# KrainskiL/CGE.jl

Measured on AMD Instinct MI355X. Metric: edge_alpha_evals_per_sec, higher is better.
Workload: dtype f64

## Files before the change

### cge.jl_amd/api.py

```python
from __future__ import annotations

import atexit
import ctypes as C
import os
import sys
import weakref

import numpy as np

from .args import _SplitRule

_HERE = os.path.dirname(os.path.abspath(__file__))
_LIB_PATH = os.path.join(_HERE, "csrc", "build", "libcge_hip.so")
_lib = None

CGE_OK = 0
_CODES = {-1: "AssertionError", -2: "ErrorException: Trying to split homogenous cluster",
          -3: "ErrorException: Unexpected empty cluster generated", -4: "HIP error / no GPU",
          -5: "collective hook failed", -6: "out of memory", -7: "bad argument"}


class CGEError(RuntimeError):
    def __init__(self, code, msg=""):
        super().__init__(f"{_CODES.get(code, 'error')} (code {code}){': ' + msg if msg else ''}")
# ... 103 lines not shown
            ctx.close()
        except Exception:
            pass


def library_path():
    return _LIB_PATH


def load_library():
    global _lib
    if _lib is None:
        if not os.path.exists(_LIB_PATH):
            raise CGEError(-4, f"{_LIB_PATH} not found: build it with `make -C cge.jl_amd/csrc` "
                               f"(or __graft_entry__.build()); there is no CPU fallback")
        L = C.CDLL(_LIB_PATH)
        L.cge_last_error.restype = C.c_char_p
        L.cge_last_error.argtypes = [C.c_void_p]
        L.cge_idx.restype = C.c_int64
        L.cge_idx.argtypes = [C.c_int64] * 3
        L.cge_destroy.argtypes = [C.c_void_p]
        L.cge_destroy.restype = None
        _lib = L
    return _lib


def read_table(path, column_major=True, n_threads=0):
    L = load_library()
    L.cge_text_table_close.argtypes = [C.c_void_p]
    L.cge_text_table_close.restype = None
    rows, cols, hdr, h = C.c_int64(), C.c_int64(), C.c_int(), C.c_void_p()
    err = C.create_string_buffer(512)
    rc = L.cge_text_table_open(os.fsencode(path), C.c_int(n_threads), C.byref(rows), C.byref(cols), C.byref(hdr),
                               C.byref(h), err, C.c_int64(512))
    if rc != 0:
        raise CGEError(rc, err.value.decode() or f"cannot read {path}")
    try:
        out = np.empty((rows.value, cols.value), dtype=np.float64, order="F" if column_major else "C")
        rc = L.cge_text_table_parse(h, out.ctypes.data_as(C.c_void_p), C.c_int(1 if column_major else 0), err,
                                    C.c_int64(512))
        if rc != 0:
            raise CGEError(rc, err.value.decode() or f"cannot parse {path}")
    finally:
        L.cge_text_table_close(h)
    return out, bool(hdr.value)


def _method_code(method):
    if isinstance(method, _SplitRule):
        return method.code
    if isinstance(method, str):
        return {"rss": 0, "rss2": 1, "size": 2, "diameter": 3}[method]
    return int(method)


def _p(a):
    return None if a is None else a.ctypes.data_as(C.c_void_p)


def _f64(a):
    return np.ascontiguousarray(a, dtype=np.float64)


def _i64(a):
    return np.ascontiguousarray(a, dtype=np.int64)


def _colmajor(a):
    a = np.asfortranarray(np.asarray(a, dtype=np.float64))
    return a, a.ravel(order="K")


def _view_layout(n, d, s0, s1):
    if (d == 1 or s1 == 1) and (n == 1 or s0 >= d):
        return 1, (s0 if n > 1 else d)
    if (n == 1 or s0 == 1) and (d == 1 or s1 >= n):
        return 0, (s1 if d > 1 else n)
    return None


def embedding_view(x):
    if isinstance(x, (int, np.integer)):
        raise TypeError("embedding_view: a raw pointer is not a view (Context.set_embedding_device takes device pointers)")
    torch = sys.modules.get("torch")
    v = EmbeddingView()
    if torch is not None and isinstance(x, torch.Tensor):
        codes = {torch.float64: DTYPE_F64, torch.float32: DTYPE_F32, torch.float16: DTYPE_F16, torch.bfloat16: DTYPE_BF16}
        t = x.detach()
        if t.dtype not in codes:
            raise ValueError(f"embedding_view: tensor dtype {t.dtype} (float64, float32, float16 or bfloat16)")
        if t.dim() != 2 or t.shape[0] < 1 or t.shape[1] < 1:
            raise ValueError("embedding_view: an embedding is a non-empty (n, d) matrix")
        lay = _view_layout(t.shape[0], t.shape[1], *t.stride())
        if lay is None:
            t = t.contiguous()
            lay = 1, t.shape[1]
        v.data, v.d, v.dtype, v.on_device = t.data_ptr(), t.shape[1], codes[t.dtype], int(t.is_cuda)
        v.row_major, v.ld = lay
        return v, t
    a = np.asarray(x)
    if a.dtype not in _NP_DTYPES:
        a = np.asarray(a, dtype=np.float64)
    if a.ndim != 2 or a.shape[0] < 1 or a.shape[1] < 1:
        raise ValueError("embedding_view: an embedding is a non-empty (n, d) matrix")
    sz = a.dtype.itemsize
    lay = None if a.strides[0] % sz or a.strides[1] % sz else _view_layout(a.shape[0], a.shape[1], a.strides[0] // sz, a.strides[1] // sz)
# ... 544 lines not shown
    def vect_b_test(self, GD, Ta, Tb, comm, C_, directed=False, form=0, landmarks=False, vC=None, n_modes=1, second=None,
                    vB=None):
        keep, out = [], {}

        def problem(GD, Ta, Tb, comm, C_, vC, vB, tag):
            C_ = int(C_)
            ln = C_ * C_ if directed else C_ * (C_ + 1) // 2
            q = VectBProblem()
            if GD is not None:
                GD, Ta, Tb, comm = _f64(GD), _f64(Ta), _f64(Tb), _i64(comm)
                q.N = GD.shape[0]
                assert GD.shape == (q.N, q.N) and Ta.shape == Tb.shape == comm.shape == (q.N,)
                vect = np.zeros(ln + VECT_B_GUARD)
                q.GD, q.Ta, q.Tb, q.comm = (a.ctypes.data for a in (GD, Ta, Tb, comm))
            else:
                vect = _f64(vB).copy()
                q.N = C_
                assert vect.shape == (ln,) and vC is not None
            q.C = C_
            js_dev, js_fused = np.full(3, np.nan), np.full(2, np.nan)
            if vC is not None:
                vC = _f64(vC)
                assert vC.shape == (ln,)
                q.vC = vC.ctypes.data
            q.vectB, q.js_dev, q.js_fused = vect.ctypes.data, js_dev.ctypes.data, js_fused.ctypes.data
            keep.extend((GD, Ta, Tb, comm, vC, vect, js_dev, js_fused))
            out[tag + "vectB"], out[tag + "guard"] = vect[:ln], vect[ln:]
            out[tag + "js_dev"], out[tag + "js_fused"] = js_dev, js_fused[:n_modes]
            return q

        p1 = problem(GD, Ta, Tb, comm, C_, vC, vB, "")
        p2 = None
        if second is not None:
            p2 = problem(*second[:5], second[5] if len(second) > 5 else None, None, "second_")
        ran = C.c_int(-1)
        self._check(self.L.cge_vect_b_test(self.h, C.byref(p1), C.byref(p2) if p2 is not None else None, C.c_int(int(directed)),
                                           C.c_int(form), C.c_int(int(landmarks)), C.c_int(n_modes), C.byref(ran)))
        out["form_ran"] = ran.value
        return out

    def segment_sort_test(self, z, offsets):
        z = _f64(z)
        off = np.ascontiguousarray(offsets, dtype=np.int32)
        zs, perm = np.empty_like(z), np.empty(z.size, dtype=np.int32)
        self._check(self.L.cge_segment_sort_test(self.h, _p(z), _p(off), C.c_int64(off.size - 1), _p(zs), _p(perm)))
        return zs, perm

    def wave_tree_test(self, x):
        x = np.ascontiguousarray(x, dtype=np.float64).reshape(-1, 64)
        a, b = np.empty(x.shape[0]), np.empty(x.shape[0])
        self._check(self.L.cge_wave_tree_test(self.h, _p(x), C.c_int64(x.shape[0]), _p(a), _p(b)))
        return a, b

    def js(self, vC, vB, vI=None, internal=True):
        vC, vB = _f64(vC), _f64(vB)
        vi = None if vI is None or len(vI) == 0 else np.ascontiguousarray(vI, dtype=np.uint8)
        out = C.c_double()
        self._check(self.L.cge_js(self.h, _p(vC), _p(vB), C.c_int64(len(vC)), _p(vi), C.c_int(int(bool(internal))),
                                  C.byref(out)))
        return out.value

    def exchange_buffer(self, min_doubles):
        ptr, cap = C.c_void_p(), C.c_int64()
        self._check(self.L.cge_exchange_buffer(self.h, C.c_int64(min_doubles), C.byref(ptr), C.byref(cap)))
        return ptr.value, cap.value

    def set_collectives(self, fn, rank, world):
        cb = ALLREDUCE_FN(fn)
        coll = Collectives(cb, None, rank, world)
        self._keep = [cb, coll]
        self._check(self.L.cge_set_collectives(self.h, C.byref(coll)))

    def set_collectives_ext(self, allgather=None, reduce_scatter=None):
        ag = GATHER_FN(allgather) if allgather else GATHER_FN()
        rs = GATHER_FN(reduce_scatter) if reduce_scatter else GATHER_FN()
        ext = CollectivesExt(ag, rs)
        self._keep = list(getattr(self, "_keep", [])) + [ag, rs, ext]
        self._check(self.L.cge_set_collectives_ext(self.h, C.byref(ext)))

    def clear_collectives(self):
        self._check(self.L.cge_comm_finalize(self.h))
        self._check(self.L.cge_set_collectives(self.h, None))
        self._keep = []

    def init_rccl(self, unique_id: bytes, rank: int, world: int):
        assert len(unique_id) == 128
        buf = C.create_string_buffer(bytes(unique_id), 128)
        self._check(self.L.cge_comm_init_rccl(self.h, buf, C.c_int(rank), C.c_int(world)))

    def finalize_rccl(self):
        self._check(self.L.cge_comm_finalize(self.h))

    def rccl_selftest(self, arr, op=0):
        a = np.ascontiguousarray(arr).copy()
        assert a.dtype.itemsize == 8
        self._check(self.L.cge_rccl_selftest(self.h, _p(a), C.c_int64(a.size), C.c_int(op)))
        return a

    def louvain(self):
        out = np.zeros(self.n, dtype=np.int64)
        nc, q, rounds = C.c_int64(), C.c_double(), C.c_int64()
        self._check(self.L.cge_louvain(self.h, _p(out), C.byref(nc), C.byref(q), C.byref(rounds)))
        return out, nc.value, q.value, rounds.value

    _TEST_OPTIONS = ("fit_persistent_test_delay", "fit_persistent_test_timeout", "test_bvec_plain", "test_rss2_one_kernel",
                     "exact_resident_limit")

    def set_option(self, key, value):
        if key in self._TEST_OPTIONS:
            self._check(self.L.cge_set_test_option(self.h, key.encode(), C.c_int64(int(value))))
            return
        self._check(self.L.cge_set_option(self.h, key.encode(), C.c_int64(int(value))))

    def get_stat(self, key):
        v = C.c_int64()
        self._check(self.L.cge_get_stat(self.h, key.encode(), C.byref(v)))
        return v.value

    def last_diameter(self):
        import struct

        hi = struct.unpack("d", struct.pack("q", self.get_stat("diameter_bits")))[0]
        return hi, {1: "brute", 2: "pruned"}.get(self.get_stat("diameter_path"), "none"), \
            self.get_stat("diameter_candidate_pairs"), self.get_stat("diameter_candidate_tiles")

    def profile_enable(self, on=True):
        self._check(self.L.cge_profile_enable(self.h, C.c_int(int(on))))

    def profile_select(self, names=()):
        self._check(self.L.cge_profile_select(self.h, ",".join(names).encode()))

    def profile_reset(self):
        self._check(self.L.cge_profile_reset(self.h))

    def profile(self):
        buf = C.create_string_buffer(4096)
        self._check(self.L.cge_profile_names(self.h, buf, C.c_int64(4096)))
        res = {}
        for name in filter(None, buf.value.decode().split(",")):
            n, ms = C.c_int64(), C.c_double()
            self._check(self.L.cge_profile_get(self.h, name.encode(), C.byref(n), C.byref(ms)))
            res[name] = {"launches": n.value, "total_ms": ms.value}
        return res

    def phase_ms(self):
        res = {}
        buf = C.create_string_buffer(4096)
        self._check(self.L.cge_phase_names(self.h, buf, C.c_int64(4096)))
        for ph in filter(None, buf.value.decode().split(",")):
            ms = C.c_double()
            self._check(self.L.cge_phase_ms(self.h, ph.encode(), C.byref(ms)))
            res[ph] = ms.value
        return res


_default_ctx = None


def default_context():
# ... 96 lines not shown
```

### cge.jl_amd/csrc/capi.cpp

```cpp
#include "common.hpp"
#include "../../include/cge_hip_testing.h"

void flush_timers(cge_ctx *c) {
    for (auto &kv : c->timers) {
        for (auto &pr : kv.second.pending) {
            float ms = 0.f;
            (void)hipEventSynchronize(pr.second);
            if (hipEventElapsedTime(&ms, pr.first, pr.second) == hipSuccess) kv.second.total_ms += ms;
            c->event_pool.push_back(pr.first);
            c->event_pool.push_back(pr.second);
        }
        kv.second.pending.clear();
    }
}
template <class Map>
static int key_names(const Map &m, char *buf, int64_t buf_len) {
    std::string s;
    for (auto &kv : m) s += (s.empty() ? "" : ",") + kv.first;
    snprintf(buf, (size_t)buf_len, "%s", s.c_str());
    return CGE_OK;
}

extern "C" {

// ... 217 lines not shown
    CGE_TRY_ON_DEVICE(c)
    host_js(c, vC, vB, len, vI, internal, out);
    CGE_CATCH(c)
}

int cge_edge_scatter(cge_ctx *c, const int64_t *v_to_l, int64_t N, int64_t C, int directed, int64_t e0, int64_t e1,
                     double *wedges_out, double *vect_C_out) {
    if (!c || N <= 0 || C <= 0 || e0 < 0 || e1 < e0) return CGE_E_ARG;
    CGE_TRY_ON_DEVICE(c)
    host_edge_scatter(c, v_to_l, N, C, directed, e0, e1, wedges_out, vect_C_out);
    CGE_CATCH(c)
}

int cge_louvain(cge_ctx *c, int64_t *comm_out, int64_t *n_comm, double *modularity, int64_t *rounds) {
    if (!c || !comm_out) return CGE_E_ARG;
    CGE_TRY_ON_DEVICE(c)
    if (!c->src.p || c->m <= 0 || c->n <= 0) CGE_THROW(CGE_E_ARG, "louvain: no resident graph (cge_set_graph)");
    if (c->edges_sharded) CGE_THROW(CGE_E_ARG, "louvain: the resident edge list is sharded over the ranks (option shard_ingest)");
    k_louvain_level1(c, comm_out, n_comm, modularity, rounds);
    CGE_CATCH(c)
}

int cge_set_option(cge_ctx *c, const char *key, int64_t value) {
    if (!c || !key) return CGE_E_ARG;
    const auto is = [&](const char *k) { return !strcmp(key, k); };
    const auto ranged = [&](auto &field, int64_t lo, int64_t hi) {
        if (value < lo || value > hi) return (int)CGE_E_ARG;
        field = (std::remove_reference_t<decltype(field)>)value;
        return (int)CGE_OK;
    };
    const auto flag = [&](auto &field) { field = value != 0; return (int)CGE_OK; };
    if (is("diameter")) return ranged(c->opt_diameter, 0, 2);
    if (is("diameter_f32")) return ranged(c->opt_diameter_f32, 0, 2);
    if (is("fit_persistent")) return ranged(c->opt_fit_persistent, 0, 2);
    if (is("pow_exp2")) return flag(c->opt_pow_exp2);
    if (is("shard_runsplit")) return ranged(c->opt_shard_forced, 0, 2);
    if (is("shard_samples")) return ranged(c->opt_shard_samples, 0, 2);
    if (is("exact_relabel")) return flag(c->opt_exact_relabel);
    if (is("bvec_blocks")) return flag(c->opt_bvec_blocks);
    if (is("wedges_reduce_scatter")) return flag(c->opt_wedges_rs);
    if (is("fit_fused")) return flag(c->opt_fit_fused);
    if (is("shard_ingest")) return flag(c->opt_shard_ingest);
    if (is("shard_rows")) return flag(c->opt_shard_rows);
    if (is("landmark_edges")) return flag(c->opt_landmark_edges);
    if (is("exact_packed")) return ranged(c->opt_exact_packed, 0, 1);
    if (is("fit_max_iterations")) return ranged(c->opt_fit_max_iters, 1, INT64_MAX);
    return CGE_E_ARG;
}
int cge_set_test_option(void *ctx, const char *key, int64_t value) {
    cge_ctx *c = (cge_ctx *)ctx;
    if (!c || !key) return CGE_E_ARG;
    if (!strcmp(key, "test_bvec_plain")) { c->opt_test_bvec_plain = value != 0; return CGE_OK; }
    if (!strcmp(key, "test_rss2_one_kernel")) { c->opt_test_rss2_one_kernel = value != 0; return CGE_OK; }
    if (!strcmp(key, "fit_persistent_test_delay") && value >= 0 && value <= 100000) { c->opt_fit_test_delay = (int)value; return CGE_OK; }
    if (!strcmp(key, "fit_persistent_test_timeout")) { c->opt_fit_test_timeout = value != 0; return CGE_OK; }
    if (!strcmp(key, "exact_resident_limit") && value >= 0) { c->opt_test_resident_limit = (double)value; return CGE_OK; }
    return CGE_E_ARG;
}
int cge_get_stat(cge_ctx *c, const char *key, int64_t *value) {
    if (!c || !key || !value) return CGE_E_ARG;
    if (!strcmp(key, "landmarks")) *value = c->lm_ready ? c->N : 0;
    else if (!strcmp(key, "diameter_path")) *value = c->stat_diameter_path;
    else if (!strcmp(key, "diameter_candidate_pairs")) *value = c->stat_cand_pairs;
    else if (!strcmp(key, "diameter_candidate_tiles")) *value = c->stat_cand_tiles;
    else if (!strcmp(key, "diameter_refs")) *value = c->stat_nref;
    else if (!strcmp(key, "diameter_bound_pass")) *value = c->stat_bound_pass;
    else if (!strcmp(key, "diameter_arg_i")) *value = c->stat_hi_i + 1;
    else if (!strcmp(key, "diameter_arg_j")) *value = c->stat_hi_j + 1;
    else if (!strcmp(key, "fit_persistent_alphas")) *value = c->stat_fit_persistent;
    else if (!strcmp(key, "fit_iterations")) *value = c->stat_fit_iters;
    else if (!strcmp(key, "exact_packed")) *value = c->stat_exact_packed;
    else if (!strcmp(key, "exact_matrix_bytes")) *value = c->stat_exact_matrix_bytes;
    else if (!strcmp(key, "fit_fused_alphas")) *value = c->stat_fit_fused;
    else if (!strcmp(key, "fit_persistent_fallbacks")) *value = c->stat_fit_fallbacks;
    else if (!strcmp(key, "fit_batched_launches")) *value = c->stat_fit_batched_launches;
    else if (!strcmp(key, "fit_batched_alphas")) *value = c->stat_fit_batched_alphas;
    else if (!strcmp(key, "landmark_batches")) *value = c->stat_lm_batches;
    else if (!strcmp(key, "landmark_batch_rows")) *value = c->stat_lm_rows;
    else if (!strcmp(key, "landmark_splits")) *value = c->stat_lm_splits;
    else if (!strcmp(key, "cut_tie_tasks")) {
        int v = 0;
        if (c->cut_ties.p && (hipStreamSynchronize(c->stream) != hipSuccess ||
                              hipMemcpy(&v, c->cut_ties.p, sizeof(int), hipMemcpyDeviceToHost) != hipSuccess))
            return CGE_E_HIP;
        *value = v;
    }
    else if (!strcmp(key, "edge_layout_build_us")) *value = c->stat_layout_build_us;
    else if (!strcmp(key, "edge_chunks")) *value = c->be_nchunks;
    else if (!strcmp(key, "edges_resident")) *value = c->m;
    else if (!strcmp(key, "edges_total")) *value = c->m_total;
    else if (!strcmp(key, "embedding_words_resident")) *value = (i64)c->Xr.n;
    else if (!strcmp(key, "rows_resident")) *value = c->Xr.p ? lm_rows(c) : 0;
    else if (!strcmp(key, "rows_total")) *value = c->n;
    else if (!strcmp(key, "collective_calls")) *value = c->stat_coll_calls;
    else if (!strcmp(key, "collective_bytes")) *value = c->stat_coll_bytes;
    else if (!strcmp(key, "diameter_bits")) memcpy(value, &c->stat_last_hi, sizeof(double));
    else return CGE_E_ARG;
    return CGE_OK;
}

int cge_profile_enable(cge_ctx *c, int on) {
    if (!c) return CGE_E_ARG;
    c->profiling = on != 0;
    return CGE_OK;
}
int cge_profile_select(cge_ctx *c, const char *names) {
// ... 118 lines not shown
    CGE_CATCH(c)
}

int cge_vect_b_test(void *ctx, const cge_vect_b_problem *p, const cge_vect_b_problem *p2, int directed, int form, int landmarks,
                    int n_modes, int *form_ran) {
    cge_ctx *c = (cge_ctx *)ctx;
    if (!c || !p || !form_ran || form < 0 || form > 6 || n_modes < 1 || n_modes > 2) return CGE_E_ARG;
    CGE_TRY_ON_DEVICE(c)
    host_vect_b_test(c, p, p2, directed != 0, form, landmarks, n_modes, form_ran);
    CGE_CATCH(c)
}

int cge_segment_sort_test(void *ctx, const double *z, const int32_t *task_row_off, int64_t T, double *zs_out, int32_t *perm_out) {
    cge_ctx *c = (cge_ctx *)ctx;
    if (!c || !z || !task_row_off || !zs_out || !perm_out || T <= 0) return CGE_E_ARG;
    CGE_TRY_ON_DEVICE(c)
    const i64 R = task_row_off[T];
    if (R <= 0) CGE_THROW(CGE_E_ARG, "segment_sort_test: no rows");
    std::vector<i32> rt(R), rows(R);
    i64 max_len = 0;
    for (i64 t = 0; t < T; t++) {
        if (task_row_off[t + 1] <= task_row_off[t]) CGE_THROW(CGE_E_ARG, "segment_sort_test: empty group");
        max_len = std::max<i64>(max_len, task_row_off[t + 1] - task_row_off[t]);
        for (i64 j = task_row_off[t]; j < task_row_off[t + 1]; j++) { rt[j] = (i32)t; rows[j] = (i32)j; }
    }
    DevBuf<double> dz, dzs;
    DevBuf<i32> dtro, drt, drows, dperm, dsrows, dstatus;
    dz.ensure(R); dzs.ensure(R); dtro.ensure(T + 1); drt.ensure(R); drows.ensure(R); dperm.ensure(R); dsrows.ensure(R); dstatus.ensure(T);
    HIP_CHECK(hipMemcpyAsync(dz.p, z, sizeof(double) * R, hipMemcpyHostToDevice, c->stream));
    HIP_CHECK(hipMemcpyAsync(dtro.p, task_row_off, sizeof(i32) * (T + 1), hipMemcpyHostToDevice, c->stream));
    HIP_CHECK(hipMemcpyAsync(drt.p, rt.data(), sizeof(i32) * R, hipMemcpyHostToDevice, c->stream));
    HIP_CHECK(hipMemcpyAsync(drows.p, rows.data(), sizeof(i32) * R, hipMemcpyHostToDevice, c->stream));
    k_segmented_sort_z(c, dz.p, drows.p, drt.p, dtro.p, R, T, dzs.p, dperm.p, dsrows.p, dstatus.p, max_len);
    HIP_CHECK(hipMemcpyAsync(zs_out, dzs.p, sizeof(double) * R, hipMemcpyDeviceToHost, c->stream));
    HIP_CHECK(hipMemcpyAsync(perm_out, dperm.p, sizeof(i32) * R, hipMemcpyDeviceToHost, c->stream));
    HIP_CHECK(hipStreamSynchronize(c->stream));
    CGE_CATCH(c)
}

int cge_wave_tree_test(void *ctx, const double *x, int64_t n_rows, double *out_ref, double *out_new) {
    cge_ctx *c = (cge_ctx *)ctx;
    if (!c || !x || !out_ref || !out_new || n_rows <= 0) return CGE_E_ARG;
    CGE_TRY_ON_DEVICE(c)
    DevBuf<double> dx, da, db;
    dx.ensure((size_t)n_rows * 64); da.ensure(n_rows); db.ensure(n_rows);
    HIP_CHECK(hipMemcpyAsync(dx.p, x, sizeof(double) * n_rows * 64, hipMemcpyHostToDevice, c->stream));
    k_wave_tree_test(c, dx.p, n_rows, da.p, db.p);
    HIP_CHECK(hipMemcpyAsync(out_ref, da.p, sizeof(double) * n_rows, hipMemcpyDeviceToHost, c->stream));
    HIP_CHECK(hipMemcpyAsync(out_new, db.p, sizeof(double) * n_rows, hipMemcpyDeviceToHost, c->stream));
    HIP_CHECK(hipStreamSynchronize(c->stream));
    CGE_CATCH(c)
}

int cge_resident_embedding_test(void *ctx, double *out, int64_t capacity_doubles, int64_t *rows, int64_t *d, int32_t *ids_out) {
    cge_ctx *c = (cge_ctx *)ctx;
    if (!c || !rows || !d) return CGE_E_ARG;
    CGE_TRY_ON_DEVICE(c)
    if (!c->Xr.p || c->d <= 0) CGE_THROW(CGE_E_ARG, "embedding not resident");
    const i64 nl = lm_rows(c);
    *rows = nl;
    *d = c->d;
    if (!out || capacity_doubles < nl * c->d) CGE_THROW(CGE_E_ARG, "resident embedding: %lld x %lld doubles do not fit the buffer", (long long)nl, (long long)c->d);
    HIP_CHECK(hipMemcpyAsync(out, c->Xr.p, sizeof(double) * (size_t)nl * c->d, hipMemcpyDeviceToHost, c->stream));
    HIP_CHECK(hipStreamSynchronize(c->stream));
    if (ids_out)
        for (i64 i = 0; i < nl; i++) ids_out[i] = c->rows_sharded ? c->h_loc2glob[i] : (i32)i;
    CGE_CATCH(c)
}

int cge_resident_graph_test(void *ctx, cge_resident_graph *o) {
    cge_ctx *c = (cge_ctx *)ctx;
    if (!c || !o) return CGE_E_ARG;
    CGE_TRY_ON_DEVICE(c)
    const bool graph = c->src.p && c->dst.p && c->m > 0;
    o->n = c->n;
    o->m = graph ? c->m : 0;
    o->unit = graph && c->unit_weights ? 1 : 0;
    o->n_comm_max = c->comm.p ? c->n_comm_max : 0;
    o->n_comm16 = c->comm16.p ? (i64)c->comm16.n : 0;
    o->have = (c->comm.p ? 1 : 0) | (c->vw.p ? 2 : 0);
    const size_t m = (size_t)o->m, n = (size_t)c->n;
    if (((o->src || o->dst || o->w) && o->cap_edges < o->m) || ((o->comm || o->vweight) && o->cap_vertices < o->n) ||
        (o->comm16 && o->cap_comm16 < o->n_comm16))
        CGE_THROW(CGE_E_ARG, "resident graph: n = %lld, m = %lld, %lld comm16 entries do not fit the buffers", (long long)o->n,
                  (long long)o->m, (long long)o->n_comm16);
    if (o->src && m) HIP_CHECK(hipMemcpyAsync(o->src, c->src.p, sizeof(i32) * m, hipMemcpyDeviceToHost, c->stream));
    if (o->dst && m) HIP_CHECK(hipMemcpyAsync(o->dst, c->dst.p, sizeof(i32) * m, hipMemcpyDeviceToHost, c->stream));
    if (o->w && m && !o->unit) {
        if (!c->w.p || c->h_w.size() != m) CGE_THROW(CGE_E_ARG, "resident graph: a weighted list without its weights or their host mirror");
        HIP_CHECK(hipMemcpyAsync(o->w, c->w.p, sizeof(double) * m, hipMemcpyDeviceToHost, c->stream));
    }
    if (o->comm && c->comm.p) HIP_CHECK(hipMemcpyAsync(o->comm, c->comm.p, sizeof(i32) * n, hipMemcpyDeviceToHost, c->stream));
    if (o->comm16 && c->comm16.p)
        HIP_CHECK(hipMemcpyAsync(o->comm16, c->comm16.p, sizeof(unsigned short) * c->comm16.n, hipMemcpyDeviceToHost, c->stream));
    if (o->vweight && c->vw.p) HIP_CHECK(hipMemcpyAsync(o->vweight, c->vw.p, sizeof(double) * n, hipMemcpyDeviceToHost, c->stream));
    HIP_CHECK(hipStreamSynchronize(c->stream));
    CGE_CATCH(c)
}

}
```

### cge.jl_amd/csrc/common.hpp

```cpp
#pragma once
#include <hip/hip_runtime.h>

#include <algorithm>
#include <atomic>
#include <chrono>
#include <condition_variable>
#include <functional>
#include <mutex>
#include <thread>
#include <cstdint>
#include <cstdio>
#include <cstdlib>
#include <cstring>
#include <map>
#include <memory>
#include <string>
#include <vector>

#include "../../include/cge_hip.h"

typedef int64_t i64;
typedef int32_t i32;

struct MaxRec {
// ... 172 lines not shown
                cv_.wait(lk, [&]() { return gen_ != seen; });
                seen = gen_;
                if (stop_) return;
                job = cur_;
            }
            if (job) work(*job);
        }
    }
    std::vector<std::thread> workers_;
    std::mutex m_;
    std::condition_variable cv_;
    std::shared_ptr<Job> cur_;
    unsigned long long gen_ = 0;
    bool stop_ = false;
};

struct KernelTimer {
    std::vector<std::pair<hipEvent_t, hipEvent_t>> pending;
    i64 launches = 0;
    double total_ms = 0.0;
};

struct Phase {
    std::map<std::string, double> ms;
};

struct ScoreGraph {
    i64 N = 0, d = 0, C = 0;
    const double *emb = nullptr;
    const double *dist = nullptr;
    const double *vw = nullptr;
    const i32 *comm = nullptr;
    const double *vectC = nullptr;
    const double *deg_in = nullptr, *deg_out = nullptr;
};

struct SampleSet {
    i64 S = 0, n_sets = 0;
    std::vector<i64> pos_idx, neg_i, neg_j, pos_idx2;
    bool on_device = false;
    DevBuf<i32> d_pos, d_ni, d_nj, d_pos2;
    void reset() {
        S = n_sets = 0;
        on_device = false;
        pos_idx.clear(); neg_i.clear(); neg_j.clear(); pos_idx2.clear();
    }
};
struct DevSamples {
    DevBuf<i32> pi, pj, ni, nj;
    DevBuf<double> wts, dpos, dneg;
    DevBuf<i32> aidx;
    DevBuf<double> afac;
};

struct cge_ctx {
    int device = 0;
    hipStream_t stream = nullptr;
    bool own_stream = false;
    std::vector<hipEvent_t> event_pool;
    PinBuf<unsigned char> stage[2];
    hipEvent_t stage_ev[2] = {nullptr, nullptr};
    hipStream_t copy_stream = nullptr;
    hipEvent_t copy_ev = nullptr, copy_done = nullptr;
    std::string err;
    int n_threads = 8;
    ThreadPool *pool = nullptr;
    cge_collectives coll{};
    cge_collectives_ext coll_ext{};
    bool has_coll = false;
    int opt_wedges_rs = 0;
    void *rccl_comm = nullptr;
    i64 stat_coll_calls = 0, stat_coll_bytes = 0;
    DevBuf<double> xown;
    double *xptr = nullptr;
    size_t xcap = 0;

    i64 n = 0, m = 0, d = 0;
    i64 m_total = 0, e_first = 0;
    bool edges_sharded = false;
    int opt_shard_ingest = 0;
    DevBuf<double> samp_xchg;
    int opt_shard_rows = 0;
    bool rows_sharded = false;
    i64 n_loc = 0;
    std::vector<i32> h_loc2glob, h_glob2loc;
    std::vector<int> comm_owner;
    DevBuf<i32> loc2glob, glob2loc, comm_loc;
    DevBuf<double> vw_loc;
    std::vector<double> h_vw_loc;
    std::vector<i32> h_gl_off;
    std::vector<int> lm_owner;
    DevBuf<i32> v2l_loc;
    bool wedges_block_only = false;
    bool unit_weights = false;
    bool blocked_ready = false;
    DevBuf<i32> src, dst;
    DevBuf<double> w;
    DevBuf<double> Xr;
    DevBuf<double> Xc;
    DevBuf<double> rnorm;
    i64 ldn = 0, dpad = 0;
    bool centred_ready = false;
    DevBuf<i32> comm;
    DevBuf<unsigned short> comm16;
    DevBuf<double> vw;
    DevBuf<unsigned> be_edge;
// ... 82 lines not shown
    bool fit_persistent_broken = false;
    i64 stat_fit_fallbacks = 0;
    int fit_fallback_streak = 0;
    i64 fit_skip_sweeps = 0;
    DevBuf<i32> sw_cm_off, sw_cm_mem, sw_cm_pos;
    DevBuf<double> sw_zeros, sw_zsum;
    DevBuf<MaxRec> mp_recs;
    DevBuf<i64> mp_count;
    DevBuf<int2> nt_pairs, nt_tiles;
    DevBuf<i32> nt_idx;
    DevBuf<double> nt_out, nt_rows;
    DevBuf<double> mp_rd2, mp_refmu;
    DevBuf<double> mp_commax;
    DevBuf<int2> mp_plist;
    DevBuf<i32> mp_lref, mp_refoff, mp_refmem;
    DevBuf<double> gmean;
    bool emb_nonfinite = false;
    DevBuf<double> Xs, rns, Ms, mnorm, Pm;
    DevBuf<double> pc_groups;
    DevBuf<float> Xs32, Ms32;
    DevBuf<unsigned short> Xb16, Mb16;
    DevBuf<int> dm_flag;
    DevBuf<double> xe, xe_rns, dm_seed;
    DevBuf<i32> xe_pos, xe_glob, xe_sub, dm_soffE;
    int opt_diameter_f32 = 2;
    DevBuf<i32> pos2node, sub_land, dm_soff, dm_memoff, dm_mem;
    DevBuf<BoundRec> bound_list;
    DevBuf<int2> tile_list;
    std::vector<i32> h_mem_off, h_mem;
    DevBuf<uint64_t> uniq_hash;
    DevBuf<unsigned long long> uniq_table;
    int opt_diameter = 0;
    i64 stat_cand_pairs = 0, stat_cand_tiles = 0;
    int stat_diameter_path = 0;
    double stat_last_hi = 0.0;
    i64 stat_hi_i = -1, stat_hi_j = -1;
    int stat_bound_pass = 0;
    i64 stat_nref = 0;
    DevBuf<i32> ls_rows, ls_row_task, ls_ct, ls_cb, ls_ce, ls_co, ls_tco;
    DevBuf<double> ls_part, ls_mean, ls_sw, ls_cov, ls_vec, ls_z, ls_sums;
    DevBuf<unsigned char> ls_side, ls_state;
    DevBuf<double> ls_params;
    PinBuf<double> pin_sums, pin_params;
    PinBuf<i32> pin_clusters;
    PinBuf<i32> pin_hb_rows, pin_hb_row_task;
    DevBuf<i32> sp_srows, sp_meta, sp_rounds, sp_tro, sp_perm, sp_status, sort_idx, sort_idx2, sort_keys32, sort_k32b, sort_cnt;
    DevBuf<unsigned char> sort_keys8;
    DevBuf<i32> lm_arena;
    i64 lm_arena_used = 0;
    DevBuf<double> lm_means;
    i64 lm_means_used = 0;
    DevBuf<i64> ls_moff;
    PinBuf<i32> pin_tab[2], pin_res;
    DevBuf<i32> dev_tab, dev_res;
    hipEvent_t tab_ev[2] = {nullptr, nullptr};
    int tab_slot = 0;
    bool lm_index_on_device = false;
    DevBuf<i32> ls_toff, ls_nlow, lm_goff, lm_glen, lm_mem, lm_memoff;
    DevBuf<unsigned char> ls_keys;
    PinBuf<i32> pin_small;
    DevBuf<unsigned char> sort_tmp;
    DevBuf<unsigned long long> sort_k64;

    DevBuf<double> sp_zs, sp_ctot, sp_coff, sp_prefix, sp_vals;
    DevBuf<double> r2_F, r2_ck;
    i64 r2_rows = 0;

    int opt_landmark_edges = 0;
    DevBuf<i32> epd_i, s_star;
    DevBuf<i64> wed_cnt;
    DevBuf<double> cc_dense;
    DevBuf<unsigned> samp_attempt;
    DevBuf<i32> samp_todo_a, samp_todo_b, samp_hit, samp_flag;
    DevBuf<unsigned long long> samp_table, samp_count;
    struct DrawPending {
        bool on = false;
        i64 seed = 0, stream_id = 0, S = 0, cnt = 0;
        int directed = 0, round = 0;
        i32 *d_pos = nullptr, *d_ni = nullptr, *d_nj = nullptr;
        const i32 *todo = nullptr;
        i32 *next = nullptr;
    } samp_pending;
    PinBuf<unsigned long long> samp_pin_cnt;
    hipEvent_t samp_ev = nullptr;
    SampleSet smp;
    std::vector<std::unique_ptr<DevSamples>> dsets;

    bool profiling = false;
    std::vector<std::string> profile_only;
    std::map<std::string, KernelTimer> timers;
    Phase phases;
};

struct ScopedKernelTimer {
    cge_ctx *c;
    KernelTimer *t = nullptr;
    hipEvent_t a = nullptr, b = nullptr;
    ScopedKernelTimer(cge_ctx *ctx, const char *name) : c(ctx) {
        if (!c->profiling) return;
        if (!c->profile_only.empty()) {
            bool hit = false;
            for (const std::string &n : c->profile_only) hit = hit || n == name;
            if (!hit) return;
        }
        t = &c->timers[name];
        a = take_event();
        b = take_event();
// ... 148 lines not shown
              RES_LEN = RES_FIT + 2, RES_STRIDE = RES_FIT + 16;
#define CGE_PREFIX_STRIDE 8
void k_gather_means(cge_ctx *c, const double *arena, const i64 *off, i64 T, i64 d, double *mean);
void k_gather_rows(cge_ctx *c, const i32 *arena, const i32 *task_off, const i32 *task_row_off, const i32 *chunk_task,
                   const i32 *chunk_beg, const i32 *chunk_end, i64 n_chunks, i32 *rows, i32 *row_task);
void k_rss_child_keys(cge_ctx *c, const i32 *perm, const i32 *row_task, const i32 *task_row_off, const i32 *meta,
                      const i32 *rounds, i64 R, i64 T, unsigned char *keys, i32 *nlow);
void k_side_counts(cge_ctx *c, const unsigned char *side, const i32 *task_row_off, i64 T, i32 *nlow);
void k_sort_children(cge_ctx *c, const unsigned char *keys, const i32 *rows, const i32 *task_row_off, const i32 *chunk_beg,
                     const i32 *chunk_end, const i32 *task_chunk_off, i64 n_chunks, i64 R, i64 T, int key_bits, i32 *out);
i64 k_groups_to_index(cge_ctx *c, const i32 *arena, const i32 *goff, const i32 *glen, i64 N, i64 n, i32 *v2l, i32 *mem);
void k_segmented_sort_z(cge_ctx *c, const double *z, const i32 *rows, const i32 *row_task, const i32 *task_row_off,
                        i64 R, i64 T, double *zs, i32 *perm, i32 *srows, i32 *status, i64 max_len = 0 );
void k_rss_side(cge_ctx *c, const double *z, const i32 *row_task, i64 n_rows, const double *params,
                unsigned char *state, unsigned char *side);
bool k_group_eig(cge_ctx *c, const double *cov, i64 n_tasks, i64 d, double *vec);
void k_group_project(cge_ctx *c, const double *Xr, const double *vw, const i32 *rows, const i32 *row_task, i64 n_rows,
                     i64 d, const double *mean, const double *vec, double *z);
void k_landmark_aggregate(cge_ctx *c, const double *Xr, const double *vw, const i32 *comm, const i32 *mem_off,
                          const i32 *mem, i64 N, i64 d, double *lemb, double *lweight, double *dii, i32 *lcomm);
bool k_edge_scatter_blocked_applies(const cge_ctx *c, i64 C);
bool k_blocked_edges_possible(const cge_ctx *c);
void k_pack_upper(cge_ctx *c, const double *dense, i64 C, double *packed);
bool k_build_blocked_edges(cge_ctx *c);
void k_edge_scatter_blocked(cge_ctx *c, i64 c0, i64 c1, i64 C, int directed, double *vectC);
bool k_wedge_scatter_blocked(cge_ctx *c, const i32 *v2l, i64 N, i64 c0, i64 c1, int directed, double *wedges, i64 *positive,
                             const char *timer = "edge_scatter_wedges");
#define CGE_COMM16_PAD 32768
void k_edge_scatter(cge_ctx *c, const i32 *src, const i32 *dst, const double *w, i64 e0, i64 e1, const i32 *v2l,
                    const i32 *comm, i64 N, i64 C, int directed, double *wedges, double *vectC);
void k_edge_degrees(cge_ctx *c, const i32 *src, const i32 *dst, const double *w, i64 m, double *deg_out,
                    double *deg_in, i32 *star);
void k_wedge_degrees(cge_ctx *c, const double *wedges, i64 N, double *deg_out, double *deg_in, i32 *star);
void k_compact_count(cge_ctx *c, const double *wedges, i64 N, int directed, i64 *count, i64 row0 = 0, i64 row1 = -1);
void k_wedge_degrees_block(cge_ctx *c, const double *wedges, i64 N, i64 row0, i64 row1, double *out3N);
void k_degrees_unpack(cge_ctx *c, const double *in3N, i64 N, double *deg_out, double *deg_in, i32 *star);
void k_louvain_level1(cge_ctx *c, i64 *comm_out_host, i64 *n_comm, double *quality, i64 *rounds);
void k_dist_matrix(cge_ctx *c, const double *emb, const double *diag, i64 N, i64 d, double *D);
void k_minmax_upper(cge_ctx *c, const double *D, i64 N, double *lo_hi);
void k_normalise(cge_ctx *c, double *D, i64 N, const double *lo_hi);
void k_packed_extrema(cge_ctx *c, const double *emb, const double *diag, i64 N, i64 d, double *lo_hi);
void k_packed_gd(cge_ctx *c, const double *emb, const double *diag, i64 N, i64 d, const double *lo_hi, double alpha,
                 int pow_method, double *PK);
void k_max_pair(cge_ctx *c, const double *Xc, const double *rnorm, i64 n, i64 ldn, i64 dpad, int part, int nparts,
                double *best_val, i64 *best_i, i64 *best_j, std::vector<double> *wg_best = nullptr);
void k_pair_dist(cge_ctx *c, const double *Xr, i64 d, const i32 *pi, const i32 *pj, i64 S, double inv_scale_den,
                 double *out);
void k_diameter_layout(cge_ctx *c, const i32 *mem_off, const i32 *mem, const i32 *soff, i64 N, i32 *pos2node, i32 *sub_land,
                       i64 n_sub);
void k_pcent(cge_ctx *c, const double *Xs, const double *rns, i64 lds_rows, const double *Ms, const double *mnorm,
             i64 ldm, i64 n_land, i64 N, i64 dpad, const i32 *soff, double *P, int part = 0, int nparts = 1);
void k_max_pair_tile_list(i64 ldn, int part, int nparts, const std::vector<double> &wg, double thr, std::vector<int2> &out);
i64 k_pair_collect(cge_ctx *c, const double *Xs, const double *rns, i64 ld, i64 nrows, i64 dpad, const int2 *tiles, i64 t0, i64 t1,
                   int tri, double thr, const i32 *ids, int2 *out, i64 cap);
void k_pair_list(cge_ctx *c, const double *Xs, const double *rns, i64 lds_rows, i64 npos, i64 dpad, const int2 *tiles,
                 i64 ntiles, double *best_val, i64 *best_i, i64 *best_j, std::vector<double> *wg_best = nullptr);
i64 k_bound_select(cge_ctx *c, const double *Q, const i32 *lref, i64 N, i64 nref, double L, BoundRec *list, i64 cap,
                   const i32 *ref_off = nullptr, const i32 *ref_mem = nullptr);
void k_ref_dist2_fm(cge_ctx *c, const double *Ms_fm, i64 nref, i64 dpad, i64 ldm);
i64 k_argmax_mapped(cge_ctx *c, const double *v, i64 n, const i32 *map, double *val = nullptr);
void k_pair_local_idx(cge_ctx *c, const i32 *pi, const i32 *pj, i64 S, const i32 *glob2loc, i32 *idx);
void k_pair_dist_rows(cge_ctx *c, const double *B, i64 d, const i32 *pi, const i32 *pj, i64 S, double den, double *out);
void k_position_ids(cge_ctx *c, const i32 *pos2node, const i32 *loc2glob, i64 npos, i32 *ids);
void k_ref_centroids(cge_ctx *c, const double *mu, const double *lw, const i32 *ref_off, const i32 *ref_mem, i64 nref,
                     i64 d, double *out);
void k_farthest_enqueue(cge_ctx *c, const double *Xr, i64 n, i64 d, i64 src, const double *srow = nullptr);
void k_farthest_collect(cge_ctx *c, double *best_val, i64 *best_i);
void k_col_mean(cge_ctx *c, const double *Xrow, i64 n, i64 d, double *mean, double sums_only = 0.0);
void k_scale_vector(cge_ctx *c, double *v, i64 n, double f);
void k_pack_landmarks(cge_ctx *c, double *lemb, double *lweight, double *dii, i32 *lcomm, i64 N, i64 d, double *X, int unpack);
void k_scatter_u64(cge_ctx *c, const uint64_t *src, const i32 *idx, i64 cnt, uint64_t *dst);
void k_scatter_i32(cge_ctx *c, const i32 *src, const i32 *idx, i64 cnt, i32 add, i32 *dst);
void k_add_i32(cge_ctx *c, const i32 *src, i64 n, i32 add, i32 *dst);
void k_gather_centre_fm(cge_ctx *c, const double *src_rowmajor, const i32 *idx, const double *mean, double *dst,
                        double *rnorm, i64 npos, i64 d, i64 ld, i64 dpad, float *dst32 = nullptr,
                        unsigned short *planes = nullptr, i64 KP = 0, int *flag = nullptr);
void k_pcent_f32(cge_ctx *c, const float *Xs32, const double *rns, i64 lds_rows, const float *Ms32, const double *mnorm,
                 i64 ldm, i64 n_land, i64 N, i64 dpad, const i32 *sub_land, double *P, int part = 0, int nparts = 1);
bool k_pcent_bf16_applies(i64 dpad);
void k_pcent_bf16(cge_ctx *c, const unsigned short *Xb, const double *rns, i64 lds_rows, const unsigned short *Mb,
                  const double *mnorm, i64 ldm, i64 n_land, i64 N, i64 KP, const i32 *sub_land, double *P, int part = 0, int nparts = 1);
void k_wave_tree_test(cge_ctx *c, const double *x, i64 n_rows, double *out_ref, double *out_new);
void k_copy_segments(cge_ctx *c, const i32 *src, const i64 *seg, i64 nseg, i32 *dst);
void k_permute_rows(cge_ctx *c, const double *src, const i32 *order, i64 n, i64 width, double *dst);
void k_permute_i32(cge_ctx *c, const i32 *src, const i32 *order, i64 n, i32 *dst);
void k_remap_i32(cge_ctx *c, i32 *idx, const i32 *map, i64 n);
#define CGE_WORD_SEGS 8
void k_copy_words(cge_ctx *c, int nseg, void *const *dst, const void *const *src, const i64 *words);
struct WordPacker {
    cge_ctx *c;
    std::vector<void *> dst;
    std::vector<const void *> src;
    std::vector<i64> words;
    explicit WordPacker(cge_ctx *c_) : c(c_) {}
    template <class T>
    void add(T *device, const T *host, i64 count) {
        static_assert(sizeof(T) % 4 == 0, "4-byte words");
        if (count <= 0) return;
        dst.push_back(device);
        src.push_back(host);
        words.push_back(count * (i64)(sizeof(T) / 4));
    }
    void flush() {
        if (dst.empty()) return;
        i64 tot = 0;
        for (i64 w : words) tot += w + (w & 1);
        const int slot = c->tab_slot;
        c->tab_slot ^= 1;
        HIP_CHECK(hipEventSynchronize(c->tab_ev[slot]));
        c->pin_tab[slot].ensure((size_t)tot);
        c->dev_tab.ensure((size_t)tot);
        i32 *h = c->pin_tab[slot].p;
        std::vector<const void *> dsrc(dst.size());
        i64 pos = 0;
        for (size_t q = 0; q < dst.size(); q++) {
            std::memcpy(h + pos, src[q], (size_t)words[q] * 4);
            dsrc[q] = c->dev_tab.p + pos;
            pos += words[q] + (words[q] & 1);
        }
        HIP_CHECK(hipMemcpyAsync(c->dev_tab.p, h, sizeof(i32) * (size_t)tot, hipMemcpyHostToDevice, c->stream));
        HIP_CHECK(hipEventRecord(c->tab_ev[slot], c->stream));
        for (size_t q0 = 0; q0 < dst.size(); q0 += CGE_WORD_SEGS) {
            const int n = (int)std::min<size_t>(CGE_WORD_SEGS, dst.size() - q0);
            k_copy_words(c, n, &dst[q0], &dsrc[q0], &words[q0]);
        }
        dst.clear(); src.clear(); words.clear();
    }
};
void k_gather_means_slots(cge_ctx *c, const double *arena, const i64 *off, const i64 *slot, i64 T, i64 d, i64 stride, i64 lead,
                          double *dst);
void k_pow_prepare(cge_ctx *c, const double *D, i64 N, bool upper_only, bool blocked = false);
void k_pow_matrix(cge_ctx *c, const double *D, i64 N, double alpha, double *GD, bool upper_only = false);
void k_pow_test(cge_ctx *c, const double *x, i64 n, double alpha, int method, double *out);
#define CGE_FLOW_NP 32
struct cge_fit_fused {
    const double *Lh; const float *Ll; double alpha;
    const i32 *comm, *fc, *ns, *base; double *partial;
    i64 S; const double *dpos, *dneg, *wts; const i32 *aidx; const double *afac, *aden; double *apw; double *auc_part;
};
bool k_fit_flow_enqueue(cge_ctx *c, const double *GD, i64 N, const double *T0, double *Tout, i64 Tld, const double *w,
                        double eps, double delta, int *dev_flags, const cge_fit_fused *ff = nullptr,
                        const cge_fit_fused *ff_dev = nullptr);
bool k_fit_flow_fused_applies(cge_ctx *c, i64 N);
void k_bins_prepare(cge_ctx *c, const i32 *cm_off, i64 N, i64 C, i64 n_partials);
struct cge_chain_tail {
    double *host_out; const double *scal; int res_js, res_len;
    uint4 *arm; i64 arm_n16; unsigned arm_word;
};
void k_bins_js(cge_ctx *c, const i32 *cm_off, i64 N, i64 C, const double *vC, double *vectB, int n_modes, double *fpart,
               const cge_chain_tail *tail = nullptr);
bool k_fit_flow_arm_region(cge_ctx *c, i64 N, i64 Tld, uint4 **ptr, i64 *n16, unsigned *word);
struct cge_flow_problem {
    const double *Lh; const float *Ll; double alpha; const cge_fit_fused *epi; int want, pad0;
    const double *T0; double *Tout; const double *w;
    double *ring, *P, *fq; unsigned *sync; int *flags;
    i64 N, Tld; int Nt, G, wg0, pad1;
};
bool k_fit_flow_geometry(i64 N, int *G, int *NW);
i64 k_fit_flow_slot_doubles(i64 N, i64 Tld);
#define CGE_BATCH_MAX 16
struct cge_flow_multi { cge_flow_problem p[CGE_BATCH_MAX]; int n, pad; };
void k_fit_flow_multi(cge_ctx *c, cge_flow_multi &tab, int NW, double eps, double delta, DevBuf<double> &flow);
bool k_fit_flow_multi_fits(int NW);
struct cge_bins_problem { const double *partial; const i32 *cm_off, *fc, *ns, *base; i64 C; int Nt, pad; double *vectB; };
struct cge_js_problem { const double *vC, *vB; i64 len, C; int mode, pad; double *part, *fpart; };
struct cge_bins_multi { cge_bins_problem p[CGE_BATCH_MAX]; };
struct cge_js_multi { cge_js_problem p[2 * CGE_BATCH_MAX]; };
void k_bins_js_multi(cge_ctx *c, const cge_bins_multi &bins, int n_bins, i64 max_C, const cge_js_multi &js, int n_js);
void k_bvec_tiles(cge_ctx *c, const double *GD, const double *Ta, const double *Tb, const i32 *cm_off, i64 N, int directed,
                  bool packed = false);
void k_auc_prepare(cge_ctx *c, const i32 *v2l, const i32 *old2new, const double *vw_orig, const double *lweight, const i32 *pi,
                   const i32 *pj, const i32 *ni, const i32 *nj, const double *wts, i64 S, i32 *aidx, double *afac, double *aden);
void k_bvec_bins(cge_ctx *c, const i32 *cm_off, i64 N, i64 C, int directed, double *vectB);
bool k_fit_persistent_dir(cge_ctx *c, const double *GD, i64 N, double *Tin, double *Tout, const double *deg_in,
                          const double *deg_out, double eps0, double f0, double delta, i64 *iters, int *dev_flags = nullptr,
                          bool *enqueued_only = nullptr);
void k_fit_verdict(cge_ctx *c, const int *flags, int async, double *out);
void k_fit_sym_step(cge_ctx *c, const double *GD, const double *Tin, double *Tout, const double *w, i64 N, double eps,
                double delta, int k, unsigned long long *fring, int *done, int *iters, bool packed = false);
void k_fit_symv_dir(cge_ctx *c, const double *GD, const double *Tin, const double *Tout, i64 N, double *Sin,
                    double *Sout, const int *done);
// ... 153 lines not shown
```

### cge.jl_amd/csrc/diameter_host.cpp

```cpp
#include <algorithm>
#include <cmath>
#include <functional>
#include <limits>

#include "common.hpp"

namespace {
struct ExactBest {
    double hi = -1.0;
    i64 i = 0, j = 0;
    void offer(double v, i64 a, i64 b) {
        if (a > b) std::swap(a, b);
        if (v > hi || (v == hi && (a < i || (a == i && b < j)))) { hi = v; i = a; j = b; }
    }
};
struct SideStream {
    cge_ctx *c;
    explicit SideStream(cge_ctx *c_) : c(c_) { std::swap(c->stream, c->copy_stream); }
    ~SideStream() { std::swap(c->stream, c->copy_stream); }
};
}

static double gram_delta(i64 dpad, double rmax) { return (double)(8 * dpad + 32) * 2.220446049250313e-16 * rmax; }

static void dm_eval_pairs(cge_ctx *c, const int2 *pairs, i64 cnt, ExactBest &eb) {
    const i64 d = c->d;
    hipStream_t st = c->stream;
    const i64 CH = 1 << 16;
    if (!c->rows_sharded) {
        std::vector<i32> ij;
        std::vector<double> val;
        for (i64 k0 = 0; k0 < cnt; k0 += CH) {
            const i64 kc = std::min(CH, cnt - k0);
            ij.resize(2 * kc);
            val.resize(kc);
            for (i64 k = 0; k < kc; k++) { ij[k] = pairs[k0 + k].x; ij[kc + k] = pairs[k0 + k].y; }
            c->nt_idx.ensure(2 * kc);
            c->nt_out.ensure(kc);
            HIP_CHECK(hipMemcpyAsync(c->nt_idx.p, ij.data(), sizeof(i32) * 2 * kc, hipMemcpyHostToDevice, st));
            k_pair_dist(c, c->Xr.p, d, c->nt_idx.p, c->nt_idx.p + kc, kc, 1.0, c->nt_out.p);
            HIP_CHECK(hipMemcpyAsync(val.data(), c->nt_out.p, sizeof(double) * kc, hipMemcpyDeviceToHost, st));
            HIP_CHECK(hipStreamSynchronize(st));
            for (i64 k = 0; k < kc; k++) eb.offer(val[k], ij[k], ij[kc + k]);
        }
        return;
    }
    const int W = c->coll.world, me = c->coll.rank;
    const i64 RCH = 4096;
    const i64 steps = (i64)cge_allreduce_scalar_max(c, (double)((cnt + RCH - 1) / RCH));
    std::vector<int2> all((size_t)W * RCH);
    std::vector<i32> loc, two;
    std::vector<double> val;
    for (i64 s = 0; s < steps; s++) {
        const i64 k0 = s * RCH, kc = std::max<i64>(0, std::min(RCH, cnt - k0));
        c->nt_pairs.ensure((size_t)W * RCH);
        HIP_CHECK(hipMemsetAsync(c->nt_pairs.p, 0, sizeof(int2) * W * RCH, st));
        std::vector<int2> mine(kc);
        for (i64 k = 0; k < kc; k++) mine[k] = make_int2(pairs[k0 + k].x + 1, pairs[k0 + k].y + 1);
        if (kc > 0) HIP_CHECK(hipMemcpyAsync(c->nt_pairs.p + (size_t)me * RCH, mine.data(), sizeof(int2) * kc, hipMemcpyHostToDevice, st));
        HIP_CHECK(hipStreamSynchronize(st));
        cge_allreduce_dev(c, reinterpret_cast<double *>(c->nt_pairs.p), W * RCH, 2);
        HIP_CHECK(hipMemcpyAsync(all.data(), c->nt_pairs.p, sizeof(int2) * W * RCH, hipMemcpyDeviceToHost, st));
        HIP_CHECK(hipStreamSynchronize(st));
        loc.clear();
        std::vector<int2> got;
        for (const int2 &q : all)
            if (q.x > 0 && q.y > 0) {
                got.push_back(make_int2(q.x - 1, q.y - 1));
                loc.push_back(c->h_glob2loc[q.x - 1]);
                loc.push_back(c->h_glob2loc[q.y - 1]);
            }
        const i64 T = (i64)got.size();
        if (T == 0) continue;
        two.resize(2 * T);
        for (i64 k = 0; k < T; k++) { two[k] = (i32)(2 * k); two[T + k] = (i32)(2 * k + 1); }
        val.resize(T);
        c->nt_idx.ensure(4 * T);
        c->nt_rows.ensure((size_t)2 * T * d);
        c->nt_out.ensure(T);
        HIP_CHECK(hipMemcpyAsync(c->nt_idx.p, loc.data(), sizeof(i32) * 2 * T, hipMemcpyHostToDevice, st));
        HIP_CHECK(hipMemcpyAsync(c->nt_idx.p + 2 * T, two.data(), sizeof(i32) * 2 * T, hipMemcpyHostToDevice, st));
        k_gather_rows_f64(c, c->Xr.p, c->n_loc, d, 1, c->nt_idx.p, 2 * T, c->nt_rows.p);
        cge_allreduce_dev(c, c->nt_rows.p, 2 * T * d, 2);
        k_pair_dist(c, c->nt_rows.p, d, c->nt_idx.p + 2 * T, c->nt_idx.p + 3 * T, T, 1.0, c->nt_out.p);
        HIP_CHECK(hipMemcpyAsync(val.data(), c->nt_out.p, sizeof(double) * T, hipMemcpyDeviceToHost, st));
        HIP_CHECK(hipStreamSynchronize(st));
        for (i64 k = 0; k < T; k++) eb.offer(got[k].x == got[k].y ? 0.0 : val[k], got[k].x, got[k].y);
    }
}

static const i64 NT_CAP = (i64)1 << 20;
template <class Flush>
static void dm_collect(cge_ctx *c, const double *Xs, const double *rns, i64 ld, i64 nrows, i64 dpad, const std::vector<int2> &tl,
                       int tri, double thr, const i32 *ids, Flush flush) {
    const i64 ntiles = (i64)tl.size();
    if (ntiles == 0) return;
    c->nt_pairs.ensure((size_t)NT_CAP);
    c->nt_tiles.ensure((size_t)ntiles);
    HIP_CHECK(hipMemcpyAsync(c->nt_tiles.p, tl.data(), sizeof(int2) * ntiles, hipMemcpyHostToDevice, c->stream));
    std::vector<int2> h;
    i64 t0 = 0, step = std::min<i64>(ntiles, (i64)1 << 17);
    while (t0 < ntiles) {
        const i64 t1 = std::min(ntiles, t0 + step);
        const i64 cnt = k_pair_collect(c, Xs, rns, ld, nrows, dpad, c->nt_tiles.p, t0, t1, tri, thr, ids, c->nt_pairs.p, NT_CAP);
        if (cnt > NT_CAP) {
            if (t1 - t0 <= 1) CGE_THROW(CGE_E_ARG, "diameter: a tile with more pairs than it has entries");
            step = (t1 - t0 + 1) / 2;
            continue;
        }
        if (cnt > 0) {
            h.resize(cnt);
            HIP_CHECK(hipMemcpyAsync(h.data(), c->nt_pairs.p, sizeof(int2) * cnt, hipMemcpyDeviceToHost, c->stream));
            HIP_CHECK(hipStreamSynchronize(c->stream));
            flush(h.data(), cnt);
        }
        t0 = t1;
    }
}

static void ensure_centred(cge_ctx *c) {
    if (c->centred_ready) return;
    if (c->rows_sharded) CGE_THROW(CGE_E_ARG, "the brute-force diameter over the whole embedding needs every row on one rank; the resident rows are sharded (option shard_rows)");
    if (!c->Xr.p || c->d <= 0) CGE_THROW(CGE_E_ARG, "diameter: embedding not resident");
    c->Xc.alloc_exact((size_t)c->ldn * c->dpad);
    c->rnorm.alloc_exact((size_t)c->ldn);
    k_gather_centre_fm(c, c->Xr.p, nullptr, c->gmean.p, c->Xc.p, c->rnorm.p, c->n, c->d, c->ldn, c->dpad);
    c->centred_ready = true;
}

double host_diameter_brute(cge_ctx *c, int part, int nparts, i64 *ai, i64 *aj) {
    ExactBest eb;
    if (c->emb_nonfinite)
        eb.hi = std::numeric_limits<double>::quiet_NaN();
    else {
        ensure_centred(c);
        double bv;
        i64 bi, bj;
        std::vector<double> wg;
        k_max_pair(c, c->Xc.p, c->rnorm.p, c->n, c->ldn, c->dpad, part, nparts, &bv, &bi, &bj, &wg);
        if (bv > -1.0) {
            double rmax = 0.0;
            k_argmax_mapped(c, c->rnorm.p, c->n, nullptr, &rmax);
            const double thr = bv - gram_delta(c->dpad, rmax);
            std::vector<int2> tl;
            k_max_pair_tile_list(c->ldn, part, nparts, wg, thr, tl);
            dm_collect(c, c->Xc.p, c->rnorm.p, c->ldn, c->n, c->dpad, tl, 1, thr, nullptr,
                       [&](const int2 *p, i64 cnt) { dm_eval_pairs(c, p, cnt, eb); });
        }
        if (eb.hi < 0.0) eb.hi = 0.0;
    }
    c->stat_diameter_path = 1;
    c->stat_hi_i = eb.i; c->stat_hi_j = eb.j;
    if (ai) *ai = eb.i + 1;
    if (aj) *aj = eb.j + 1;
    return eb.hi;
}

struct DmPrep {
    std::vector<i64> soff;
    i64 npos = 0, lds_rows = 0;
    const i32 *d_off = nullptr, *d_mem = nullptr;
    bool by_comm = false;
    i64 nref = 0, ldm = 0, KP = 0;
    const double *mu_ref = nullptr;
    bool b16 = false, f32 = false;
    double seed_norm = -1.0;
// ... 47 lines not shown
            if (lcomm[a] < 0 || lcomm[a] >= C) CGE_THROW(CGE_E_ARG, "diameter: landmark community out of range");
            lref[a] = lcomm[a];
            roff[lcomm[a] + 1]++;
        }
        for (i64 q = 0; q < C; q++) roff[q + 1] += roff[q];
        std::vector<i32> cur(roff.begin(), roff.end() - 1);
        for (i64 a = 0; a < N; a++) rmem[cur[lcomm[a]]++] = (i32)a;
        c->mp_refoff.ensure(C + 1);
        c->mp_refmem.ensure(N);
        c->mp_refmu.ensure((size_t)C * d);
        c->mp_lref.ensure(N);
        WordPacker pk(c);
        pk.add(c->mp_refoff.p, roff.data(), C + 1);
        pk.add(c->mp_refmem.p, rmem.data(), N);
        pk.add(c->mp_lref.p, lref.data(), N);
        pk.flush();
        k_ref_centroids(c, mu, lw, c->mp_refoff.p, c->mp_refmem.p, C, d, c->mp_refmu.p);
        mu_ref = c->mp_refmu.p;
    } else {
        for (i64 a = 0; a < N; a++) lref[a] = (i32)a;
        c->mp_lref.ensure(N);
        WordPacker pk(c);
        pk.add(c->mp_lref.p, lref.data(), N);
        pk.flush();
    }
    const i64 ldm = S.ldm = (nref + 127) / 128 * 128;
    c->rns.ensure(lds_rows);
    c->Ms.ensure((size_t)ldm * dpad);
    c->mnorm.ensure(ldm);
    c->Pm.ensure((size_t)N * nref);
    bool &b16 = S.b16, &f32 = S.f32;
    b16 = c->opt_diameter_f32 >= 2 && k_pcent_bf16_applies(dpad);
    f32 = c->opt_diameter_f32 != 0 && !b16;
    const i64 KP = S.KP = (dpad + 31) / 32 * 32;
    if (f32) {
        c->Xs32.ensure((size_t)lds_rows * dpad);
        c->Ms32.ensure((size_t)ldm * dpad);
    }
    if (b16) {
        c->Xb16.ensure((size_t)2 * lds_rows * KP);
        c->Mb16.ensure((size_t)2 * ldm * KP);
    }
    const bool lowp = b16 || f32;
    if (lowp) {
        c->dm_flag.ensure(1);
        HIP_CHECK(hipMemsetAsync(c->dm_flag.p, 0, sizeof(int), st));
    } else
        c->Xs.ensure((size_t)lds_rows * dpad);
    k_gather_centre_fm(c, c->Xr.p, c->pos2node.p, c->gmean.p, lowp ? nullptr : c->Xs.p, c->rns.p, npos, d, lds_rows, dpad,
                       f32 ? c->Xs32.p : nullptr, b16 ? c->Xb16.p : nullptr, KP, lowp ? c->dm_flag.p : nullptr);
    k_gather_centre_fm(c, mu_ref, nullptr, c->gmean.p, c->Ms.p, c->mnorm.p, nref, d, ldm, dpad, f32 ? c->Ms32.p : nullptr,
                       b16 ? c->Mb16.p : nullptr, KP, lowp ? c->dm_flag.p : nullptr);
    int unfit = 0;
    if (lowp) HIP_CHECK(hipMemcpyAsync(&unfit, c->dm_flag.p, sizeof(int), hipMemcpyDeviceToHost, st));
    S.seed_norm = -1.0;
    S.seed_vertex = k_argmax_mapped(c, c->rns.p, npos, c->pos2node.p, &S.seed_norm);
    if (RS && lowp) {
        const double bad = cge_allreduce_scalar_max(c, (unfit & 1) ? 1.0 : 0.0), big = cge_allreduce_scalar_max(c, (unfit & 2) ? 1.0 : 0.0);
        unfit = (bad != 0.0 ? 1 : 0) | (big != 0.0 ? 2 : 0);
    }
    if (lowp && ((unfit & 1) || !(unfit & 2))) {
        b16 = f32 = false;
        c->Xs.ensure((size_t)lds_rows * dpad);
        k_gather_centre_fm(c, c->Xr.p, c->pos2node.p, c->gmean.p, c->Xs.p, c->rns.p, npos, d, lds_rows, dpad, nullptr, nullptr, KP, nullptr);
    }
    c->stat_bound_pass = b16 ? 2 : (f32 ? 1 : 0);
    return true;
}

static void dm_bound_pass(cge_ctx *c, const DmPrep &S, i64 N, int part, int nparts) {
    const i64 dpad = c->dpad;
    if (S.npos > 0) {
        if (S.b16)
            k_pcent_bf16(c, c->Xb16.p, c->rns.p, S.lds_rows, c->Mb16.p, c->mnorm.p, S.ldm, N, S.nref, S.KP, c->sub_land.p, c->Pm.p, part, nparts);
        else if (S.f32)
            k_pcent_f32(c, c->Xs32.p, c->rns.p, S.lds_rows, c->Ms32.p, c->mnorm.p, S.ldm, N, S.nref, dpad, c->dm_soff.p, c->Pm.p, part, nparts);
        else
            k_pcent(c, c->Xs.p, c->rns.p, S.lds_rows, c->Ms.p, c->mnorm.p, S.ldm, N, S.nref, dpad, c->sub_land.p, c->Pm.p, part, nparts);
    } else
        HIP_CHECK(hipMemsetAsync(c->Pm.p, 0, sizeof(double) * (size_t)(N * S.nref), c->stream));
}

struct DmSearch {
    cge_ctx *c;
    const bool RS;
    const int W, me;
    const int part, nparts;
    const i64 N;
    const std::vector<i32> &gl_off;
    DmPrep prep;
    double rmax = -1.0;
    double L = 0.0;
    i64 far_i = -1, far_j = -1;
    double delta = 0.0;
    ExactBest eb;
    double best = 0.0;
    std::vector<BoundRec> cand;
    size_t left = 0;
    double tphase = now_ms();
    void lap(const char *name) { const double t = now_ms(); c->phases.ms[name] += t - tphase; tphase = t; }
    i64 len16(i64 a) const { return (i64)((gl_off[a + 1] - gl_off[a] + 15) / 16 * 16); }
    i64 pair_tiles(const BoundRec &r, const std::function<void(i64, i64)> &visit = nullptr) const {
        const i64 ta = (len16(r.a) + 127) / 128, tb = (len16(r.b) + 127) / 128;
        if (visit)
            for (i64 x = 0; x < ta; x++)
                for (i64 y = (r.a == r.b ? x : 0); y < tb; y++) visit(x, y);
        return r.a == r.b ? ta * (ta + 1) / 2 : ta * tb;
    }
};
// ... 20 lines not shown
        k_ref_dist2_fm(c, c->Ms.p, P.nref, c->dpad, P.ldm);
        return;
    }
    hipStream_t st = c->stream;
    const int winner = dm_elect(c, P.seed_norm, P.seed_vertex >= 0, &S.rmax);
    c->dm_seed.ensure(d + 1);
    HIP_CHECK(hipMemsetAsync(c->dm_seed.p, 0, sizeof(double) * (d + 1), st));
    if (winner == S.me) {
        HIP_CHECK(hipMemcpyAsync(c->dm_seed.p, c->Xr.p + P.seed_vertex * d, sizeof(double) * d, hipMemcpyDeviceToDevice, st));
        const double gid = (double)(c->h_loc2glob[P.seed_vertex] + 1);
        HIP_CHECK(hipMemcpyAsync(c->dm_seed.p + d, &gid, sizeof(double), hipMemcpyHostToDevice, st));
        HIP_CHECK(hipStreamSynchronize(st));
    }
    cge_allreduce_dev(c, c->dm_seed.p, d + 1, 2);
    double gid = 0.0;
    HIP_CHECK(hipMemcpyAsync(&gid, c->dm_seed.p + d, sizeof(double), hipMemcpyDeviceToHost, st));
    HIP_CHECK(hipStreamSynchronize(st));
    S.far_i = S.far_j = (i64)gid - 1;
    k_farthest_enqueue(c, c->Xr.p, lm_rows(c), d, 0, c->dm_seed.p);
    k_ref_dist2_fm(c, c->Ms.p, P.nref, c->dpad, P.ldm);
}

static void dm_bounds(DmSearch &S) {
    cge_ctx *c = S.c;
    const DmPrep &P = S.prep;
    double v = -1.0, Lmax;
    i64 q = 0;
    if (S.RS) {
        k_farthest_collect(c, &v, &q);
        const int winner = dm_elect(c, v, true, &Lmax);
        const double qid = cge_allreduce_scalar_max(c, winner == S.me ? (double)(c->h_loc2glob[q] + 1) : 0.0);
        if (Lmax > S.L) { S.L = Lmax; S.far_j = (i64)qid - 1; }
    }
    const bool shard_q = !S.RS && S.nparts > 1 && c->has_coll && (c->rccl_comm || (c->xptr && (size_t)(S.N * P.nref) <= c->xcap));
    dm_bound_pass(c, P, S.N, shard_q ? S.part : 0, shard_q ? S.nparts : 1);
    if (shard_q || S.RS) cge_allreduce_dev(c, c->Pm.p, S.N * P.nref, 1);
    S.lap("dm_refs_pcent");
    if (!S.RS) {
        SideStream side(c);
        k_farthest_collect(c, &v, &q);
        if (v > S.L) { S.L = v; S.far_j = q; }
    }
    S.lap("dm_farthest");
}

static bool dm_select(DmSearch &S) {
    cge_ctx *c = S.c;
    const DmPrep &P = S.prep;
    S.delta = gram_delta(c->dpad, std::max(S.rmax, 0.0));
    const int2 far = make_int2((int)S.far_i, (int)S.far_j);
    dm_eval_pairs(c, &far, 1, S.eb);
    const i64 cap = std::min<i64>(S.N * (S.N + 1) / 2, (i64)4 << 20);
    c->bound_list.ensure((size_t)cap);
    const i64 cnt = k_bound_select(c, c->Pm.p, c->mp_lref.p, S.N, P.nref, S.L * (1.0 - 1e-9), c->bound_list.p, cap,
                                   P.by_comm ? c->mp_refoff.p : nullptr, P.by_comm ? c->mp_refmem.p : nullptr);
    c->stat_cand_pairs = cnt;
    if (cnt > cap) {
        if (S.RS) CGE_THROW(CGE_E_ARG, "diameter (shard_rows): the bounds prune too little (more than %lld candidate landmark pairs) and the brute-force "
                                       "fallback needs every row on one rank", (long long)cap);
        return false;
    }
    S.cand.resize(cnt);
    if (cnt > 0) {
        HIP_CHECK(hipMemcpyAsync(S.cand.data(), c->bound_list.p, sizeof(BoundRec) * cnt, hipMemcpyDeviceToHost, c->stream));
        HIP_CHECK(hipStreamSynchronize(c->stream));
    }
    S.lap("dm_select");
    std::make_heap(S.cand.begin(), S.cand.end(), cand_later);
    S.left = S.cand.size();
    double tiles_total = 0.0;
    for (const BoundRec &r : S.cand) tiles_total += (double)S.pair_tiles(r);
    const double nT = (double)((c->n + 127) / 128);
    if (!S.RS && c->opt_diameter != 2 && tiles_total > 0.5 * nT * (nT + 1) / 2) return false;
    S.best = S.L - S.delta;
    return true;
}

struct DmRound {
    std::vector<BoundRec> pairs;
    std::vector<i32> lms;
    std::vector<char> in_round;
    std::vector<i32> eoff;
    i64 E = 0, ldE = 0;
    i64 tile_cap = 4096;
    i64 global_tile = 0;
    explicit DmRound(i64 N) : in_round(N, 0), eoff(N + 1) {}
};

static bool dm_round_fill(DmSearch &S, DmRound &R) {
    const i64 pos_cap = std::max<i64>(8192, ((i64)512 << 20) / (S.c->dpad * 8));
    std::vector<BoundRec> &cand = S.cand;
    R.pairs.clear();
    R.lms.clear();
    R.E = 0;
    i64 ntile = 0;
    while (S.left > 0 && ntile < R.tile_cap) {
        std::pop_heap(cand.begin(), cand.begin() + S.left, cand_later);
        const BoundRec r = cand[S.left - 1];
        if (r.B * (1.0 + 1e-9) + 1e-9 < S.best) { S.left = 0; break; }
        const i64 extra = (R.in_round[r.a] ? 0 : S.len16(r.a)) + ((r.b != r.a && !R.in_round[r.b]) ? S.len16(r.b) : 0);
        if (!R.pairs.empty() && R.E + extra > pos_cap) {
            std::push_heap(cand.begin(), cand.begin() + S.left, cand_later);
            break;
        }
        S.left--;
        R.pairs.push_back(r);
        for (i32 a : {r.a, r.b})
            if (!R.in_round[a]) { R.in_round[a] = 1; R.lms.push_back(a); R.E += S.len16(a); }
        ntile += S.pair_tiles(r);
    }
    R.tile_cap = 131072;
    return !R.pairs.empty();
}

static void dm_round_gather(DmSearch &S, DmRound &R) {
    cge_ctx *c = S.c;
    const i64 N = S.N, d = c->d, dpad = c->dpad, E = R.E;
    i64 at = 0;
    for (i64 a = 0; a < N; a++) {
// ... 147 lines not shown
```

### cge.jl_amd/csrc/kernels_dist.hip

```cpp
#include "common.hpp"
#include <type_traits>
#include "mfma_tile.hpp"

#define WAVE 64

#define DT 64
#define DK 16
__device__ __forceinline__ void tile_dist2(const double *__restrict__ emb, i64 N, i64 d, i64 i0, i64 j0, int ty, int tx,
                                           double (*As)[DK + 1], double (*Bs)[DK + 1], double acc[4][4]) {
#pragma unroll
    for (int a = 0; a < 4; a++)
#pragma unroll
        for (int b = 0; b < 4; b++) acc[a][b] = 0.0;
    for (i64 k0 = 0; k0 < d; k0 += DK) {
        __syncthreads();
        for (int e = threadIdx.x; e < DT * DK; e += 256) {
            const int r = e / DK, kk = e % DK;
            const i64 k = k0 + kk;
            As[r][kk] = (i0 + r < N && k < d) ? emb[(i0 + r) * d + k] : 0.0;
            Bs[r][kk] = (j0 + r < N && k < d) ? emb[(j0 + r) * d + k] : 0.0;
        }
        __syncthreads();
        const int kmax = (int)min((i64)DK, d - k0);
        for (int kk = 0; kk < kmax; kk++) {
// ... 700 lines not shown
        d4 acc[4][4];
        gram_tile_128(Xs + (i64)wave * lds_rows + i0 + c2, Xs + (i64)wave * lds_rows + j0 + c2, lds_rows, lds_rows,
                      nchunk, lds, acc, wave, c2, wr, wc, lr, lk);
#pragma unroll
        for (int b = 0; b < 4; b++) {
            const i64 j = j0 + wc * 64 + b * 16 + lr;
            const double rj = rns[j];
#pragma unroll
            for (int a = 0; a < 4; a++)
#pragma unroll
                for (int r = 0; r < 4; r++) {
                    const i64 i = i0 + wr * 64 + a * 16 + lk + 4 * r;
                    if (i < npos && j < npos) {
                        const double v = gram_value(rns[i], rj, acc[a][b][r]);
                        if (v > best) { best = v; best_i = i; best_j = j; }
                    }
                }
        }
    }
    reduce_best(best, best_i, best_j, lds, recs);
}

__global__ __launch_bounds__(256, 2) void pair_collect_kernel(const double *__restrict__ Xs, const double *__restrict__ rns, i64 ld,
                                                              i64 nrows, i64 dpad, const int2 *__restrict__ tiles, i64 t0, i64 t1,
                                                              int tri, double thr, const i32 *__restrict__ ids,
                                                              int2 *__restrict__ out, unsigned *__restrict__ count, unsigned cap) {
    extern __shared__ __attribute__((aligned(16))) double lds[];
    const int tid = threadIdx.x, wave = tid >> 6, lane = tid & 63;
    const int wr = wave >> 1, wc = wave & 1, lr = lane & 15, lk = lane >> 4, c2 = lane * 2;
    const i64 nchunk = dpad / MP_BK;
    for (i64 t = t0 + blockIdx.x; t < t1; t += gridDim.x) {
        const i64 i0 = tiles[t].x, j0 = tiles[t].y;
        d4 acc[4][4];
        gram_tile_128(Xs + (i64)wave * ld + i0 + c2, Xs + (i64)wave * ld + j0 + c2, ld, ld, nchunk, lds, acc, wave, c2, wr, wc, lr, lk);
#pragma unroll
        for (int b = 0; b < 4; b++) {
            const i64 j = j0 + wc * 64 + b * 16 + lr;
            const double rj = rns[j];
#pragma unroll
            for (int a = 0; a < 4; a++)
#pragma unroll
                for (int r = 0; r < 4; r++) {
                    const i64 i = i0 + wr * 64 + a * 16 + lk + 4 * r;
                    const bool in = tri ? (j < nrows && i < j) : (i < nrows && j < nrows);
                    if (in && gram_value(rns[i], rj, acc[a][b][r]) >= thr) {
                        const unsigned at = atomicAdd(count, 1u);
                        if (at < cap) out[at] = ids ? make_int2(ids[i] - 1, ids[j] - 1) : make_int2((int)i, (int)j);
                    }
                }
        }
    }
}

static void best_of_recs(cge_ctx *c, const MaxRec *d_recs, int nwg, double *bv, i64 *bi, i64 *bj, std::vector<double> *wg = nullptr) {
    std::vector<MaxRec> h(nwg);
    HIP_CHECK(hipMemcpyAsync(h.data(), d_recs, sizeof(MaxRec) * nwg, hipMemcpyDeviceToHost, c->stream));
    HIP_CHECK(hipStreamSynchronize(c->stream));
    *bv = -1.0; *bi = 0; *bj = 0;
    for (int k = 0; k < nwg; k++)
        if (h[k].val > *bv || (h[k].val == *bv && (h[k].i < *bi || (h[k].i == *bi && h[k].j < *bj)))) {
            *bv = h[k].val; *bi = h[k].i; *bj = h[k].j;
        }
    if (wg) {
        wg->resize(nwg);
        for (int k = 0; k < nwg; k++) (*wg)[k] = h[k].val;
    }
}
#define MP_NWG 512
#define MP_LDS_BYTES ((size_t)2 * 2 * MP_BK * MP_LD * sizeof(double))

void k_max_pair(cge_ctx *c, const double *Xc, const double *rnorm, i64 n, i64 ldn, i64 dpad, int part, int nparts,
                double *best_val, i64 *best_i, i64 *best_j, std::vector<double> *wg_best) {
    c->mp_recs.ensure(MP_NWG);
    MaxRec *recs = c->mp_recs.p;
    {
        ScopedKernelTimer t(c, "max_pair_dist");
        hipLaunchKernelGGL(max_pair_kernel, dim3(MP_NWG), dim3(256), MP_LDS_BYTES, c->stream, Xc, rnorm, n, ldn, dpad,
                           part, nparts, recs);
    }
    best_of_recs(c, recs, MP_NWG, best_val, best_i, best_j, wg_best);
}

void k_pcent(cge_ctx *c, const double *Xs, const double *rns, i64 lds_rows, const double *Ms, const double *mnorm,
             i64 ldm, i64 n_land, i64 N, i64 dpad, const i32 *sub_land, double *P, int part, int nparts) {
    HIP_CHECK(hipMemsetAsync(P, 0, sizeof(double) * n_land * N, c->stream));
    ScopedKernelTimer t(c, "pcent");
    const i64 nTI = lds_rows / MP_BM, I0 = nTI * part / nparts, I1 = nTI * (part + 1) / nparts;
    const i64 ntiles = (I1 - I0) * (ldm / MP_BN);
    if (ntiles <= 0) return;
    hipLaunchKernelGGL(pcent_kernel, dim3((unsigned)std::min<i64>(ntiles, 2048)), dim3(256), MP_LDS_BYTES, c->stream, Xs,
                       rns, lds_rows, Ms, mnorm, ldm, N, dpad, sub_land, reinterpret_cast<unsigned long long *>(P), I0, I1,
                       1.0 + (double)(dpad + 8) * 2.220446049250313e-16);
}

void k_pcent_f32(cge_ctx *c, const float *Xs32, const double *rns, i64 lds_rows, const float *Ms32, const double *mnorm,
                 i64 ldm, i64 n_land, i64 N, i64 dpad, const i32 *soff, double *P, int part, int nparts) {
    const i64 ngroups = lds_rows / 16;
    c->pc_groups.ensure((size_t)ngroups * ldm);
    if (nparts > 1) HIP_CHECK(hipMemsetAsync(c->pc_groups.p, 0, sizeof(double) * (size_t)ngroups * ldm, c->stream));
    ScopedKernelTimer t(c, "pcent");
    const i64 nTI = lds_rows / 128, I0 = nTI * part / nparts, I1 = nTI * (part + 1) / nparts;
    const i64 ntiles = (I1 - I0) * (ldm / 128);
    const double e1 = 1.0 + 1.01 * (double)(dpad + 3) * 5.9604644775390625e-08;
    if (ntiles > 0 && dpad <= 128) {
        cge_allow_lds((const void *)pcent_f32_rowres_kernel, 160 * 1024);
        const size_t lds = ((size_t)dpad * 128 + 2 * PF_BK * 128) * sizeof(float);
        hipLaunchKernelGGL(pcent_f32_rowres_kernel, dim3((unsigned)std::min<i64>(I1 - I0, 512)), dim3(256), lds, c->stream, Xs32, rns,
                           lds_rows, Ms32, mnorm, ldm, N, dpad, c->pc_groups.p, I0, I1, e1);
    } else if (ntiles > 0)
        hipLaunchKernelGGL(pcent_f32_kernel, dim3((unsigned)std::min<i64>(ntiles, 2048)), dim3(256), PF_LDS_BYTES, c->stream,
// ... 3 lines not shown

bool k_pcent_bf16_applies(i64 dpad) { return (dpad + 31) / 32 * 32 <= 128; }
void k_pcent_bf16(cge_ctx *c, const unsigned short *Xb, const double *rns, i64 lds_rows, const unsigned short *Mb,
                  const double *mnorm, i64 ldm, i64 n_land, i64 N, i64 KP, const i32 *sub_land, double *P, int part, int nparts) {
    HIP_CHECK(hipMemsetAsync(P, 0, sizeof(double) * n_land * N, c->stream));
    ScopedKernelTimer t(c, "pcent");
    const i64 nTI = lds_rows / 128, I0 = nTI * part / nparts, I1 = nTI * (part + 1) / nparts;
    const double e1 = 1.0 + 1.05 * (3.0 * (double)(KP + 2) * 1.1920928955078125e-07 + 3.2 * 1.52587890625e-05);
    if (I1 > I0) {
        const size_t lds = (size_t)4 * 128 * (KP + PB_APAD) * sizeof(unsigned short) + (size_t)8 * 128 * sizeof(double);
        const int pb_diag = 0;
#define PB_GO(NKS)                                                                                                         \
    do {                                                                                                                   \
        auto kern = pcent_bf16_kernel<NKS>;                                                                                 \
        cge_allow_lds((const void *)kern, 160 * 1024); \
        hipLaunchKernelGGL(kern, dim3((unsigned)std::min<i64>(I1 - I0, 256)), dim3(PB_T), lds, c->stream, Xb, rns, lds_rows, Mb, \
                           mnorm, ldm, sub_land, N, reinterpret_cast<unsigned long long *>(P), I0, I1, e1, pb_diag);        \
    } while (0)
        if (KP == 32) PB_GO(2);
        else if (KP == 64) PB_GO(4);
        else if (KP == 96) PB_GO(6);
        else PB_GO(8);
#undef PB_GO
    }
}

void k_pair_list(cge_ctx *c, const double *Xs, const double *rns, i64 lds_rows, i64 npos, i64 dpad, const int2 *tiles,
                 i64 ntiles, double *best_val, i64 *best_i, i64 *best_j, std::vector<double> *wg_best) {
    c->mp_recs.ensure(MP_NWG);
    MaxRec *recs = c->mp_recs.p;
    const int nwg = (int)std::max<i64>(1, std::min<i64>(ntiles, MP_NWG));
    {
        ScopedKernelTimer t(c, "pair_list");
        hipLaunchKernelGGL(pair_list_kernel, dim3(nwg), dim3(256), MP_LDS_BYTES, c->stream, Xs, rns, lds_rows, npos,
                           dpad, tiles, ntiles, recs);
    }
    best_of_recs(c, recs, nwg, best_val, best_i, best_j, wg_best);
}

void k_max_pair_tile_list(i64 ldn, int part, int nparts, const std::vector<double> &wg, double thr, std::vector<int2> &out) {
    const i64 nT = ldn / MP_BM, nS = (nT + MP_SB - 1) / MP_SB, total = nS * (nS + 1) / 2 * MP_SB * MP_SB;
    out.clear();
    for (i64 b = 0; b < (i64)wg.size(); b++) {
        if (!(wg[b] >= thr)) continue;
        for (i64 t = b; t < total; t += (i64)wg.size()) {
            i64 SI, I, J;
            tile_from_linear(t, nS, SI, I, J);
            if (I >= nT || J >= nT || J < I || (SI % nparts) != part) continue;
            out.push_back(make_int2((int)(I * MP_BM), (int)(J * MP_BN)));
        }
    }
}
i64 k_pair_collect(cge_ctx *c, const double *Xs, const double *rns, i64 ld, i64 nrows, i64 dpad, const int2 *tiles, i64 t0, i64 t1,
                   int tri, double thr, const i32 *ids, int2 *out, i64 cap) {
    if (t1 <= t0) return 0;
    c->mp_count.ensure(2);
    unsigned *cnt = reinterpret_cast<unsigned *>(c->mp_count.p);
    HIP_CHECK(hipMemsetAsync(cnt, 0, sizeof(unsigned), c->stream));
    {
        ScopedKernelTimer t(c, "pair_collect");
        hipLaunchKernelGGL(pair_collect_kernel, dim3((unsigned)std::min<i64>(t1 - t0, MP_NWG)), dim3(256), MP_LDS_BYTES, c->stream, Xs, rns,
                           ld, nrows, dpad, tiles, t0, t1, tri, thr, ids, out, cnt, (unsigned)cap);
    }
    unsigned h = 0;
    HIP_CHECK(hipMemcpyAsync(&h, cnt, sizeof(unsigned), hipMemcpyDeviceToHost, c->stream));
    HIP_CHECK(hipStreamSynchronize(c->stream));
    return (i64)h;
}

__global__ __launch_bounds__(256) void bound_select_kernel(const double *__restrict__ Q, const i32 *__restrict__ lref,
                                                           const double *__restrict__ rd2, i64 N, i64 nref, double L,
                                                           BoundRec *__restrict__ list, i64 cap,
                                                           unsigned long long *__restrict__ count) {
    const i64 total = N * N, stride = (i64)gridDim.x * blockDim.x;
    for (i64 e = (i64)blockIdx.x * blockDim.x + threadIdx.x; e < total; e += stride) {
        const i64 a = e / N, b = e - a * N;
        if (b < a) continue;
        const i64 ra = lref[a], rb = lref[b];
        const double qaa = Q[a * nref + ra], qbb = Q[b * nref + rb];
        const double pre = Q[a * nref + rb] + Q[b * nref + ra] + 2.0 * sqrt(qaa * qbb);
        if (pre * (1.0 + 1e-9) + 1e-9 < L) continue;
        const double Bv = pre - rd2[ra * nref + rb] * (1.0 - 1e-9);
        if (Bv * (1.0 + 1e-9) + 1e-9 >= L) {
            const unsigned long long idx = atomicAdd(count, 1ULL);
            if ((i64)idx < cap) list[idx] = BoundRec{Bv, (i32)a, (i32)b};
        }
    }
}
__global__ __launch_bounds__(256) void ref_dist2_fm_kernel(const double *__restrict__ Ms, i64 nref, i64 dpad, i64 ldm,
                                                           double *__restrict__ rd2) {
    const i64 a = blockIdx.x;
    for (i64 b = threadIdx.x; b < nref; b += blockDim.x) {
        double s = 0.0;
#pragma unroll 8
        for (i64 k = 0; k < dpad; k++) {
            const double df = Ms[k * ldm + a] - Ms[k * ldm + b];
            s += df * df;
        }
        rd2[a * nref + b] = s;
    }
}
__global__ __launch_bounds__(256) void comm_max_kernel(const double *__restrict__ Q, const i32 *__restrict__ ref_off,
                                                       const i32 *__restrict__ ref_mem, i64 nref, double *__restrict__ Mx) {
    const i64 ca = blockIdx.x;
    const i32 b = ref_off[ca], e = ref_off[ca + 1];
    for (i64 r = threadIdx.x; r < nref; r += blockDim.x) {
        double v = 0.0;
        for (i32 t = b; t < e; t++) v = fmax(v, Q[(i64)ref_mem[t] * nref + r]);
        Mx[ca * nref + r] = v;
    }
}
__global__ __launch_bounds__(256) void comm_pairs_kernel(const double *__restrict__ Mx, const double *__restrict__ rd2, i64 C,
                                                         double L, int2 *__restrict__ plist, unsigned *__restrict__ pcount) {
    const i64 total = C * C, stride = (i64)gridDim.x * blockDim.x;
    for (i64 e = (i64)blockIdx.x * blockDim.x + threadIdx.x; e < total; e += stride) {
        const i64 ca = e / C, cb = e - ca * C;
        if (cb < ca) continue;
        const double pre = Mx[ca * C + cb] + Mx[cb * C + ca] + 2.0 * sqrt(Mx[ca * C + ca] * Mx[cb * C + cb]);
        if (pre * (1.0 + 1e-9) + 1e-9 < L) continue;
        const double Bv = pre - rd2[ca * C + cb] * (1.0 - 1e-9);
        if (Bv * (1.0 + 1e-9) + 1e-9 >= L) plist[atomicAdd(pcount, 1u)] = make_int2((int)ca, (int)cb);
    }
}
__global__ __launch_bounds__(256) void bound_expand_kernel(const double *__restrict__ Q, const double *__restrict__ rd2,
                                                           const i32 *__restrict__ ref_off, const i32 *__restrict__ ref_mem,
                                                           i64 nref, double L, const int2 *__restrict__ plist,
                                                           const unsigned *__restrict__ pcount, BoundRec *__restrict__ list,
                                                           i64 cap, unsigned long long *__restrict__ count) {
    const unsigned np = *pcount;
    for (unsigned q = blockIdx.x; q < np; q += gridDim.x) {
        const i64 ca = plist[q].x, cb = plist[q].y;
        const i32 a0 = ref_off[ca], na = ref_off[ca + 1] - a0, b0 = ref_off[cb], nb = ref_off[cb + 1] - b0;
        const double r2 = rd2[ca * nref + cb] * (1.0 - 1e-9);
        for (i64 e = threadIdx.x; e < (i64)na * nb; e += blockDim.x) {
            const i64 ia = e / nb, ib = e - ia * nb;
            i64 a = ref_mem[a0 + ia], b = ref_mem[b0 + ib];
            if (ca == cb && b < a) continue;
            i64 ra = ca, rb = cb;
            if (b < a) { const i64 t = a; a = b; b = t; ra = cb; rb = ca; }
            const double qaa = Q[a * nref + ra], qbb = Q[b * nref + rb];
            const double pre = Q[a * nref + rb] + Q[b * nref + ra] + 2.0 * sqrt(qaa * qbb);
            if (pre * (1.0 + 1e-9) + 1e-9 < L) continue;
            const double Bv = pre - r2;
            if (Bv * (1.0 + 1e-9) + 1e-9 >= L) {
                const unsigned long long idx = atomicAdd(count, 1ULL);
                if ((i64)idx < cap) list[idx] = BoundRec{Bv, (i32)a, (i32)b};
            }
        }
    }
}
void k_ref_dist2_fm(cge_ctx *c, const double *Ms_fm, i64 nref, i64 dpad, i64 ldm) {
    c->mp_rd2.ensure((size_t)nref * nref);
    hipLaunchKernelGGL(ref_dist2_fm_kernel, dim3((unsigned)nref), dim3(256), 0, c->stream, Ms_fm, nref, dpad, ldm, c->mp_rd2.p);
}
i64 k_bound_select(cge_ctx *c, const double *Q, const i32 *lref, i64 N, i64 nref, double L, BoundRec *list, i64 cap,
                   const i32 *ref_off, const i32 *ref_mem) {
    c->mp_count.ensure(2);
    HIP_CHECK(hipMemsetAsync(c->mp_count.p, 0, 2 * sizeof(i64), c->stream));
    ScopedKernelTimer tm(c, "bound_select");
    if (ref_off && ref_mem) {
        c->mp_commax.ensure((size_t)nref * nref);
        c->mp_plist.ensure((size_t)nref * (nref + 1) / 2);
        hipLaunchKernelGGL(comm_max_kernel, dim3((unsigned)nref), dim3(256), 0, c->stream, Q, ref_off, ref_mem, nref, c->mp_commax.p);
        hipLaunchKernelGGL(comm_pairs_kernel, dim3(grid_for(nref * nref, 256)), dim3(256), 0, c->stream, c->mp_commax.p, c->mp_rd2.p,
                           nref, L, c->mp_plist.p, reinterpret_cast<unsigned *>(c->mp_count.p + 1));
        hipLaunchKernelGGL(bound_expand_kernel, dim3(2048), dim3(256), 0, c->stream, Q, c->mp_rd2.p, ref_off, ref_mem, nref, L,
                           c->mp_plist.p, reinterpret_cast<const unsigned *>(c->mp_count.p + 1), list, cap,
                           reinterpret_cast<unsigned long long *>(c->mp_count.p));
    } else
        hipLaunchKernelGGL(bound_select_kernel, dim3(grid_for(N * N, 256)), dim3(256), 0, c->stream, Q, lref, c->mp_rd2.p, N,
                           nref, L, list, cap, reinterpret_cast<unsigned long long *>(c->mp_count.p));
    i64 cnt = 0;
    HIP_CHECK(hipMemcpyAsync(&cnt, c->mp_count.p, sizeof(i64), hipMemcpyDeviceToHost, c->stream));
    HIP_CHECK(hipStreamSynchronize(c->stream));
    return cnt;
}

__device__ __forceinline__ double row16_sum(double v) {
    const auto mv = [](double x, auto ctrl) {
        const long long b = __double_as_longlong(x);
        const int lo = __builtin_amdgcn_update_dpp(0, (int)(unsigned)b, decltype(ctrl)::value, 0xf, 0xf, false);
        const int hi = __builtin_amdgcn_update_dpp(0, (int)(unsigned)(b >> 32), decltype(ctrl)::value, 0xf, 0xf, false);
        return __longlong_as_double(((long long)hi << 32) | (unsigned)lo);
    };
    v += mv(v, std::integral_constant<int, 0xB1>());
    v += mv(v, std::integral_constant<int, 0x4E>());
    v += mv(v, std::integral_constant<int, 0x141>());
    v += mv(v, std::integral_constant<int, 0x140>());
    return v;
}
__global__ __launch_bounds__(256) void farthest_kernel(const double *__restrict__ Xr, i64 n, i64 d, i64 src,
                                                       const double *__restrict__ srow, MaxRec *__restrict__ recs) {
    extern __shared__ __attribute__((aligned(16))) double lds[];
    const int lane = threadIdx.x & 63, sub = lane & 15, quarter = lane >> 4;
    const i64 wave_global = ((i64)blockIdx.x * blockDim.x + threadIdx.x) >> 6;
    const i64 nwaves = ((i64)gridDim.x * blockDim.x) >> 6;
    const double *s = srow ? srow : Xr + src * d;
    double best = -1.0;
    i64 bi = 0;
    for (i64 base = wave_global * 8; base < n; base += nwaves * 8) {
        const i64 i0 = base + quarter, i1 = base + 4 + quarter;
        const bool in0 = i0 < n, in1 = i1 < n;
        const double *x0 = Xr + (in0 ? i0 : 0) * d, *x1 = Xr + (in1 ? i1 : 0) * d;
        double a0 = 0.0, a1 = 0.0;
        if ((d & 1) == 0) {
            const d2 *p0 = reinterpret_cast<const d2 *>(x0), *p1 = reinterpret_cast<const d2 *>(x1),
                     *s2 = reinterpret_cast<const d2 *>(s);
            for (i64 k = sub; k < (d >> 1); k += 16) {
                const d2 sv = s2[k], v0 = p0[k], v1 = p1[k];
                const double t0 = v0.x - sv.x, t1 = v0.y - sv.y, u0 = v1.x - sv.x, u1 = v1.y - sv.y;
                a0 += t0 * t0 + t1 * t1;
                a1 += u0 * u0 + u1 * u1;
            }
        } else
            for (i64 k = sub; k < d; k += 16) {
                const double t = x0[k] - s[k], u = x1[k] - s[k];
                a0 += t * t;
                a1 += u * u;
            }
        a0 = row16_sum(a0);
        a1 = row16_sum(a1);
        if (in0 && a0 > best) { best = a0; bi = i0; }
        if (in1 && a1 > best) { best = a1; bi = i1; }
    }
    reduce_best(best, bi, src, lds, recs);
}
__global__ __launch_bounds__(256) void argmax_kernel(const double *__restrict__ v, i64 n, const i32 *__restrict__ map,
                                                     MaxRec *__restrict__ recs) {
    extern __shared__ __attribute__((aligned(16))) double lds[];
    double best = -1.0;
    i64 bi = 0;
    for (i64 i = (i64)blockIdx.x * blockDim.x + threadIdx.x; i < n; i += (i64)gridDim.x * blockDim.x)
        if (v[i] > best) { best = v[i]; bi = i; }
    reduce_best(best, bi, map ? (i64)map[bi] : bi, lds, recs);
}
i64 k_argmax_mapped(cge_ctx *c, const double *v, i64 n, const i32 *map, double *val) {
    if (n <= 0) { if (val) *val = -1.0; return -1; }
    c->mp_recs.ensure(MP_NWG);
    MaxRec *recs = c->mp_recs.p;
    const int nwg = (int)std::max<i64>(1, std::min<i64>((n + 255) / 256, 256));
    hipLaunchKernelGGL(argmax_kernel, dim3(nwg), dim3(256), 768 * sizeof(double), c->stream, v, n, map, recs);
    double bv;
    i64 bi, bj;
    best_of_recs(c, recs, nwg, &bv, &bi, &bj);
    if (val) *val = bv;
    return bj;
}
static const int FAR_NWG = 1024 > MP_NWG ? MP_NWG : 1024;
void k_farthest_enqueue(cge_ctx *c, const double *Xr, i64 n, i64 d, i64 src, const double *srow) {
    c->mp_recs.ensure(MP_NWG);
    MaxRec *recs = c->mp_recs.p;
    hipLaunchKernelGGL(farthest_kernel, dim3(FAR_NWG), dim3(256), 768 * sizeof(double), c->stream, Xr, n, d, src, srow, recs);
}
void k_farthest_collect(cge_ctx *c, double *best_val, i64 *best_i) {
    i64 bj;
    best_of_recs(c, c->mp_recs.p, FAR_NWG, best_val, best_i, &bj);
}

__global__ void pair_dist_kernel(const double *__restrict__ Xr, i64 d, const i32 *__restrict__ pi,
                                 const i32 *__restrict__ pj, i64 S, double den, double *__restrict__ out) {
    const i64 stride = (i64)gridDim.x * blockDim.x;
    for (i64 k = (i64)blockIdx.x * blockDim.x + threadIdx.x; k < S; k += stride) {
        const double *a = Xr + (i64)pi[k] * d, *b = Xr + (i64)pj[k] * d;
        double s = 0.0;
        if (pi[k] != pj[k]) {
            for (i64 q = 0; q < d; q++) {
                const double df = __dsub_rn(a[q], b[q]);
                s = __dadd_rn(s, __dmul_rn(df, df));
            }
            s = sqrt(s);
        }
        out[k] = s / den;
    }
}
__global__ void pair_local_idx_kernel(const i32 *__restrict__ pi, const i32 *__restrict__ pj, i64 S, const i32 *__restrict__ glob2loc,
                                      i32 *__restrict__ idx) {
    const i64 k = (i64)blockIdx.x * blockDim.x + threadIdx.x;
    if (k >= S) return;
    idx[2 * k] = glob2loc[pi[k]];
    idx[2 * k + 1] = glob2loc[pj[k]];
}
__global__ void pair_dist_rows_kernel(const double *__restrict__ B, i64 d, const i32 *__restrict__ pi, const i32 *__restrict__ pj,
                                      i64 S, double den, double *__restrict__ out) {
    const i64 stride = (i64)gridDim.x * blockDim.x;
    for (i64 k = (i64)blockIdx.x * blockDim.x + threadIdx.x; k < S; k += stride) {
        const double *a = B + (2 * k) * d, *b = a + d;
        double s = 0.0;
        if (pi[k] != pj[k]) {
            for (i64 q = 0; q < d; q++) {
                const double df = __dsub_rn(a[q], b[q]);
                s = __dadd_rn(s, __dmul_rn(df, df));
            }
            s = sqrt(s);
        }
        out[k] = s / den;
    }
}
// ... 87 lines not shown
```

### cge.jl_amd/csrc/kernels_lm.hip

```cpp
#include "common.hpp"
#include <type_traits>
#include "mfma_tile.hpp"

#define WAVE 64

template <int CTRL>
__device__ __forceinline__ double dpp_move(double v) {
    const long long b = __double_as_longlong(v);
    const int lo = __builtin_amdgcn_update_dpp(0, (int)(unsigned)b, CTRL, 0xf, 0xf, false);
    const int hi = __builtin_amdgcn_update_dpp(0, (int)(unsigned)(b >> 32), CTRL, 0xf, 0xf, false);
    return __longlong_as_double(((long long)hi << 32) | (unsigned)lo);
}
__device__ __forceinline__ double lane_value(double v, int lane) {
    const long long b = __double_as_longlong(v);
    const int lo = __builtin_amdgcn_readlane((int)(unsigned)b, lane);
    const int hi = __builtin_amdgcn_readlane((int)(unsigned)(b >> 32), lane);
    return __longlong_as_double(((long long)hi << 32) | (unsigned)lo);
}
__device__ __forceinline__ double wave_allsum(double v) {
    v += dpp_move<0xB1>(v);
    v += dpp_move<0x4E>(v);
    v += dpp_move<0x141>(v);
    v += dpp_move<0x140>(v);
    return ((lane_value(v, 0) + lane_value(v, 16)) + lane_value(v, 32)) + lane_value(v, 48);
// ... 160 lines not shown
                const double *row = src + (node[r] < 0 ? 0 : node[r]) * d;
                const bool in = node[r] >= 0;
                if ((d & 1) == 0 && k + 1 < d) {
                    const double2 t = *reinterpret_cast<const double2 *>(row + k);
                    v0[r] = in ? t.x : m0;
                    v1[r] = in ? t.y : m1;
                } else {
                    v0[r] = (in && k < d) ? row[k] : m0;
                    v1[r] = (in && k + 1 < d) ? row[k + 1] : m1;
                }
            }
#pragma unroll
            for (int r = 0; r < R; r++) {
                const i64 p = p0 + r;
                if (p >= npos) continue;
                const double a = v0[r] - m0, b = v1[r] - m1;
                unsigned short h[2], l[2];
                const double vv[2] = {a, b};
#pragma unroll
                for (int q = 0; q < 2; q++) {
                    const float f = (float)vv[q], af = fabsf(f);
                    if (flag) {
                        if (!(af < 1.2676506e30f) || (af != 0.0f && af < 7.8886091e-31f)) bad = true;
                        if (af >= 9.094947e-13f) big = true;
                    }
                    unsigned u = __float_as_uint(f);
                    u += 0x7FFFu + ((u >> 16) & 1u);
                    h[q] = (unsigned short)(u >> 16);
                    unsigned w = __float_as_uint(f - __uint_as_float((unsigned)h[q] << 16));
                    w += 0x7FFFu + ((w >> 16) & 1u);
                    l[q] = (unsigned short)(w >> 16);
                }
                *reinterpret_cast<unsigned *>(planes + p * KP + k) = (unsigned)h[0] | ((unsigned)h[1] << 16);
                *reinterpret_cast<unsigned *>(planes + ld * KP + p * KP + k) = (unsigned)l[0] | ((unsigned)l[1] << 16);
                sq[r] += a * a + b * b;
            }
        }
#pragma unroll
        for (int r = 0; r < R; r++) {
            const double s = wave_allsum(sq[r]);
            if (lane == 0 && p0 + r < npos) rnorm[p0 + r] = s;
        }
    }
    if (flag) {
        const unsigned long long mb = __ballot(bad), mg = __ballot(big);
        const int need = (mb ? 1 : 0) | (mg ? 2 : 0);
        if (lane == 0 && need && (__hip_atomic_load(flag, __ATOMIC_RELAXED, __HIP_MEMORY_SCOPE_AGENT) & need) != need) atomicOr(flag, need);
    }
}
void k_gather_centre_fm(cge_ctx *c, const double *src_rowmajor, const i32 *idx, const double *mean, double *dst,
                        double *rnorm, i64 npos, i64 d, i64 ld, i64 dpad, float *dst32, unsigned short *planes, i64 KP,
                        int *flag) {
    const bool planes_only = planes && !dst && !dst32 && npos > 0;
    if (dst) HIP_CHECK(hipMemsetAsync(dst, 0, sizeof(double) * (size_t)(ld * dpad), c->stream));
    if (planes_only) {
        for (int q = 0; q < 2; q++)
            HIP_CHECK(hipMemsetAsync(planes + (size_t)q * ld * KP + (size_t)npos * KP, 0, sizeof(unsigned short) * (size_t)((ld - npos) * KP), c->stream));
    } else if (planes)
        HIP_CHECK(hipMemsetAsync(planes, 0, sizeof(unsigned short) * (size_t)(2 * ld * KP), c->stream));
    if (dst32) HIP_CHECK(hipMemsetAsync(dst32, 0, sizeof(float) * (size_t)(ld * dpad), c->stream));
    HIP_CHECK(hipMemsetAsync(rnorm, 0, sizeof(double) * (size_t)ld, c->stream));
    if (planes_only) {
        const unsigned nb = (unsigned)std::min<i64>((npos + 15) / 16, 16384);
        hipLaunchKernelGGL(gather_planes_kernel, dim3(nb), dim3(256), 0, c->stream, src_rowmajor, idx, mean, npos, d, ld, planes, KP,
                           flag, rnorm);
        return;
    }
    dim3 grid((unsigned)((npos + 31) / 32));
    hipLaunchKernelGGL(gather_centre_fm_kernel, grid, dim3(32, 8), 0, c->stream, src_rowmajor, idx, mean, dst, npos, d,
                       ld, dst32, planes, KP, flag, rnorm);
}

__device__ __forceinline__ uint64_t mix64(uint64_t x) {
    x ^= x >> 30; x *= 0xbf58476d1ce4e5b9ULL;
    x ^= x >> 27; x *= 0x94d049bb133111ebULL;
    x ^= x >> 31;
    return x;
}
__global__ void row_hash_kernel(const double *__restrict__ Xrow, uint64_t *__restrict__ hash, i64 n, i64 d) {
    i64 row = ((i64)blockIdx.x * blockDim.x + threadIdx.x) / WAVE;
    int lane = threadIdx.x & (WAVE - 1);
    if (row >= n) return;
    const uint64_t *p = reinterpret_cast<const uint64_t *>(Xrow + row * d);
    uint64_t h = 0;
    for (i64 k = lane; k < d; k += WAVE) h += mix64(p[k] ^ (0x9e3779b97f4a7c15ULL * (uint64_t)(k + 1)));
    for (int off = 32; off > 0; off >>= 1) h += __shfl_down(h, off);
    if (lane == 0) hash[row] = mix64(h);
}
void k_row_hash(cge_ctx *c, const double *Xrow, uint64_t *hash, i64 n, i64 d) {
    i64 threads = n * WAVE;
    hipLaunchKernelGGL(row_hash_kernel, dim3((unsigned)((threads + 255) / 256)), dim3(256), 0, c->stream, Xrow, hash,
                       n, d);
}
__global__ void count_distinct_kernel(const uint64_t *__restrict__ hash, i64 n, unsigned long long *__restrict__ table, i64 mask,
                                      unsigned long long *__restrict__ count) {
    const i64 stride = (i64)gridDim.x * blockDim.x;
    unsigned long long mine = 0;
    for (i64 i = (i64)blockIdx.x * blockDim.x + threadIdx.x; i < n; i += stride) {
        unsigned long long key = hash[i];
        if (key == ~0ULL) key = 0x5bd1e995ULL;
        i64 slot = (i64)(mix64(key) & (uint64_t)mask);
        for (;;) {
            const unsigned long long old = atomicCAS(&table[slot], ~0ULL, key);
            if (old == ~0ULL) { mine++; break; }
            if (old == key) break;
            slot = (slot + 1) & mask;
        }
    }
    if (mine) atomicAdd(count, mine);
}
i64 k_count_distinct(cge_ctx *c, const uint64_t *hash, i64 n) {
    i64 tsize = 1024;
    while (tsize < 2 * n) tsize <<= 1;
    c->uniq_table.ensure((size_t)tsize + 1);
    HIP_CHECK(hipMemsetAsync(c->uniq_table.p, 0xFF, sizeof(unsigned long long) * tsize, c->stream));
    HIP_CHECK(hipMemsetAsync(c->uniq_table.p + tsize, 0, sizeof(unsigned long long), c->stream));
    hipLaunchKernelGGL(count_distinct_kernel, dim3(grid_for(n, 256, 1024)), dim3(256), 0, c->stream, hash, n, c->uniq_table.p, tsize - 1,
                       c->uniq_table.p + tsize);
    unsigned long long cnt = 0;
    HIP_CHECK(hipMemcpyAsync(&cnt, c->uniq_table.p + tsize, sizeof(cnt), hipMemcpyDeviceToHost, c->stream));
    HIP_CHECK(hipStreamSynchronize(c->stream));
    return (i64)cnt;
}

#define MAXSLOT 16

template <int NS>
__global__ __launch_bounds__(256) void group_mean_partial_kernel(const double *__restrict__ Xr,
                                                                 const double *__restrict__ vw,
                                                                 const i32 *__restrict__ rows,
                                                                 const i32 *__restrict__ chunk_beg,
                                                                 const i32 *__restrict__ chunk_end, i64 d,
                                                                 double *__restrict__ part ) {
    __shared__ double red[4][WAVE * 4 + 1];
    const int wave = threadIdx.x >> 6, lane = threadIdx.x & 63;
    const i64 ch = blockIdx.x;
    const i32 beg = chunk_beg[ch], end = chunk_end[ch];
    double acc[MAXSLOT];
#pragma unroll
    for (int s = 0; s < MAXSLOT; s++) acc[s] = 0.0;
    double wsum = 0.0;
    constexpr int RF = NS <= 4 ? 4 : 1;
    i32 j = beg + wave;
    for (; j + 4 * (RF - 1) < end; j += 4 * RF) {
        double xv[RF][NS], w[RF];
#pragma unroll
        for (int q = 0; q < RF; q++) {
            const i64 v = rows[j + 4 * q];
            w[q] = vw[v];
            const double *x = Xr + v * d;
#pragma unroll
            for (int s = 0; s < NS; s++) {
                const i64 col = lane + 64 * s;
                xv[q][s] = (col < d) ? x[col] : 0.0;
            }
        }
#pragma unroll
        for (int q = 0; q < RF; q++) {
            wsum += w[q];
#pragma unroll
            for (int s = 0; s < NS; s++) acc[s] += xv[q][s] * w[q];
        }
    }
    for (; j < end; j += 4) {
        const i64 v = rows[j];
        const double w = vw[v];
        wsum += w;
        const double *x = Xr + v * d;
#pragma unroll
        for (int s = 0; s < NS; s++) {
            const i64 col = lane + 64 * s;
            if (col < d) acc[s] += x[col] * w;
        }
    }
// ... 1305 lines not shown
            const unsigned long long below = (i == 0) ? 0ULL : (~0ULL >> (64 - i));
            const i64 cl = nlow + __popcll(ml & below) + el, ch = nhigh + __popcll(mh & below) + eh;
            if (cl < ch) { al |= 1ULL << i; el++; } else eh++;
        }
        if (valid) side[o + j] = (isl || (ise && ((al >> lane) & 1ULL))) ? 1 : 2;
        nlow += __popcll(ml) + el;
        nhigh += __popcll(mh) + eh;
        }
    }
    if (lane == 0 && nlow_out) nlow_out[t] = (i32)nlow;
}
void k_cut_sides(cge_ctx *c, const double *z, const double *zs, const i32 *task_row_off, i64 n_tasks, int use_median,
                 unsigned char *side, i32 *nlow_out, int *tie_tasks) {
    ScopedKernelTimer t(c, "cut_sides");
    hipLaunchKernelGGL(cut_sides_kernel, dim3((unsigned)n_tasks), dim3(256), 0, c->stream, z, zs, task_row_off, use_median, side, nlow_out,
                       tie_tasks);
}

__global__ void rss_side_kernel(const double *__restrict__ z, const i32 *__restrict__ row_task, i64 n_rows,
                                const double *__restrict__ params, unsigned char *__restrict__ state,
                                unsigned char *__restrict__ side) {
    const i64 j = (i64)blockIdx.x * blockDim.x + threadIdx.x;
    if (j >= n_rows) return;
    const double *p = params + 4 * (i64)row_task[j];
    unsigned char st = state[j], sd = 0;
    if (st == 0) {
        const int absorb = (int)p[1], mode = (int)p[3];
        const double zj = z[j];
        if (absorb != 0 && ((zj < p[0]) ? 1 : 2) == absorb) {
            st = (unsigned char)absorb;
            state[j] = st;
        }
        if (st == 0 && mode != 0) sd = (mode == 2) ? 1 : ((zj < p[2]) ? 1 : 2);
    }
    side[j] = sd;
}
void k_rss_side(cge_ctx *c, const double *z, const i32 *row_task, i64 n_rows, const double *params,
                unsigned char *state, unsigned char *side) {
    hipLaunchKernelGGL(rss_side_kernel, dim3((unsigned)((n_rows + 255) / 256)), dim3(256), 0, c->stream, z, row_task,
                       n_rows, params, state, side);
}

struct WordSegs {
    unsigned *dst[CGE_WORD_SEGS];
    const unsigned *src[CGE_WORD_SEGS];
    long long end[CGE_WORD_SEGS];
};
__global__ void copy_words_kernel(WordSegs s, int n) {
    const long long total = s.end[n - 1];
    for (long long i = (long long)blockIdx.x * blockDim.x + threadIdx.x; i < total; i += (long long)gridDim.x * blockDim.x) {
        long long beg = 0;
#pragma unroll
        for (int q = 0; q < CGE_WORD_SEGS; q++) {
            if (q < n && i >= beg && i < s.end[q]) s.dst[q][i - beg] = s.src[q][i - beg];
            if (q < n) beg = s.end[q];
        }
    }
}
void k_copy_words(cge_ctx *c, int nseg, void *const *dst, const void *const *src, const i64 *words) {
    if (nseg <= 0) return;
    if (nseg > CGE_WORD_SEGS) CGE_THROW(CGE_E_ARG, "k_copy_words: %d segments", nseg);
    WordSegs s;
    long long tot = 0;
    for (int q = 0; q < CGE_WORD_SEGS; q++) {
        s.dst[q] = q < nseg ? (unsigned *)dst[q] : nullptr;
        s.src[q] = q < nseg ? (const unsigned *)src[q] : nullptr;
        if (q < nseg) tot += words[q];
        s.end[q] = tot;
    }
    if (tot == 0) return;
    const unsigned nb = (unsigned)std::min<long long>((tot + 255) / 256, 1024);
    hipLaunchKernelGGL(copy_words_kernel, dim3(nb), dim3(256), 0, c->stream, s, nseg);
}

__device__ __forceinline__ double fast_rcp(double q) {
    double r = __builtin_amdgcn_rcp(q);
    r = fma(fma(-q, r, 1.0), r, r);
    return r;
}
constexpr int STURM_B = 8;
__device__ __forceinline__ double sturm_top_eigenvalue(const double *diag, const double *off2, int d, double glo, double ghi,
                                                       double tiny, int lane) {
    const double rtiny = fast_rcp(tiny);
    double lo = glo, hi = ghi + tiny;
    for (int it = 0; it < 64; it++) {
        const double x = lo + (hi - lo) * ((double)(lane + 1) / 65.0);
        int cnt = 0;
        double q = diag[0] - x;
        if (q < 0) cnt++;
        auto step = [&](double dg, double o2) {
            const double r = fast_rcp(q);
            q = dg - x - o2 * (q == 0.0 ? rtiny : r);
            if (q < 0) cnt++;
        };
        int i = 1;
        for (; i + STURM_B <= d; i += STURM_B) {
            double dg[STURM_B], o2[STURM_B];
#pragma unroll
            for (int u = 0; u < STURM_B; u++) { dg[u] = diag[i + u]; o2[u] = off2[i + u]; }
#pragma unroll
            for (int u = 0; u < STURM_B; u++) step(dg[u], o2[u]);
        }
        for (; i < d; i++) step(diag[i], off2[i]);
        const unsigned long long mask = __ballot(cnt >= d);
        double nlo, nhi;
        if (mask == 0ULL) {
            nlo = __shfl(x, 63);
            nhi = hi;
        } else {
            const int f = __ffsll((long long)mask) - 1;
            nhi = __shfl(x, f);
            nlo = (f > 0) ? __shfl(x, f - 1) : lo;
        }
        if (!(nhi > nlo) || (nlo == lo && nhi == hi)) break;
        lo = fmax(lo, nlo);
        hi = fmin(hi, nhi);
    }
    return 0.5 * (lo + hi);
}
template <int N>
__device__ __forceinline__ void fmac_bcast(double &acc, double bc, double a) {
    asm volatile("v_fmac_f64_dpp %0, %1, %2 row_newbcast:%3 row_mask:0xf bank_mask:0xf" : "+v"(acc) : "v"(bc), "v"(a), "n"(N));
}
template <int N>
__device__ __forceinline__ void fnmac_bcast(double &acc, double bc, double a) {
// ... 1344 lines not shown
```

### cge.jl_amd/csrc/kernels_sort.hip

```cpp
#include <cstring>

#include "common.hpp"

#include <rocprim/rocprim.hpp>

using RadixOnly = rocprim::radix_sort_config<rocprim::default_config, rocprim::default_config, rocprim::default_config, 4096>;
static int sort_radix_mask() { return 1; }
template <class K, class V>
static hipError_t radix_pairs(void *tmp, size_t &bytes, const K *ki, K *ko, const V *vi, V *vo, size_t n, int b0, int b1,
                              hipStream_t st) {
    if (sort_radix_mask() & (sizeof(K) > 4 ? 2 : 1))
        return rocprim::radix_sort_pairs<RadixOnly>(tmp, bytes, ki, ko, vi, vo, n, b0, b1, st);
    return rocprim::radix_sort_pairs(tmp, bytes, ki, ko, vi, vo, n, b0, b1, st);
}
__global__ void iota_local_kernel(const i32 *__restrict__ row_task, const i32 *__restrict__ task_row_off, i64 R,
                                  i32 *__restrict__ idx) {
    const i64 j = (i64)blockIdx.x * blockDim.x + threadIdx.x;
    if (j < R) idx[j] = (i32)(j - task_row_off[row_task[j]]);
}
__global__ void sorted_gather_kernel(const i32 *__restrict__ rows, const i32 *__restrict__ row_task,
                                     const i32 *__restrict__ task_row_off, const i32 *__restrict__ perm, i64 R,
                                     i32 *__restrict__ srows) {
    const i64 j = (i64)blockIdx.x * blockDim.x + threadIdx.x;
    if (j < R) srows[j] = rows[task_row_off[row_task[j]] + perm[j]];
// ... 328 lines not shown
        __syncthreads();
        for (int k = tid; k < B; k += 256) run[k] += (wcnt[0][k] + wcnt[1][k]) + (wcnt[2][k] + wcnt[3][k]);
        __syncthreads();
    }
}
void k_sort_children(cge_ctx *c, const unsigned char *keys, const i32 *rows, const i32 *task_row_off, const i32 *chunk_beg,
                     const i32 *chunk_end, const i32 *task_chunk_off, i64 n_chunks, i64 R, i64 T, int key_bits, i32 *out) {
    ScopedKernelTimer tm(c, "children_sort");
    if (R <= 0 || T <= 0 || n_chunks <= 0) return;
    const int B = 1 << key_bits;
    if (B > CP_MAXB) CGE_THROW(CGE_E_ASSERT, "children lists: %d buckets", B);
    c->sort_cnt.ensure((size_t)n_chunks * B);
    hipLaunchKernelGGL(child_hist_kernel, dim3((unsigned)n_chunks), dim3(256), 0, c->stream, keys, chunk_beg, chunk_end, B, c->sort_cnt.p);
    hipLaunchKernelGGL(child_offsets_kernel, dim3((unsigned)T), dim3(CP_MAXB), 0, c->stream, task_chunk_off, task_row_off, B,
                       c->sort_cnt.p);
    hipLaunchKernelGGL(child_scatter_kernel, dim3((unsigned)n_chunks), dim3(256), 0, c->stream, keys, rows, chunk_beg, chunk_end, B,
                       c->sort_cnt.p, out);
}

__global__ __launch_bounds__(256) void assign_groups_kernel(const i32 *__restrict__ arena, const i32 *__restrict__ goff,
                                                            const i32 *__restrict__ glen, i32 *__restrict__ v2l) {
    const i64 g = blockIdx.x;
    const i64 o = goff[g], k = glen[g];
    for (i64 q = threadIdx.x; q < k; q += 256) v2l[arena[o + q]] = (i32)g;
}
__global__ void count_unassigned_kernel(const i32 *__restrict__ v2l, i64 n, i32 *__restrict__ cnt) {
    const i64 i = (i64)blockIdx.x * blockDim.x + threadIdx.x;
    if (i < n && v2l[i] < 0) atomicAdd(cnt, 1);
}
__global__ void iota_kernel(i32 *__restrict__ x, i64 n) {
    const i64 i = (i64)blockIdx.x * blockDim.x + threadIdx.x;
    if (i < n) x[i] = (i32)i;
}
i64 k_groups_to_index(cge_ctx *c, const i32 *arena, const i32 *goff, const i32 *glen, i64 N, i64 n, i32 *v2l, i32 *mem) {
    hipStream_t st = c->stream;
    HIP_CHECK(hipMemsetAsync(v2l, 0xFF, sizeof(i32) * n, st));
    hipLaunchKernelGGL(assign_groups_kernel, dim3((unsigned)N), dim3(256), 0, st, arena, goff, glen, v2l);
    c->sort_cnt.ensure(1);
    HIP_CHECK(hipMemsetAsync(c->sort_cnt.p, 0, sizeof(i32), st));
    const unsigned nb = (unsigned)((n + 255) / 256);
    hipLaunchKernelGGL(count_unassigned_kernel, dim3(nb), dim3(256), 0, st, v2l, n, c->sort_cnt.p);
    c->sort_idx.ensure(n);
    c->sort_keys32.ensure(n);
    hipLaunchKernelGGL(iota_kernel, dim3(nb), dim3(256), 0, st, c->sort_idx.p, n);
    int bits = 1;
    while (((i64)1 << bits) < N) bits++;
    size_t bytes = 0;
    HIP_CHECK(radix_pairs(nullptr, bytes, (const unsigned *)v2l, (unsigned *)c->sort_keys32.p, c->sort_idx.p, mem,
                                        (size_t)n, 0, bits, st));
    c->sort_tmp.ensure(bytes);
    HIP_CHECK(radix_pairs(c->sort_tmp.p, bytes, (const unsigned *)v2l, (unsigned *)c->sort_keys32.p,
                                        c->sort_idx.p, mem, (size_t)n, 0, bits, st));
    i32 bad = 0;
    HIP_CHECK(hipMemcpyAsync(&bad, c->sort_cnt.p, sizeof(i32), hipMemcpyDeviceToHost, st));
    HIP_CHECK(hipStreamSynchronize(st));
    return bad;
}

__global__ void scatter_i32_kernel(const i32 *__restrict__ src, const i32 *__restrict__ idx, i64 cnt, i32 add, i32 *__restrict__ dst) {
    const i64 i = (i64)blockIdx.x * blockDim.x + threadIdx.x;
    if (i < cnt) dst[idx[i]] = src[i] + add;
}
__global__ void add_i32_kernel(const i32 *__restrict__ src, i64 n, i32 add, i32 *__restrict__ dst) {
    const i64 i = (i64)blockIdx.x * blockDim.x + threadIdx.x;
    if (i < n) dst[i] = src[i] + add;
}
void k_scatter_i32(cge_ctx *c, const i32 *src, const i32 *idx, i64 cnt, i32 add, i32 *dst) {
    if (cnt > 0) hipLaunchKernelGGL(scatter_i32_kernel, dim3((unsigned)((cnt + 255) / 256)), dim3(256), 0, c->stream, src, idx, cnt, add, dst);
}
void k_add_i32(cge_ctx *c, const i32 *src, i64 n, i32 add, i32 *dst) {
    if (n > 0) hipLaunchKernelGGL(add_i32_kernel, dim3((unsigned)((n + 255) / 256)), dim3(256), 0, c->stream, src, n, add, dst);
}

__global__ void gather_means_kernel(const double *__restrict__ arena, const i64 *__restrict__ off, i64 d,
                                    double *__restrict__ mean) {
    const i64 t = blockIdx.x;
    const double *src = arena + off[t];
    for (i64 q = threadIdx.x; q < d; q += blockDim.x) mean[t * d + q] = src[q];
}
__global__ void copy_segments_kernel(const i32 *__restrict__ src, const i64 *__restrict__ seg, i32 *__restrict__ dst) {
    const i64 so = seg[3 * blockIdx.x], dof = seg[3 * blockIdx.x + 1], len = seg[3 * blockIdx.x + 2];
    for (i64 j = threadIdx.x; j < len; j += blockDim.x) dst[dof + j] = src[so + j];
}
void k_copy_segments(cge_ctx *c, const i32 *src, const i64 *seg, i64 nseg, i32 *dst) {
    if (nseg > 0) hipLaunchKernelGGL(copy_segments_kernel, dim3((unsigned)nseg), dim3(256), 0, c->stream, src, seg, dst);
}
__global__ void gather_means_slots_kernel(const double *__restrict__ arena, const i64 *__restrict__ off,
                                          const i64 *__restrict__ slot, i64 d, i64 stride, i64 lead, double *__restrict__ dst) {
    const i64 t = blockIdx.x;
    const double *src = arena + off[t];
    double *out = dst + slot[t] * stride + lead;
    for (i64 q = threadIdx.x; q < d; q += blockDim.x) out[q] = src[q];
}
void k_gather_means_slots(cge_ctx *c, const double *arena, const i64 *off, const i64 *slot, i64 T, i64 d, i64 stride, i64 lead,
                          double *dst) {
    if (T > 0)
        hipLaunchKernelGGL(gather_means_slots_kernel, dim3((unsigned)T), dim3(128), 0, c->stream, arena, off, slot, d, stride, lead, dst);
}
void k_gather_means(cge_ctx *c, const double *arena, const i64 *off, i64 T, i64 d, double *mean) {
    hipLaunchKernelGGL(gather_means_kernel, dim3((unsigned)T), dim3(128), 0, c->stream, arena, off, d, mean);
}
```

### cge.jl_amd/csrc/landmarks_host.cpp

```cpp
#include <algorithm>
#include <atomic>
#include <cfloat>
#include <cmath>
#include <memory>

#include "common.hpp"

namespace {

struct PhaseAcc {
    cge_ctx *c;
    const char *name;
    double t0;
    PhaseAcc(cge_ctx *ctx, const char *n) : c(ctx), name(n), t0(now_ms()) {}
    ~PhaseAcc() { c->phases.ms[name] += now_ms() - t0; }
};

struct Group {
    i64 off = -1, len = 0;
    std::vector<i64> what;
    double value = 0.0;
    bool has_split = false;
    int rc = CGE_OK;
    i64 coff = -1, nlow = 0;
// ... 265 lines not shown
    nrm = std::sqrt(nrm);
    if (!(nrm > 0.0) || !std::isfinite(nrm)) {
        for (i64 i = 0; i < d; i++) y[i] = (i == 0) ? 1.0 : 0.0;
        nrm = 1.0;
    }
    i64 big = 0;
    for (i64 i = 0; i < d; i++) {
        vout[i] = y[i] / nrm;
        if (std::fabs(vout[i]) > std::fabs(vout[big])) big = i;
    }
    if (vout[big] < 0.0)
        for (i64 i = 0; i < d; i++) vout[i] = -vout[i];
}

namespace {

struct Batch {
    i64 T = 0, R = 0, NC = 0, max_len = 0;
    i32 *rows = nullptr, *row_task = nullptr;
    std::vector<i32> chunk_task, chunk_beg, chunk_end, chunk_order, task_chunk_off, task_row_off, task_off;
};
void batch_tables(Batch &B, const std::vector<i64> &lens) {
    const i64 CH = CGE_CHUNK_ROWS, T = (i64)lens.size();
    B.T = T;
    B.chunk_task.clear(); B.chunk_beg.clear(); B.chunk_end.clear();
    B.task_chunk_off.assign(T + 1, 0);
    B.task_row_off.assign(T + 1, 0);
    i64 pos = 0;
    B.max_len = 0;
    for (i64 t = 0; t < T; t++) {
        B.task_row_off[t] = (i32)pos;
        B.task_chunk_off[t] = (i32)B.chunk_task.size();
        const i64 k = lens[t];
        B.max_len = std::max(B.max_len, k);
        for (i64 s = 0; s < k; s += CH) {
            B.chunk_task.push_back((i32)t);
            B.chunk_beg.push_back((i32)(pos + s));
            B.chunk_end.push_back((i32)(pos + std::min(k, s + CH)));
        }
        pos += k;
    }
    B.R = pos;
    B.task_row_off[T] = (i32)pos;
    B.task_chunk_off[T] = (i32)B.chunk_task.size();
    B.NC = (i64)B.chunk_task.size();
    const i64 NB = CH / 16 + 1;
    std::vector<i32> first(NB + 1, 0);
    auto bucket = [&](i64 ch) { return NB - 1 - (B.chunk_end[ch] - B.chunk_beg[ch] + 15) / 16; };
    for (i64 ch = 0; ch < B.NC; ch++) first[bucket(ch) + 1]++;
    for (i64 b = 0; b < NB; b++) first[b + 1] += first[b];
    B.chunk_order.resize(B.NC);
    for (i64 ch = 0; ch < B.NC; ch++) B.chunk_order[first[bucket(ch)]++] = (i32)ch;
}
struct WordGatherer {
    cge_ctx *c;
    std::vector<void *> ddst;
    std::vector<const void *> dsrc;
    std::vector<i64> words, offs;
    i64 tot = 0;
    explicit WordGatherer(cge_ctx *c_) : c(c_) {}
    template <class T>
    size_t add(const T *device, i64 count) {
        static_assert(sizeof(T) % 4 == 0, "4-byte words");
        dsrc.push_back(device);
        const i64 w = count * (i64)(sizeof(T) / 4);
        words.push_back(w);
        offs.push_back(tot);
        tot += w + (w & 1);
        return words.size() - 1;
    }
    void fetch() {
        fetch_async();
        wait();
    }
    void wait() { HIP_CHECK(hipEventSynchronize(c->copy_done)); }
    void fetch_async() {
        c->pin_res.ensure((size_t)std::max<i64>(tot, 1));
        c->dev_res.ensure((size_t)std::max<i64>(tot, 1));
        ddst.resize(dsrc.size());
        for (size_t q = 0; q < dsrc.size(); q++) ddst[q] = c->dev_res.p + offs[q];
        for (size_t q0 = 0; q0 < dsrc.size(); q0 += CGE_WORD_SEGS) {
            const int n = (int)std::min<size_t>(CGE_WORD_SEGS, dsrc.size() - q0);
            k_copy_words(c, n, &ddst[q0], &dsrc[q0], &words[q0]);
        }
        if (tot > 0)
            HIP_CHECK(hipMemcpyAsync(c->pin_res.p, c->dev_res.p, sizeof(i32) * (size_t)tot, hipMemcpyDeviceToHost, c->stream));
        HIP_CHECK(hipEventRecord(c->copy_done, c->stream));
    }
    template <class T>
    const T *get(size_t item) const { return reinterpret_cast<const T *>(c->pin_res.p + offs[item]); }
};
void upload_tables(cge_ctx *c, const Batch &B, WordPacker &pk) {
    const i64 d = c->d;
    c->ls_rows.ensure(B.R); c->ls_row_task.ensure(B.R); c->ls_ct.ensure(B.NC); c->ls_cb.ensure(B.NC);
    c->ls_ce.ensure(B.NC); c->ls_co.ensure(B.NC); c->ls_tco.ensure(B.T + 1); c->sp_tro.ensure(B.T + 1);
    c->ls_part.ensure((size_t)B.NC * std::max(d * d, 2 * (2 * d + 1)));
    c->ls_side.ensure(B.R);
    c->ls_sums.ensure((size_t)B.T * 2 * (2 * d + 1));
    pk.add(c->ls_ct.p, B.chunk_task.data(), B.NC);
    pk.add(c->ls_cb.p, B.chunk_beg.data(), B.NC);
    pk.add(c->ls_ce.p, B.chunk_end.data(), B.NC);
    pk.add(c->ls_co.p, B.chunk_order.data(), B.NC);
    pk.add(c->ls_tco.p, B.task_chunk_off.data(), B.T + 1);
    pk.add(c->sp_tro.p, B.task_row_off.data(), B.T + 1);
}
void build_batch(cge_ctx *c, Group *const *groups, i64 T, Batch &B) {
    std::vector<i64> lens(T);
    B.task_off.resize(T);
    for (i64 t = 0; t < T; t++) {
        lens[t] = groups[t]->len;
        B.task_off[t] = (i32)groups[t]->off;
    }
    batch_tables(B, lens);
}
void upload_batch(cge_ctx *c, const Batch &B, const i64 *moff = nullptr) {
    WordPacker pk(c);
    upload_tables(c, B, pk);
    c->ls_toff.ensure(B.T);
    pk.add(c->ls_toff.p, B.task_off.data(), B.T);
    if (moff) {
        c->ls_moff.ensure(B.T);
        pk.add(c->ls_moff.p, moff, B.T);
    }
    pk.flush();
    k_gather_rows(c, c->lm_arena.p, c->ls_toff.p, c->sp_tro.p, c->ls_ct.p, c->ls_cb.p, c->ls_ce.p, B.NC, c->ls_rows.p,
                  c->ls_row_task.p);
}
void build_batch_host(cge_ctx *c, Group *const *groups, i64 T, Batch &B) {
    std::vector<i64> lens(T);
    for (i64 t = 0; t < T; t++) lens[t] = (i64)groups[t]->what.size();
    batch_tables(B, lens);
    c->pin_hb_rows.ensure(B.R);
    c->pin_hb_row_task.ensure(B.R);
    B.rows = c->pin_hb_rows.p;
    B.row_task = c->pin_hb_row_task.p;
    parallel_for(c, T, [&](i64 t) {
        const Group *g = groups[t];
        const i64 o = B.task_row_off[t], k = (i64)g->what.size();
        for (i64 j = 0; j < k; j++) {
            B.rows[o + j] = (i32)(g->what[j] - 1);
            B.row_task[o + j] = (i32)t;
        }
    });
}
// ... 199 lines not shown
}
void rule_rss_sorted_collect(cge_ctx *c, SplitBatch &S) {
    const i64 T = S.B.T, d = c->d;
    S.wg->wait();
    const i32 *status = S.wg->get<i32>(S.i_status), *meta = S.wg->get<i32>(S.i_meta);
    const double *vals = S.wg->get<double>(S.i_vals);
    std::memcpy(S.nlow.data(), S.wg->get<i32>(S.i_nlow), sizeof(i32) * T);
    for (i64 t = 0; t < T; t++) {
        Group *g = S.groups[t];
        if (status[t] == 2) { g->rc = CGE_E_HOMOGENEOUS; S.done[t] = 1; continue; }
        if (status[t] == 1 || meta[2 * t + 1] != 0) { S.done[t] = 0; continue; }
        S.vlow[t] = vals[2 * t];
        S.vhigh[t] = vals[2 * t + 1];
        g->cmean_off = S.mbase + 2 * t * d;
        g->rc = CGE_OK;
        S.done[t] = 1;
    }
}

void rule_rss2_enqueue(cge_ctx *c, SplitBatch &S) {
    const Batch &B = S.B;
    const i64 T = B.T, R = B.R, d = c->d;
    hipStream_t st = c->stream;
    c->sp_srows.ensure(R); c->sp_zs.ensure(R); c->sp_perm.ensure(R); c->sp_status.ensure(T);
    c->sp_meta.ensure(2 * T); c->sp_vals.ensure(2 * T);
    k_segmented_sort_z(c, c->ls_z.p, c->ls_rows.p, c->ls_row_task.p, c->sp_tro.p, R, T, c->sp_zs.p, c->sp_perm.p,
                       c->sp_srows.p, c->sp_status.p, B.max_len);
    HIP_CHECK(hipMemcpyAsync(c->lm_arena.p + S.base, c->sp_srows.p, sizeof(i32) * R, hipMemcpyDeviceToDevice, st));
    c->r2_rows = R;
    k_rss2_walk(c, c->Xr.p, lm_vw(c), c->sp_srows.p, c->sp_tro.p, T, d, c->sp_meta.p, c->sp_vals.p, c->lm_means.p + S.mbase);
    S.wg.reset(new WordGatherer(c));
    S.i_meta = S.wg->add(c->sp_meta.p, 2 * T); S.i_vals = S.wg->add(c->sp_vals.p, 2 * T);
    S.wg->fetch_async();
}
void rule_rss2_collect(cge_ctx *c, SplitBatch &S) {
    const i64 T = S.B.T, d = c->d;
    S.wg->wait();
    const i32 *meta = S.wg->get<i32>(S.i_meta);
    const double *vals = S.wg->get<double>(S.i_vals);
    for (i64 t = 0; t < T; t++) {
        Group *g = S.groups[t];
        S.nlow[t] = meta[2 * t] + 1;
        S.vlow[t] = vals[2 * t];
        S.vhigh[t] = vals[2 * t + 1];
        g->cmean_off = S.mbase + 2 * t * d;
        g->rc = CGE_OK;
        S.done[t] = 1;
    }
}

void rule_cut_enqueue(cge_ctx *c, SplitBatch &S, bool use_median) {
    const Batch &B = S.B;
    const i64 T = B.T, R = B.R, d = c->d;
    hipStream_t st = c->stream;
    if (use_median) {
        c->sp_srows.ensure(R); c->sp_zs.ensure(R); c->sp_perm.ensure(R); c->sp_status.ensure(T);
        k_segmented_sort_z(c, c->ls_z.p, c->ls_rows.p, c->ls_row_task.p, c->sp_tro.p, R, T, c->sp_zs.p, c->sp_perm.p,
                           c->sp_srows.p, c->sp_status.p, B.max_len);
    }
    c->ls_nlow.ensure(T);
    k_cut_sides(c, c->ls_z.p, use_median ? c->sp_zs.p : nullptr, c->sp_tro.p, T, use_median ? 1 : 0, c->ls_side.p, c->ls_nlow.p,
                c->cut_ties.p);
    c->pin_res.ensure((size_t)T);
    HIP_CHECK(hipMemcpyAsync(c->pin_res.p, c->ls_nlow.p, sizeof(i32) * T, hipMemcpyDeviceToHost, st));
    k_group_side_sums(c, c->Xr.p, lm_vw(c), c->ls_rows.p, c->ls_side.p, c->ls_cb.p, c->ls_ce.p, B.NC, c->ls_tco.p, B.T, d,
                      c->ls_part.p, c->ls_sums.p);
    c->sp_vals.ensure(2 * T);
    k_side_values_means(c, c->ls_sums.p, T, d, c->sp_vals.p, c->lm_means.p + S.mbase);
    c->pin_sums.ensure((size_t)2 * T);
    HIP_CHECK(hipMemcpyAsync(c->pin_sums.p, c->sp_vals.p, sizeof(double) * 2 * T, hipMemcpyDeviceToHost, st));
    HIP_CHECK(hipEventRecord(c->copy_done, st));
    k_sort_children(c, c->ls_side.p, c->ls_rows.p, c->sp_tro.p, c->ls_cb.p, c->ls_ce.p, c->ls_tco.p, B.NC, R, T, 2, c->lm_arena.p + S.base);
}
void rule_cut_collect(cge_ctx *c, SplitBatch &S) {
    const i64 T = S.B.T, d = c->d;
    HIP_CHECK(hipEventSynchronize(c->copy_done));
    const double *vals = c->pin_sums.p;
    std::memcpy(S.nlow.data(), c->pin_res.p, sizeof(i32) * T);
    for (i64 t = 0; t < T; t++) {
        Group *g = S.groups[t];
        S.vlow[t] = vals[2 * t];
        S.vhigh[t] = vals[2 * t + 1];
        g->cmean_off = S.mbase + 2 * t * d;
        g->rc = CGE_OK;
        S.done[t] = 1;
    }
}

void rss_generic_tasks(cge_ctx *c, SplitBatch &out, const std::vector<i64> &todo) {
    const Batch &B = out.B;
    Group *const *groups = out.groups;
    const i64 d = c->d, width = 2 * (2 * d + 1), base = out.base;
    hipStream_t st = c->stream;
    std::vector<Group *> fg;
    std::vector<std::vector<i32>> rows(todo.size());
    std::vector<double> fz;
    std::vector<i64> zoff(todo.size() + 1, 0);
    for (size_t q = 0; q < todo.size(); q++) zoff[q + 1] = zoff[q] + groups[todo[q]]->len;
    fz.resize(zoff.back());
    for (size_t q = 0; q < todo.size(); q++) {
        const i64 t = todo[q], o = B.task_row_off[t], k = groups[t]->len;
        rows[q].resize(k);
        HIP_CHECK(hipMemcpyAsync(rows[q].data(), c->ls_rows.p + o, sizeof(i32) * k, hipMemcpyDeviceToHost, st));
        HIP_CHECK(hipMemcpyAsync(fz.data() + zoff[q], c->ls_z.p + o, sizeof(double) * k, hipMemcpyDeviceToHost, st));
    }
    HIP_CHECK(hipStreamSynchronize(st));
    for (size_t q = 0; q < todo.size(); q++) {
        Group *g = groups[todo[q]];
        g->what.resize(rows[q].size());
        for (size_t j = 0; j < rows[q].size(); j++) g->what[j] = (i64)rows[q][j] + 1;
        fg.push_back(g);
    }
    Batch FB;
    build_batch_host(c, fg.data(), (i64)fg.size(), FB);
    upload_batch_host(c, FB);
    c->ls_z.ensure(FB.R);
    HIP_CHECK(hipMemcpyAsync(c->ls_z.p, fz.data(), sizeof(double) * FB.R, hipMemcpyHostToDevice, st));
    std::vector<RssState> rs;
    rule_rss_batched(c, FB, fg.data(), fz.data(), rs);
    std::vector<unsigned char> side(FB.R, 0);
    for (size_t q = 0; q < fg.size(); q++) {
        if (rs[q].rc != CGE_OK) continue;
        unsigned char *sd = &side[FB.task_row_off[q]];
        for (i64 j : rs[q].low) sd[j] = 1;
        for (i64 j : rs[q].high) sd[j] = 2;
    }
    const double *sums = side_sums(c, FB, side);
    for (size_t q = 0; q < fg.size(); q++) {
        const i64 t = todo[q];
        Group *g = fg[q];
        g->rc = rs[q].rc;
// ... 652 lines not shown
    const i64 nbig = (i64)locals.size(), W = c->has_coll ? c->coll.world : 1;
    if (c->rows_sharded) return forced_rowsharded(c, locals, forced, method, pool);
    if (W > 1 && c->opt_shard_forced && forced >= 2) {
        GroupGather G;
        G.shape(total, nbig, nbig * forced, 3, c->d);
        if (cge_exchange_fits(c, (size_t)(G.words() + W))) return forced_over_ranks(c, locals, cl_off, forced, method, pool, G);
    }
    forced_local(c, locals, forced, method, pool);
}

void merge_into_global(cge_ctx *c, const i64 *cl_off, const std::vector<i64> &order, i64 forced, const StagedClusters &sc,
                       const std::vector<Local> &locals, GroupPool &pool, Heap &H) {
    PhaseAcc pa(c, "lm_merge");
    size_t li = 0;
    for (i64 cidx : order) {
        if (cl_off[cidx + 1] - cl_off[cidx] > forced) {
            for (Group *g : locals[li++].out) H.put(g);
            continue;
        }
        for (i64 t = cl_off[cidx]; t < cl_off[cidx + 1]; t++) {
            pool.emplace_back();
            Group *g = &pool.back();
            g->off = sc.a_off[cidx] >= 0 ? sc.a_off[cidx] + (t - cl_off[cidx]) : -1;
            g->len = 1;
            g->value = DBL_EPSILON;
            g->owner = sc.owner[cidx];
            H.put(g);
        }
    }
}

void final_index(cge_ctx *c, const Heap &H, std::vector<i64> &group_ids, bool want_index) {
    PhaseAcc pfin(c, "lm_final");
    const i64 n = c->n, NG = (i64)H.len(), nrows = lm_rows(c);
    const bool RS = c->rows_sharded;
    const int me = RS ? c->coll.rank : 0;
    hipStream_t st = c->stream;
    c->pin_small.ensure((size_t)2 * NG + 2);
    i32 *goff = c->pin_small.p, *glen = goff + NG;
    c->h_mem_off.assign(NG + 1, 0);
    c->h_gl_off.assign(NG + 1, 0);
    c->lm_owner.assign(NG, 0);
    for (i64 g = 0; g < NG; g++) {
        const Group *G = H.at(g + 1);
        const bool mine = !RS || G->owner == me;
        goff[g] = mine ? (i32)G->off : 0;
        glen[g] = mine ? (i32)G->len : 0;
        c->h_mem_off[g + 1] = c->h_mem_off[g] + glen[g];
        c->h_gl_off[g + 1] = c->h_gl_off[g] + (i32)G->len;
        c->lm_owner[g] = G->owner;
    }
    DevBuf<i32> &v2l_rows = RS ? c->v2l_loc : c->v2l;
    c->lm_goff.ensure(NG); c->lm_glen.ensure(NG); c->v2l.ensure(n); v2l_rows.ensure(nrows); c->lm_mem.ensure(nrows); c->lm_memoff.ensure(NG + 1);
    HIP_CHECK(hipMemcpyAsync(c->lm_goff.p, goff, sizeof(i32) * NG, hipMemcpyHostToDevice, st));
    HIP_CHECK(hipMemcpyAsync(c->lm_glen.p, glen, sizeof(i32) * NG, hipMemcpyHostToDevice, st));
    HIP_CHECK(hipMemcpyAsync(c->lm_memoff.p, c->h_mem_off.data(), sizeof(i32) * (NG + 1), hipMemcpyHostToDevice, st));
    const i64 unassigned = k_groups_to_index(c, c->lm_arena.p, c->lm_goff.p, c->lm_glen.p, NG, nrows, v2l_rows.p, c->lm_mem.p);
    bool cover_bad = unassigned != 0 || c->h_mem_off[NG] != nrows || c->h_gl_off[NG] != n;
    if (RS) {
        const i64 words = (n + 1) / 2;
        DevBuf<i32> &tmp = c->sort_idx2;
        tmp.ensure(2 * words);
        HIP_CHECK(hipMemsetAsync(tmp.p, 0, sizeof(i32) * 2 * words, st));
        k_scatter_i32(c, v2l_rows.p, c->loc2glob.p, nrows, 1, tmp.p);
        cge_allreduce_dev(c, reinterpret_cast<double *>(tmp.p), words, 2);
        k_add_i32(c, tmp.p, n, -1, c->v2l.p);
        std::vector<double> verdict(1, cover_bad ? 1.0 : 0.0);
        exchange_group_words(c, verdict);
        cover_bad = verdict[0] != 0.0;
    }
    if (cover_bad)
        CGE_THROW(CGE_E_ASSERT, "AssertionError: all(>=(0), group_ids) [%lld rows without a group, %lld of %lld rows in the groups here, %lld of %lld over all ranks]",
                  (long long)unassigned, (long long)c->h_mem_off[NG], (long long)nrows, (long long)c->h_gl_off[NG], (long long)n);
    c->lm_index_on_device = want_index;
    c->h_mem.clear();
    if (want_index) {
        HIP_CHECK(hipStreamSynchronize(st));
        group_ids.clear();
        return;
    }
    c->h_v2l0.resize(n);
    HIP_CHECK(hipMemcpyAsync(c->h_v2l0.data(), c->v2l.p, sizeof(i32) * n, hipMemcpyDeviceToHost, st));
    HIP_CHECK(hipStreamSynchronize(st));
    group_ids.resize(n);
    parallel_for(c, 64, [&](i64 part) {
        for (i64 i = n * part / 64; i < n * (part + 1) / 64; i++) group_ids[i] = c->h_v2l0[i];
    });
}

}

void host_group_stats_test(cge_ctx *c, const i32 *ids, const i32 *task_row_off, i64 T, const unsigned char *side, const double *mean_in,
                           double *mean, double *sw, double *cov, double *vec, double *z, double *sums) {
    const i64 d = c->d, nrows = lm_rows(c);
    if (!c->Xr.p || d <= 0 || c->Xr.n < (size_t)(nrows * d) || !c->vw.p || (i64)c->h_vw.size() != c->n)
        CGE_THROW(CGE_E_ARG, "group_stats_test: embedding / vertex weights are not resident");
    if (c->rows_sharded) CGE_THROW(CGE_E_ARG, "group_stats_test: not with option shard_rows");
    if (side && d > 512) CGE_THROW(CGE_E_ARG, "group_stats_test: side sums need d <= 512");
    if (task_row_off[0] != 0) CGE_THROW(CGE_E_ARG, "group_stats_test: task_row_off[0] != 0");
    for (i64 t = 0; t < T; t++)
        if (task_row_off[t + 1] <= task_row_off[t]) CGE_THROW(CGE_E_ARG, "group_stats_test: empty group %lld", (long long)t);
    const i64 R = task_row_off[T];
    std::vector<char> seen((size_t)nrows, 0);
    for (i64 j = 0; j < R; j++) {
        if (ids[j] < 0 || ids[j] >= nrows) CGE_THROW(CGE_E_ARG, "group_stats_test: id %d outside the %lld resident rows", ids[j], (long long)nrows);
        if (seen[ids[j]]) CGE_THROW(CGE_E_ARG, "group_stats_test: id %d in two groups", ids[j]);
        seen[ids[j]] = 1;
        if (side && side[j] > 2) CGE_THROW(CGE_E_ARG, "group_stats_test: side %d of row %lld", (int)side[j], (long long)j);
    }
// ... 138 lines not shown
```

### cge.jl_amd/csrc/score_host.cpp

```cpp
#include "common.hpp"

struct EdgeShare {
    i64 rank, world;
    i64 lo(i64 cnt) const { return cnt * rank / world; }
    i64 hi(i64 cnt) const { return cnt * (rank + 1) / world; }
};
static EdgeShare edge_share(const cge_ctx *c) {
    const bool split = c->has_coll && !c->edges_sharded;
    return {split ? c->coll.rank : 0, split ? c->coll.world : 1};
}
struct RowBlock { i64 per, r0, r1; };
static RowBlock wedge_row_block(const cge_ctx *c, i64 N) {
    if (!c->has_coll) return {N, 0, N};
    const i64 per = (N + c->coll.world - 1) / c->coll.world, r0 = std::min<i64>(N, per * c->coll.rank);
    return {per, r0, std::min<i64>(N, r0 + per)};
}


static i64 count_distinct_rows(const double *X, i64 d, std::vector<i64> &rows) {
    const size_t bytes = sizeof(double) * d;
    std::sort(rows.begin(), rows.end(), [&](i64 a, i64 b) { return memcmp(X + a * d, X + b * d, bytes) < 0; });
    i64 uniq = rows.empty() ? 0 : 1;
    for (size_t t = 1; t < rows.size(); t++)
        if (memcmp(X + rows[t - 1] * d, X + rows[t] * d, bytes) != 0) uniq++;
// ... 55 lines not shown
    return std::min(land, uniq);
}

static void scatter_vectC_resident(cge_ctx *c, i64 C, int directed, double *vectC) {
    const i64 vlen = directed ? C * C : packed_len(C);
    const EdgeShare mine = edge_share(c);
    bool done = false;
    if (k_edge_scatter_blocked_applies(c, C) && (c->blocked_ready || k_build_blocked_edges(c))) {
        k_edge_scatter_blocked(c, mine.lo(c->be_nchunks), mine.hi(c->be_nchunks), C, directed, vectC);
        done = true;
    } else if (C > 1 && C <= 16384 && (c->blocked_ready || (k_blocked_edges_possible(c) && k_build_blocked_edges(c)))) {
        DevBuf<i64> &cnt = c->wed_cnt;
        cnt.ensure(1);
        double *dense = vectC;
        if (!directed) { c->cc_dense.ensure((size_t)C * C); dense = c->cc_dense.p; }
        if (k_wedge_scatter_blocked(c, c->comm.p, C, mine.lo(c->be_nchunks), mine.hi(c->be_nchunks), directed, dense, cnt.p, "edge_scatter")) {
            if (!directed) k_pack_upper(c, dense, C, vectC);
            done = true;
        }
    }
    if (!done) {
        HIP_CHECK(hipMemsetAsync(vectC, 0, sizeof(double) * vlen, c->stream));
        k_edge_scatter(c, c->src.p, c->dst.p, c->unit_weights ? nullptr : c->w.p, mine.lo(c->m), mine.hi(c->m), nullptr, c->comm.p, 1, C,
                       directed, nullptr, vectC);
    }
    if (c->has_coll) cge_allreduce_dev(c, vectC, vlen, 0);
}

static void scatter_wedges(cge_ctx *c, int directed) {
    const i64 N = c->N;
    hipStream_t st = c->stream;
    const RowBlock blk = wedge_row_block(c, N);
    const i64 Npad = c->has_coll ? blk.per * c->coll.world : N;
    c->wedges.ensure((size_t)Npad * N);
    c->wedges_block_only = false;
    DevBuf<i64> &cnt = c->wed_cnt;
    cnt.ensure(1);
    const EdgeShare mine = edge_share(c);
    bool tiled = (c->blocked_ready || (k_blocked_edges_possible(c) && k_build_blocked_edges(c))) &&
                 k_wedge_scatter_blocked(c, c->v2l.p, N, mine.lo(c->be_nchunks), mine.hi(c->be_nchunks), directed, c->wedges.p, cnt.p);
    if (!tiled) {
        HIP_CHECK(hipMemsetAsync(c->wedges.p, 0, sizeof(double) * N * N, st));
        k_edge_scatter(c, c->src.p, c->dst.p, c->unit_weights ? nullptr : c->w.p, mine.lo(c->m), mine.hi(c->m), c->v2l.p, c->comm.p, N,
                       c->n_comm_max, directed, c->wedges.p, nullptr);
    }
    if (c->has_coll) {
        if (Npad > N) HIP_CHECK(hipMemsetAsync(c->wedges.p + (size_t)N * N, 0, sizeof(double) * (size_t)(Npad - N) * N, st));
        c->wedges_block_only = c->opt_wedges_rs && cge_reduce_scatter_dev(c, c->wedges.p, blk.per * N);
        if (!c->wedges_block_only) cge_allreduce_dev(c, c->wedges.p, N * N, 0);
        k_compact_count(c, c->wedges.p, N, directed, cnt.p, blk.r0, blk.r1);
        cge_allreduce_dev(c, reinterpret_cast<double *>(cnt.p), 1, 2);
    } else if (!tiled)
        k_compact_count(c, c->wedges.p, N, directed, cnt.p);
    HIP_CHECK(hipMemcpyAsync(&c->n_ledges, cnt.p, sizeof(i64), hipMemcpyDeviceToHost, st));
    HIP_CHECK(hipStreamSynchronize(st));
    c->wedges_ready = true;
}

static void lm_clamp(cge_ctx *c, LandmarkRun &R) {
    check_resident(c, "landmarks");
    if (R.method < 0 || R.method > 3) CGE_THROW(CGE_E_ARG, "unknown split method %d", R.method);
    R.t0 = now_ms();
    R.land = clamp_to_unique_rows(c, R.land, &c->lm_truncated);
    c->phases.ms["lm_unique"] = now_ms() - R.t0;
}

static void lm_split(cge_ctx *c, LandmarkRun &R) {
    std::vector<i64> gid;
    host_runsplit(c, R.cl_flat, R.cl_off, R.ncl, R.land, R.forced, R.method, gid, true);
    HIP_CHECK(hipStreamSynchronize(c->stream));
    c->phases.ms["landmarks"] = now_ms() - R.t0;
    c->N = (i64)c->h_mem_off.size() - 1;
    c->h_v2l.clear();
}

static void lm_aggregate(cge_ctx *c, LandmarkRun &R) {
    R.t0 = now_ms();
    const i64 N = c->N, d = c->d;
    c->lemb.ensure((size_t)N * d);
    c->lweight.ensure(N); c->dii.ensure(N); c->lcomm.ensure(N);
    {
        ScopedKernelTimer tm(c, "landmark_aggregate");
        k_landmark_aggregate(c, c->Xr.p, lm_vw(c), lm_comm(c), c->lm_memoff.p, c->lm_mem.p, N, d, c->lemb.p, c->lweight.p, c->dii.p,
                             c->lcomm.p);
    }
    if (c->rows_sharded) {
        DevBuf<double> &X = c->samp_xchg;
        const i64 words = N * (d + 3);
        X.ensure(words);
        k_pack_landmarks(c, c->lemb.p, c->lweight.p, c->dii.p, c->lcomm.p, N, d, X.p, 0);
        cge_allreduce_dev(c, X.p, words, 2);
        k_pack_landmarks(c, c->lemb.p, c->lweight.p, c->dii.p, c->lcomm.p, N, d, X.p, 1);
    }
    HIP_CHECK(hipStreamSynchronize(c->stream));
    c->phases.ms["aggregate"] = now_ms() - R.t0;
}

static void lm_scatter(cge_ctx *c, LandmarkRun &R) {
    R.t0 = now_ms();
    const i64 C = c->n_comm_max;
    c->vectC.ensure(R.directed ? C * C : packed_len(C));
    scatter_vectC_resident(c, C, R.directed, c->vectC.p);
    c->lm_directed = R.directed;
    c->wedges_ready = false;
    c->n_ledges = -1;
    if (R.need_wedges) scatter_wedges(c, R.directed);
    HIP_CHECK(hipStreamSynchronize(c->stream));
    c->phases.ms["scatter"] = now_ms() - R.t0;
// ... 142 lines not shown
}

static OrigView resident_orig_view(cge_ctx *c, const double *lweight) {
    OrigView ov;
    ov.n = c->n; ov.m = c->m; ov.Xr = c->Xr.p; ov.vw = c->vw.p; ov.v2l = c->v2l.p; ov.lweight = lweight;
    ov.src = c->src.p; ov.dst = c->dst.p; ov.h_w = c->h_w.empty() ? nullptr : c->h_w.data();
    return ov;
}

static void sweep_resident(cge_ctx *c, const ScoreGraph &G, const OrigView *ov, int directed, int split, const SampleSet &smp,
                           double out[7], int *out_len, cge_trace *trace, SweepHandoff *defer = nullptr) {
    host_wgcl_sweep(c, G, ov, c->src.p, c->dst.p, c->h_w.empty() ? nullptr : c->h_w.data(), c->m, directed, split, smp, out, out_len,
                    trace, defer);
}

struct Score {
    bool landmarks, reuse_samples;
    bool samples_early;
    ScoreGraph G;
    OrigView ov;
    std::vector<i32> lcomm_host;
};

static void score_graph_landmarks(cge_ctx *c, const cge_score_args *a, Score &S) {
    LandmarkRun R = score_landmark_run(c, a);
    lm_clamp(c, R);
    if (S.samples_early) {
        c->smp.reset();
        make_samples(c, a->seed, a->auc_samples, a->directed, false, c->smp, true);
    }
    lm_split(c, R);
    lm_aggregate(c, R);
    lm_scatter(c, R);
    const i64 N = c->N;
    S.G = score_graph(N, c->d, c->n_comm_max, c->lemb.p, c->dii.p, c->lweight.p, c->lcomm.p, c->vectC.p);
    if (!a->directed) return;
    c->s_degin.ensure(N); c->s_degout.ensure(N); c->s_star.ensure(N);
    if (c->wedges_block_only) {
        const RowBlock blk = wedge_row_block(c, N);
        DevBuf<double> &X = c->samp_xchg;
        X.ensure(3 * N);
        k_wedge_degrees_block(c, c->wedges.p, N, blk.r0, blk.r1, X.p);
        cge_allreduce_dev(c, X.p, 3 * N, 0);
        k_degrees_unpack(c, X.p, N, c->s_degout.p, c->s_degin.p, c->s_star.p);
    } else
        k_wedge_degrees(c, c->wedges.p, N, c->s_degout.p, c->s_degin.p, c->s_star.p);
}

static void score_landmark_view(cge_ctx *c, Score &S) {
    const double t0 = now_ms();
    const i64 N = c->N;
    S.ov = resident_orig_view(c, c->lweight.p);
    S.lcomm_host.resize(N);
    HIP_CHECK(hipMemcpyAsync(S.lcomm_host.data(), c->lcomm.p, sizeof(i32) * N, hipMemcpyDeviceToHost, c->stream));
    HIP_CHECK(hipStreamSynchronize(c->stream));
    S.ov.hi = host_diameter_landmarks(c, c->lemb.p, c->lweight.p, S.lcomm_host, c->n_comm_max, N);
    S.ov.h_lcomm = S.lcomm_host.data();
    c->phases.ms["diameter"] = now_ms() - t0;
}

static void score_graph_exact(cge_ctx *c, const cge_score_args *a, Score &S) {
    if (c->edges_sharded)
        CGE_THROW(CGE_E_ARG, "score: exact mode reads the whole edge list on every rank; the resident one is sharded (option shard_ingest)");
    if (c->rows_sharded)
        CGE_THROW(CGE_E_ARG, "score: exact mode reads every embedding row on every rank; the resident rows are sharded (option shard_rows)");
    const i64 N = c->n, C = c->n_comm_max;
    DevBuf<double> &zeros = c->sw_zeros;
    zeros.ensure(N);
    HIP_CHECK(hipMemsetAsync(zeros.p, 0, sizeof(double) * N, c->stream));
    c->vectC.ensure(a->directed ? C * C : packed_len(C));
    scatter_vectC_resident(c, C, a->directed, c->vectC.p);
    S.G = score_graph(N, c->d, C, c->Xr.p, zeros.p, c->vw.p, c->comm.p, c->vectC.p);
    if (a->directed) edge_degrees(c, c->src.p, c->dst.p, c->unit_weights ? nullptr : c->w.p, c->m, N, c->s_star);
}

static void score_samples(cge_ctx *c, const cge_score_args *a, const Score &S) {
    const double t0 = now_ms();
    if (S.reuse_samples) {
    } else if (S.samples_early && c->samp_pending.on) k_draw_samples_finish(c);
    else {
        c->smp.reset();
        make_samples(c, a->seed, a->auc_samples, a->directed, a->directed && !S.landmarks, c->smp);
    }
    c->phases.ms["samples"] = now_ms() - t0;
}

void host_score(cge_ctx *c, const cge_score_args *a, double out[7], int *out_len, cge_trace *trace, SweepHandoff *defer,
                bool reuse_samples) {
    check_resident(c, "score");
    c->phases.ms.clear();
    Score S{a->land != -1, reuse_samples};
    S.samples_early = S.landmarks && !reuse_samples && samples_can_start_early(c, a->seed, false);
    struct DrainDraw {
        cge_ctx *c;
        ~DrainDraw() {
            if (c->samp_pending.on) (void)hipStreamSynchronize(c->stream);
            c->samp_pending.on = false;
        }
    } drain{c};
    if (S.landmarks) score_graph_landmarks(c, a, S);
    else score_graph_exact(c, a, S);
    if (a->directed && directed_guard(c, S.G, c->s_star, out, out_len)) return;
    if (S.landmarks) score_landmark_view(c, S);
    score_samples(c, a, S);
    const double t0 = now_ms();
    sweep_resident(c, S.G, S.landmarks ? &S.ov : nullptr, a->directed, a->split, c->smp, out, out_len, trace, defer);
    HIP_CHECK(hipStreamSynchronize(c->stream));
    c->phases.ms[defer && defer->deferred ? "sweep_setup" : "sweep"] = now_ms() - t0;
// ... 181 lines not shown
```

### cge.jl_amd/csrc/wgcl_host.cpp

```cpp
#include <algorithm>
#include <cmath>
#include <cstring>

#include "common.hpp"
#include "../../include/cge_hip_testing.h"

static inline uint64_t ctr_rand(uint64_t seed, uint64_t stream, uint64_t k, uint64_t attempt, uint64_t which) {
    return cge_ctr_rand(seed, stream, k, attempt, which);
}
static inline uint64_t bounded(uint64_t r, uint64_t range) { return cge_bounded(r, range); }

void host_pos_draw(i64 seed, i64 stream_id, i64 S, i64 m, i64 *pos_idx) {
    for (i64 k = 0; k < S; k++)
        pos_idx[k] = (i64)bounded(ctr_rand((uint64_t)seed, (uint64_t)stream_id, (uint64_t)k, 0, 0), (uint64_t)m) + 1;
}

void host_draw_samples(cge_ctx *c, i64 seed, i64 stream_id, i64 S, int directed, i64 *pos_idx, i64 *neg_i, i64 *neg_j) {
    const i64 n = c->n, m = c->m;
    if (m <= 0 || n < 2) CGE_THROW(CGE_E_ARG, "draw_samples: no resident graph");
    const uint64_t sd = (uint64_t)seed, st = (uint64_t)stream_id;
    host_pos_draw(seed, stream_id, S, m, pos_idx);
    if ((double)n * (double)(n - 1) <= 33554432.0) {
        std::vector<i32> hs(m), hd(m);
        HIP_CHECK(hipMemcpyAsync(hs.data(), c->src.p, sizeof(i32) * m, hipMemcpyDeviceToHost, c->stream));
// ... 378 lines not shown
        if (ring) HIP_CHECK(hipMemcpyAsync(hr, ring, sizeof(hr), hipMemcpyDeviceToHost, st));
        HIP_CHECK(hipStreamSynchronize(st));
        const i64 iters = hf[1];
        if (hf[0]) return iters;
        if (ring) {
            double flast;
            std::memcpy(&flast, &hr[(k - 1) % 3], sizeof(double));
            if (!(flast > AlphaBook::delta)) return iters;
        }
        if (iters > c->opt_fit_max_iters) CGE_THROW(CGE_E_ASSERT, "Chung-Lu fit did not converge at alpha=%g (%lld iterations; the reference's `while diff > delta` would not return)", alpha, (long long)iters);
        batch = std::max<i64>(4, std::min<i64>(batch, 32));
    }
}

static void fit_undirected(cge_ctx *c, i64 N, const double *w, i64 Tld, double alpha, bool upper, bool packed,
                           const cge_fit_fused *ff, const cge_fit_fused *ff_dev, FitForm &fit, AlphaSlot &sl) {
    hipStream_t st = c->stream;
    double *const GD = packed ? c->sw_PK.p : c->sw_GD.p, *const TT = c->fp_T.p;
    int *flags = c->sw_flags.p;
    if (!fit.persistent) HIP_CHECK(hipMemsetAsync(flags, 0, sizeof(int) * 4, st));
    sl.t0_par = fit.tpar;
    if (fit.persistent) {
        const int tnext = (fit.tpar + 1) % 3;
        if (k_fit_flow_enqueue(c, ff ? nullptr : GD, N, TT + (i64)fit.tpar * Tld, TT + (i64)tnext * Tld, Tld, w, 0.25,
                               AlphaBook::delta, (int *)(c->sw_scal.p + RES_FIT), ff, ff_dev)) {
            sl.fused = ff != nullptr;
            sl.fit_async = true;
            fit.tpar = tnext;
            return;
        }
        fit.persistent = false;
        if (ff) {
            k_pow_prepare(c, c->sw_D.p, N, upper);
            k_pow_matrix(c, c->sw_D.p, N, alpha, GD, upper);
        }
        HIP_CHECK(hipMemsetAsync(flags, 0, sizeof(int) * 4, st));
    }
    HIP_CHECK(hipMemsetAsync(c->sw_fring.p, 0, sizeof(unsigned long long) * 4, st));
    double *Tb2[2] = {TT + (i64)fit.tpar * Tld, TT + (i64)((fit.tpar + 1) % 3) * Tld};
    c->sweep_used_fp_P = true;
    sl.iters = fit_by_launches(c, fit.prev_iters, alpha, flags, c->sw_fring.p, [&](i64 k) {
        k_fit_sym_step(c, GD, Tb2[k & 1], Tb2[(k + 1) & 1], w, N, 0.25, AlphaBook::delta, (int)k, c->sw_fring.p, flags, flags + 1,
                       packed);
    });
    if (sl.iters & 1) fit.tpar = (fit.tpar + 1) % 3;
}

static void fit_directed(cge_ctx *c, const ScoreGraph &G, double alpha, FitForm &fit, AlphaSlot &sl) {
    hipStream_t st = c->stream;
    const i64 N = G.N;
    const double *GD = c->sw_GD.p;
    double *Tin = c->sw_T1.p, *Tout = c->sw_T2.p;
    int *flags = c->sw_flags.p;
    HIP_CHECK(hipMemsetAsync(flags, 0, sizeof(int) * 4, st));
    const double init[2] = {0.9, 1.0};
    HIP_CHECK(hipMemcpyAsync(c->sw_fitstate.p, init, sizeof(init), hipMemcpyHostToDevice, st));
    bool enqueued_only = false;
    if (fit.persistent_dir && k_fit_persistent_dir(c, GD, N, Tin, Tout, G.deg_in, G.deg_out, 0.9, 1.0, AlphaBook::delta,
                                                   &sl.iters, (int *)(c->sw_scal.p + RES_FIT), &enqueued_only)) {
        if (enqueued_only) sl.fit_async = true;
        else c->stat_fit_persistent++;
        return;
    }
    if (fit.persistent_dir) {
        fit.persistent_dir = false;
        HIP_CHECK(hipMemsetAsync(flags, 0, sizeof(int) * 4, st));
    }
    sl.iters = fit_by_launches(c, fit.prev_iters, alpha, flags, nullptr, [&](i64) {
        k_fit_symv_dir(c, GD, Tin, Tout, N, c->sw_S1.p, c->sw_S2.p, flags);
        k_fit_update_dir(c, Tin, Tout, c->sw_S1.p, c->sw_S2.p, G.deg_in, G.deg_out, N, AlphaBook::delta, flags, flags + 1,
                         c->sw_fitstate.p);
    });
}

static void local_score_tallies(cge_ctx *c, const double *Ta, const double *Tb, i64 N, int directed, const OrigView *orig,
                                const i32 *old2new, const DevSamples &ds, i64 s0, i64 s1, double alpha, bool packed) {
    double *part = c->sw_scal.p + RES_AUC;
    if (!orig) {
        k_auc_exact(c, packed ? c->sw_PK.p : c->sw_GD.p, Ta, Tb, N, ds.pi.p + s0, ds.pj.p + s0, ds.ni.p + s0, ds.nj.p + s0,
                    ds.wts.p + s0, s1 - s0, nullptr, part, packed);
        return;
    }
    if (old2new) {
        c->sw_rl_T.ensure((size_t)2 * N);
        k_permute_rows(c, Ta, old2new, N, 1, c->sw_rl_T.p);
        Ta = c->sw_rl_T.p;
        if (directed) {
            k_permute_rows(c, Tb, old2new, N, 1, c->sw_rl_T.p + N);
            Tb = c->sw_rl_T.p + N;
        } else
            Tb = Ta;
    }
    k_auc_landmark(c, Ta, Tb, orig->v2l, orig->vw, orig->lweight, ds.pi.p + s0, ds.pj.p + s0, ds.ni.p + s0, ds.nj.p + s0,
                   ds.dpos.p + s0, ds.dneg.p + s0, ds.wts.p + s0, s1 - s0, alpha, nullptr, part);
}

static void divergence_and_copy_out(cge_ctx *c, const ScoreGraph &G, int directed, int split, const double *Ta,
                                    const double *Tb, bool want_div, bool bvec_partials, bool arm, i64 Tld, int slot, bool packed) {
    hipStream_t st = c->stream;
    const i64 N = G.N, C = G.C, vlen = directed ? C * C : packed_len(C);
    const double *GD = packed ? c->sw_PK.p : c->sw_GD.p;
    if (packed && want_div && !(c->bvec_blocks && !directed && !c->opt_test_bvec_plain))
        CGE_THROW(CGE_E_ASSERT, "packed exact sweep without the tile form of vect_B");
    const i32 *cm_off = c->sw_cm_off.p;
    double *scal = c->sw_scal.p, *vectB = c->sw_vectB.p, *host_out = c->pin_scal.p + RES_STRIDE * slot;
    if (want_div && (bvec_partials || c->bvec_blocks) && !directed && !c->opt_test_bvec_plain) {
        if (!bvec_partials) k_bvec_tiles(c, GD, Ta, Tb, cm_off, N, directed, packed);
        cge_chain_tail tail{};
        tail.host_out = host_out;
// ... 456 lines not shown
```

### include/cge_hip_testing.h

```cpp
#ifndef CGE_HIP_TESTING_H
#define CGE_HIP_TESTING_H
#include <stdint.h>
#ifdef __cplusplus
extern "C" {
#endif
int cge_host_eig_top(const double *A, int64_t d, double *v);
int cge_batch_pack_test(const int64_t *N, int64_t K, int cus, int32_t *group_of);
int cge_host_pos_draw(int64_t seed, int64_t stream_id, int64_t S, int64_t m, int64_t *pos_idx);
int cge_group_eig(void *ctx, const double *A, int64_t T, int64_t d, double *v);
int cge_group_stats_test(void *ctx, const int32_t *ids, const int32_t *task_row_off, int64_t T, const uint8_t *side, const double *mean_in,
                         double *mean, double *sw, double *cov, double *vec, double *z, double *sums);
int cge_group_cut_test(void *ctx, const int32_t *ids, const int32_t *task_row_off, int64_t T, int method, const double *z, int force_generic,
                       int32_t *rc, int32_t *nlow, int32_t *children, double *vlow, double *vhigh, double *cmeans, int32_t *route,
                       int32_t *ties);
int cge_diameter_bounds_test(void *ctx, const int64_t *v2l, int64_t N, const int64_t *lcomm, int64_t C, int pass, double *P,
                             int64_t *nref, int *pass_ran, double *ref_points, double *mean);
int cge_pow_test(void *ctx, const double *x, int64_t n, double alpha, int method, double *out);
#define CGE_VECT_B_GUARD 64
typedef struct cge_vect_b_problem {
    const double *GD, *Ta, *Tb;
    const int64_t *comm;
    int64_t N, C;
    const double *vC;
    double *vectB, *js_dev, *js_fused;
} cge_vect_b_problem;
int cge_vect_b_test(void *ctx, const cge_vect_b_problem *p, const cge_vect_b_problem *p2, int directed, int form, int landmarks,
                    int n_modes, int *form_ran);
int cge_packed_gd_test(void *ctx, const double *emb , const double *diag , int64_t N, int64_t d,
                       double alpha, int pow_method, double *lo_hi , double *GD );
int cge_rccl_selftest(void *ctx, double *host_inout, int64_t count, int op);
int cge_segment_sort_test(void *ctx, const double *z, const int32_t *task_row_off, int64_t T, double *zs_out, int32_t *perm_out);
int cge_wave_tree_test(void *ctx, const double *x, int64_t n_rows, double *out_ref, double *out_new);
int cge_set_test_option(void *ctx, const char *key, int64_t value);
int cge_resident_embedding_test(void *ctx, double *out, int64_t capacity_doubles, int64_t *rows, int64_t *d, int32_t *ids_out);
typedef struct cge_resident_graph {
    int64_t n, m, n_comm_max, n_comm16;
    int unit, have;
    int32_t *src, *dst, *comm;
    double *w, *vweight;
    uint16_t *comm16;
    int64_t cap_edges, cap_vertices, cap_comm16;
} cge_resident_graph;
int cge_resident_graph_test(void *ctx, cge_resident_graph *out);
#ifdef __cplusplus
}
#endif
#endif
```

Baseline: 11.87 billion.

## Route small host-device transfers through pinned memory via copy kernels directly

WordPacker now lets the copy kernel read uploaded words straight from pinned host memory when the total is small, skipping the staging hipMemcpyAsync and device table. It also gains a zero path so memsets can ride in the same launch. WordGatherer moves into the shared header and writes results straight into pinned host memory, dropping the device staging buffer and D2H copy. Several scattered hipMemcpyAsync, hipMemset and sync pairs across the fit, diameter and score code are replaced with these batched helpers. The intent is to cut per-transfer launch and copy-engine overhead. The trade-off is that kernels read or write over the host interconnect, which may be slower for larger payloads.

```diff
diff --git a/cge.jl_amd/api.py b/cge.jl_amd/api.py
--- a/cge.jl_amd/api.py
+++ b/cge.jl_amd/api.py
@@ -179,6 +179,15 @@
     if isinstance(method, str):
         return {"rss": 0, "rss2": 1, "size": 2, "diameter": 3}[method]
     return int(method)
+
+
+def word_layout(words):
+    words = _i64(words)
+    offs, tot, launches = np.empty(len(words), np.int64), C.c_int64(), C.c_int64()
+    rc = load_library().cge_word_layout_test(_p(words), C.c_int64(len(words)), _p(offs), C.byref(tot), C.byref(launches))
+    if rc != 0:
+        raise CGEError(rc, "cge_word_layout_test")
+    return offs, tot.value, launches.value
 
 
 def _p(a):
@@ -829,6 +838,19 @@
         self._check(self.L.cge_wave_tree_test(self.h, _p(x), C.c_int64(x.shape[0]), _p(a), _p(b)))
         return a, b
 
+    def word_exchange_test(self, words, host_in, item8=None, copied=None, zero=()):
+        words = _i64(words)
+        host_in = np.ascontiguousarray(host_in, dtype=np.uint32).reshape(-1, int(words.sum()))
+        i8 = np.ascontiguousarray(np.zeros(len(words)) if item8 is None else item8, dtype=np.uint8)
+        cp = np.ascontiguousarray(np.ones(len(words)) if copied is None else copied, dtype=np.uint8)
+        z = _i64(np.asarray(list(zero), dtype=np.int64).reshape(-1, 3))
+        zs, zb, zl = (np.ascontiguousarray(z[:, k]) for k in range(3))
+        dev, got = np.empty(host_in.shape[1], np.uint32), np.empty(host_in.shape, np.uint32)
+        self._check(self.L.cge_word_exchange_test(self.h, C.c_int64(len(words)), _p(words), _p(i8), _p(cp),
+                                                  C.c_int64(host_in.shape[0]), _p(host_in), C.c_int64(len(z)), _p(zs), _p(zb),
+                                                  _p(zl), _p(dev), _p(got)))
+        return dev, got
+
     def js(self, vC, vB, vI=None, internal=True):
         vC, vB = _f64(vC), _f64(vB)
         vi = None if vI is None or len(vI) == 0 else np.ascontiguousarray(vI, dtype=np.uint8)
@@ -881,7 +903,7 @@
         return out, nc.value, q.value, rounds.value
 
     _TEST_OPTIONS = ("fit_persistent_test_delay", "fit_persistent_test_timeout", "test_bvec_plain", "test_rss2_one_kernel",
-                     "exact_resident_limit")
+                     "exact_resident_limit", "word_direct_max")
 
     def set_option(self, key, value):
         if key in self._TEST_OPTIONS:
diff --git a/cge.jl_amd/csrc/capi.cpp b/cge.jl_amd/csrc/capi.cpp
--- a/cge.jl_amd/csrc/capi.cpp
+++ b/cge.jl_amd/csrc/capi.cpp
@@ -293,6 +293,7 @@
     if (!c || !key) return CGE_E_ARG;
     if (!strcmp(key, "test_bvec_plain")) { c->opt_test_bvec_plain = value != 0; return CGE_OK; }
     if (!strcmp(key, "test_rss2_one_kernel")) { c->opt_test_rss2_one_kernel = value != 0; return CGE_OK; }
+    if (!strcmp(key, "word_direct_max") && value >= 0) { c->word_direct_max = value; return CGE_OK; }
     if (!strcmp(key, "fit_persistent_test_delay") && value >= 0 && value <= 100000) { c->opt_fit_test_delay = (int)value; return CGE_OK; }
     if (!strcmp(key, "fit_persistent_test_timeout")) { c->opt_fit_test_timeout = value != 0; return CGE_OK; }
     if (!strcmp(key, "exact_resident_limit") && value >= 0) { c->opt_test_resident_limit = (double)value; return CGE_OK; }
@@ -517,6 +518,69 @@
     CGE_CATCH(c)
 }
 
+int cge_word_layout_test(const int64_t *words, int64_t n, int64_t *offs, int64_t *total, int64_t *launches) {
+    if (n < 0 || (n > 0 && (!words || !offs)) || !total || !launches) return CGE_E_ARG;
+    for (int64_t q = 0; q < n; q++)
+        if (words[q] < 0) return CGE_E_ARG;
+    static_assert(sizeof(i64) == sizeof(int64_t), "i64");
+    *total = word_layout((const i64 *)words, (size_t)n, (i64 *)offs);
+    *launches = word_launches((size_t)n);
+    return CGE_OK;
+}
+int cge_word_exchange_test(void *ctx, int64_t nseg, const int64_t *words, const uint8_t *item8, const uint8_t *copied, int64_t rounds,
+                           const uint32_t *host_in, int64_t nzero, const int64_t *zero_seg, const int64_t *zero_beg,
+                           const int64_t *zero_len, uint32_t *dev_out, uint32_t *gathered) {
+    cge_ctx *c = (cge_ctx *)ctx;
+    if (!c || nseg <= 0 || !words || !item8 || !copied || rounds <= 0 || !host_in || !dev_out || !gathered || nzero < 0) return CGE_E_ARG;
+    CGE_TRY_ON_DEVICE(c)
+    std::vector<i64> off(nseg), goff(nseg);
+    i64 W = 0, A = 0;
+    for (i64 q = 0; q < nseg; q++) {
+        if (words[q] < 0 || (item8[q] && (words[q] & 1))) CGE_THROW(CGE_E_ARG, "segment %lld: %lld words", (long long)q, (long long)words[q]);
+        off[q] = W; W += words[q];
+        goff[q] = A; A += words[q] + (words[q] & 1);
+    }
+    for (i64 z = 0; z < nzero; z++)
+        if (zero_seg[z] < 0 || zero_seg[z] >= nseg || zero_beg[z] < 0 || zero_len[z] < 0 || zero_beg[z] + zero_len[z] > words[zero_seg[z]])
+            CGE_THROW(CGE_E_ARG, "zero range %lld outside its segment", (long long)z);
+    DevBuf<unsigned> arena;
+    arena.ensure((size_t)A + 2);
+    HIP_CHECK(hipMemsetAsync(arena.p, 0xA5, sizeof(unsigned) * ((size_t)A + 2), c->stream));
+    HIP_CHECK(hipStreamSynchronize(c->stream));
+    HIP_CHECK(hipEventSynchronize(c->copy_done));
+    c->pin_res.ensure((size_t)std::max<i64>(rounds * A, 1));
+    std::vector<std::unique_ptr<WordGatherer>> wg;
+    for (i64 r = 0; r < rounds; r++) {
+        WordPacker pk(c);
+        for (i64 q = 0; q < nseg; q++) {
+            if (!copied[q]) continue;
+            const uint32_t *h = host_in + r * W + off[q];
+            if (item8[q]) pk.add((unsigned long long *)(arena.p + goff[q]), (const unsigned long long *)h, words[q] / 2);
+            else pk.add(arena.p + goff[q], (const unsigned *)h, words[q]);
+        }
+        for (i64 z = 0; z < nzero; z++) pk.zero(arena.p + goff[zero_seg[z]] + zero_beg[z], zero_len[z]);
+        pk.flush();
+        wg.emplace_back(new WordGatherer(c, r * A));
+        for (i64 q = 0; q < nseg; q++) {
+            if (item8[q]) wg.back()->add((const unsigned long long *)(arena.p + goff[q]), words[q] / 2);
+            else wg.back()->add(arena.p + goff[q], words[q]);
+        }
+        wg.back()->fetch_async();
+    }
+    wg.back()->wait();
+    for (i64 r = 0; r < rounds; r++)
+        for (i64 q = 0; q < nseg; q++)
+            if (words[q] > 0) std::memcpy(gathered + r * W + off[q], wg[r]->get<unsigned>((size_t)q), sizeof(unsigned) * words[q]);
+    std::vector<unsigned> host_arena((size_t)A + 2);
+    HIP_CHECK(hipMemcpy(host_arena.data(), arena.p, sizeof(unsigned) * ((size_t)A + 2), hipMemcpyDeviceToHost));
+    for (i64 q = 0; q < nseg; q++)
+        if (words[q] > 0) std::memcpy(dev_out + off[q], host_arena.data() + goff[q], sizeof(unsigned) * words[q]);
+    for (i64 q = 0; q < nseg; q++)
+        if ((words[q] & 1) && host_arena[goff[q] + words[q]] != 0xA5A5A5A5u) CGE_THROW(CGE_E_ASSERT, "word behind segment %lld was written", (long long)q);
+    if (host_arena[A] != 0xA5A5A5A5u || host_arena[A + 1] != 0xA5A5A5A5u) CGE_THROW(CGE_E_ASSERT, "words behind the arena were written");
+    CGE_CATCH(c)
+}
+
 int cge_resident_embedding_test(void *ctx, double *out, int64_t capacity_doubles, int64_t *rows, int64_t *d, int32_t *ids_out) {
     cge_ctx *c = (cge_ctx *)ctx;
     if (!c || !rows || !d) return CGE_E_ARG;
diff --git a/cge.jl_amd/csrc/common.hpp b/cge.jl_amd/csrc/common.hpp
--- a/cge.jl_amd/csrc/common.hpp
+++ b/cge.jl_amd/csrc/common.hpp
@@ -248,6 +248,12 @@
     DevBuf<i32> aidx;
     DevBuf<double> afac;
 };
+
+#define CGE_WORD_SEGS 8
+#ifndef CGE_WORD_DIRECT_MAX
+#define CGE_WORD_DIRECT_MAX ((i64)1 << 18)
+#endif
+#define CGE_WORD_ZERO_MAX ((i64)1 << 18)
 
 struct cge_ctx {
     int device = 0;
@@ -436,7 +442,8 @@
     i64 lm_means_used = 0;
     DevBuf<i64> ls_moff;
     PinBuf<i32> pin_tab[2], pin_res;
-    DevBuf<i32> dev_tab, dev_res;
+    DevBuf<i32> dev_tab;
+    i64 word_direct_max = CGE_WORD_DIRECT_MAX;
     hipEvent_t tab_ev[2] = {nullptr, nullptr};
     int tab_slot = 0;
     bool lm_index_on_device = false;
@@ -691,13 +698,14 @@
              i64 ldm, i64 n_land, i64 N, i64 dpad, const i32 *soff, double *P, int part = 0, int nparts = 1);
 void k_max_pair_tile_list(i64 ldn, int part, int nparts, const std::vector<double> &wg, double thr, std::vector<int2> &out);
 i64 k_pair_collect(cge_ctx *c, const double *Xs, const double *rns, i64 ld, i64 nrows, i64 dpad, const int2 *tiles, i64 t0, i64 t1,
-                   int tri, double thr, const i32 *ids, int2 *out, i64 cap);
+                   int tri, double thr, const i32 *ids, int2 *out, i64 cap, int2 *head = nullptr, i64 nhead = 0);
 void k_pair_list(cge_ctx *c, const double *Xs, const double *rns, i64 lds_rows, i64 npos, i64 dpad, const int2 *tiles,
                  i64 ntiles, double *best_val, i64 *best_i, i64 *best_j, std::vector<double> *wg_best = nullptr);
 i64 k_bound_select(cge_ctx *c, const double *Q, const i32 *lref, i64 N, i64 nref, double L, BoundRec *list, i64 cap,
-                   const i32 *ref_off = nullptr, const i32 *ref_mem = nullptr);
+                   const i32 *ref_off = nullptr, const i32 *ref_mem = nullptr, BoundRec *head = nullptr, i64 nhead = 0);
 void k_ref_dist2_fm(cge_ctx *c, const double *Ms_fm, i64 nref, i64 dpad, i64 ldm);
-i64 k_argmax_mapped(cge_ctx *c, const double *v, i64 n, const i32 *map, double *val = nullptr);
+i64 k_argmax_mapped(cge_ctx *c, const double *v, i64 n, const i32 *map, double *val = nullptr, const int *ride_dev = nullptr,
+                    int *ride_host = nullptr);
 void k_pair_local_idx(cge_ctx *c, const i32 *pi, const i32 *pj, i64 S, const i32 *glob2loc, i32 *idx);
 void k_pair_dist_rows(cge_ctx *c, const double *B, i64 d, const i32 *pi, const i32 *pj, i64 S, double den, double *out);
 void k_position_ids(cge_ctx *c, const i32 *pos2node, const i32 *loc2glob, i64 npos, i32 *ids);
@@ -724,8 +732,17 @@
 void k_permute_rows(cge_ctx *c, const double *src, const i32 *order, i64 n, i64 width, double *dst);
 void k_permute_i32(cge_ctx *c, const i32 *src, const i32 *order, i64 n, i32 *dst);
 void k_remap_i32(cge_ctx *c, i32 *idx, const i32 *map, i64 n);
-#define CGE_WORD_SEGS 8
 void k_copy_words(cge_ctx *c, int nseg, void *const *dst, const void *const *src, const i64 *words);
+void k_zero_words(cge_ctx *c, int nseg, void *const *dst, const i64 *words);
+inline i64 word_layout(const i64 *words, size_t n, i64 *offs) {
+    i64 pos = 0;
+    for (size_t q = 0; q < n; q++) {
+        offs[q] = pos;
+        pos += words[q] + (words[q] & 1);
+    }
+    return pos;
+}
+inline i64 word_launches(size_t n) { return (i64)((n + CGE_WORD_SEGS - 1) / CGE_WORD_SEGS); }
 struct WordPacker {
     cge_ctx *c;
     std::vector<void *> dst;
@@ -740,32 +757,108 @@
         src.push_back(host);
         words.push_back(count * (i64)(sizeof(T) / 4));
     }
+    template <class T>
+    void zero(T *device, i64 count) {
+        static_assert(sizeof(T) % 4 == 0, "4-byte words");
+        if (count <= 0) return;
+        dst.push_back(device);
+        src.push_back(nullptr);
+        words.push_back(count * (i64)(sizeof(T) / 4));
+    }
+    void zero_bytes(void *device, size_t bytes) {
+        if (bytes == 0) return;
+        if (bytes % 4 == 0 && (uintptr_t)device % 4 == 0 && (i64)(bytes / 4) <= CGE_WORD_ZERO_MAX) zero((unsigned *)device, (i64)(bytes / 4));
+        else HIP_CHECK(hipMemsetAsync(device, 0, bytes, c->stream));
+    }
     void flush() {
         if (dst.empty()) return;
-        i64 tot = 0;
-        for (i64 w : words) tot += w + (w & 1);
-        const int slot = c->tab_slot;
-        c->tab_slot ^= 1;
-        HIP_CHECK(hipEventSynchronize(c->tab_ev[slot]));
-        c->pin_tab[slot].ensure((size_t)tot);
-        c->dev_tab.ensure((size_t)tot);
-        i32 *h = c->pin_tab[slot].p;
-        std::vector<const void *> dsrc(dst.size());
-        i64 pos = 0;
-        for (size_t q = 0; q < dst.size(); q++) {
-            std::memcpy(h + pos, src[q], (size_t)words[q] * 4);
-            dsrc[q] = c->dev_tab.p + pos;
-            pos += words[q] + (words[q] & 1);
+        const size_t n = dst.size();
+        std::vector<i64> staged(n), offs(n);
+        for (size_t q = 0; q < n; q++) staged[q] = src[q] ? words[q] : 0;
+        const i64 tot = word_layout(staged.data(), n, offs.data());
+        std::vector<const void *> dsrc(n, nullptr);
+        int slot = -1;
+        bool direct = true;
+        if (tot > 0) {
+            slot = c->tab_slot;
+            c->tab_slot ^= 1;
+            HIP_CHECK(hipEventSynchronize(c->tab_ev[slot]));
+            c->pin_tab[slot].ensure((size_t)tot);
+            i32 *h = c->pin_tab[slot].p;
+            direct = tot <= c->word_direct_max;
+            const i32 *base = h;
+            if (!direct) {
+                c->dev_tab.ensure((size_t)tot);
+                base = c->dev_tab.p;
+            }
+            for (size_t q = 0; q < n; q++)
+                if (src[q]) {
+                    std::memcpy(h + offs[q], src[q], (size_t)words[q] * 4);
+                    dsrc[q] = base + offs[q];
+                }
+            if (!direct) {
+                HIP_CHECK(hipMemcpyAsync(c->dev_tab.p, h, sizeof(i32) * (size_t)tot, hipMemcpyHostToDevice, c->stream));
+                HIP_CHECK(hipEventRecord(c->tab_ev[slot], c->stream));
+            }
         }
-        HIP_CHECK(hipMemcpyAsync(c->dev_tab.p, h, sizeof(i32) * (size_t)tot, hipMemcpyHostToDevice, c->stream));
-        HIP_CHECK(hipEventRecord(c->tab_ev[slot], c->stream));
-        for (size_t q0 = 0; q0 < dst.size(); q0 += CGE_WORD_SEGS) {
-            const int n = (int)std::min<size_t>(CGE_WORD_SEGS, dst.size() - q0);
-            k_copy_words(c, n, &dst[q0], &dsrc[q0], &words[q0]);
+        for (size_t q0 = 0; q0 < n; q0 += CGE_WORD_SEGS) {
+            const int k = (int)std::min<size_t>(CGE_WORD_SEGS, n - q0);
+            k_copy_words(c, k, &dst[q0], &dsrc[q0], &words[q0]);
         }
+        if (slot >= 0 && direct) HIP_CHECK(hipEventRecord(c->tab_ev[slot], c->stream));
         dst.clear(); src.clear(); words.clear();
     }
 };
+struct WordGatherer {
+    cge_ctx *c;
+    std::vector<void *> ddst;
+    std::vector<const void *> dsrc;
+    std::vector<i64> words, offs;
+    i64 base, tot = 0;
+    explicit WordGatherer(cge_ctx *c_, i64 base_ = 0) : c(c_), base(base_ + (base_ & 1)) {}
+    template <class T>
+    size_t add(const T *device, i64 count) {
+        static_assert(sizeof(T) % 4 == 0, "4-byte words");
+        dsrc.push_back(device);
+        const i64 w = count * (i64)(sizeof(T) / 4);
+        words.push_back(w);
+        offs.push_back(base + tot);
+        tot += w + (w & 1);
+        return words.size() - 1;
+    }
+    void fetch() {
+        fetch_async();
+        wait();
+    }
+    void wait() { HIP_CHECK(hipEventSynchronize(c->copy_done)); }
+    void fetch_async() {
+        const size_t need = (size_t)std::max<i64>(base + tot, 1);
+        if (need > c->pin_res.n) HIP_CHECK(hipEventSynchronize(c->copy_done));
+        c->pin_res.ensure(need);
+        ddst.resize(dsrc.size());
+        for (size_t q = 0; q < dsrc.size(); q++) ddst[q] = c->pin_res.p + offs[q];
+        for (size_t q0 = 0; q0 < dsrc.size(); q0 += CGE_WORD_SEGS) {
+            const int n = (int)std::min<size_t>(CGE_WORD_SEGS, dsrc.size() - q0);
+            k_copy_words(c, n, &ddst[q0], &dsrc[q0], &words[q0]);
+        }
+        HIP_CHECK(hipEventRecord(c->copy_done, c->stream));
+    }
+    template <class T>
+    const T *get(size_t item) const { return reinterpret_cast<const T *>(c->pin_res.p + offs[item]); }
+};
+template <class T>
+inline void fetch_words(cge_ctx *c, const T *device, i64 count, T *host) {
+    static_assert(sizeof(T) % 4 == 0, "4-byte words");
+    if (count * (i64)(sizeof(T) / 4) > CGE_WORD_ZERO_MAX) {
+        HIP_CHECK(hipMemcpyAsync(host, device, sizeof(T) * (size_t)count, hipMemcpyDeviceToHost, c->stream));
+        HIP_CHECK(hipStreamSynchronize(c->stream));
+        return;
+    }
+    WordGatherer g(c);
+    const size_t i = g.add(device, count);
+    g.fetch();
+    std::memcpy(host, g.get<T>(i), sizeof(T) * (size_t)count);
+}
 void k_gather_means_slots(cge_ctx *c, const double *arena, const i64 *off, const i64 *slot, i64 T, i64 d, i64 stride, i64 lead,
                           double *dst);
 void k_pow_prepare(cge_ctx *c, const double *D, i64 N, bool upper_only, bool blocked = false);
diff --git a/cge.jl_amd/csrc/diameter_host.cpp b/cge.jl_amd/csrc/diameter_host.cpp
--- a/cge.jl_amd/csrc/diameter_host.cpp
+++ b/cge.jl_amd/csrc/diameter_host.cpp
@@ -37,10 +37,11 @@
             for (i64 k = 0; k < kc; k++) { ij[k] = pairs[k0 + k].x; ij[kc + k] = pairs[k0 + k].y; }
             c->nt_idx.ensure(2 * kc);
             c->nt_out.ensure(kc);
-            HIP_CHECK(hipMemcpyAsync(c->nt_idx.p, ij.data(), sizeof(i32) * 2 * kc, hipMemcpyHostToDevice, st));
+            WordPacker pk(c);
+            pk.add(c->nt_idx.p, ij.data(), 2 * kc);
+            pk.flush();
             k_pair_dist(c, c->Xr.p, d, c->nt_idx.p, c->nt_idx.p + kc, kc, 1.0, c->nt_out.p);
-            HIP_CHECK(hipMemcpyAsync(val.data(), c->nt_out.p, sizeof(double) * kc, hipMemcpyDeviceToHost, st));
-            HIP_CHECK(hipStreamSynchronize(st));
+            fetch_words(c, c->nt_out.p, kc, val.data());
             for (i64 k = 0; k < kc; k++) eb.offer(val[k], ij[k], ij[kc + k]);
         }
         return;
@@ -90,6 +91,7 @@
 }
 
 static const i64 NT_CAP = (i64)1 << 20;
+static const i64 DM_HEAD = 4096;
 template <class Flush>
 static void dm_collect(cge_ctx *c, const double *Xs, const double *rns, i64 ld, i64 nrows, i64 dpad, const std::vector<int2> &tl,
                        int tri, double thr, const i32 *ids, Flush flush) {
@@ -97,21 +99,27 @@
     if (ntiles == 0) return;
     c->nt_pairs.ensure((size_t)NT_CAP);
     c->nt_tiles.ensure((size_t)ntiles);
-    HIP_CHECK(hipMemcpyAsync(c->nt_tiles.p, tl.data(), sizeof(int2) * ntiles, hipMemcpyHostToDevice, c->stream));
-    std::vector<int2> h;
+    {
+        WordPacker pk(c);
+        pk.add(c->nt_tiles.p, tl.data(), ntiles);
+        pk.flush();
+    }
+    std::vector<int2> h(DM_HEAD);
     i64 t0 = 0, step = std::min<i64>(ntiles, (i64)1 << 17);
     while (t0 < ntiles) {
         const i64 t1 = std::min(ntiles, t0 + step);
-        const i64 cnt = k_pair_collect(c, Xs, rns, ld, nrows, dpad, c->nt_tiles.p, t0, t1, tri, thr, ids, c->nt_pairs.p, NT_CAP);
+        const i64 cnt = k_pair_collect(c, Xs, rns, ld, nrows, dpad, c->nt_tiles.p, t0, t1, tri, thr, ids, c->nt_pairs.p, NT_CAP, h.data(),
+                                       DM_HEAD);
         if (cnt > NT_CAP) {
             if (t1 - t0 <= 1) CGE_THROW(CGE_E_ARG, "diameter: a tile with more pairs than it has entries");
             step = (t1 - t0 + 1) / 2;
             continue;
         }
         if (cnt > 0) {
-            h.resize(cnt);
-            HIP_CHECK(hipMemcpyAsync(h.data(), c->nt_pairs.p, sizeof(int2) * cnt, hipMemcpyDeviceToHost, c->stream));
-            HIP_CHECK(hipStreamSynchronize(c->stream));
+            if (cnt > DM_HEAD) {
+                h.resize(cnt);
+                fetch_words(c, c->nt_pairs.p, cnt, h.data());
+            }
             flush(h.data(), cnt);
         }
         t0 = t1;
@@ -265,9 +273,8 @@
     k_gather_centre_fm(c, mu_ref, nullptr, c->gmean.p, c->Ms.p, c->mnorm.p, nref, d, ldm, dpad, f32 ? c->Ms32.p : nullptr,
                        b16 ? c->Mb16.p : nullptr, KP, lowp ? c->dm_flag.p : nullptr);
     int unfit = 0;
-    if (lowp) HIP_CHECK(hipMemcpyAsync(&unfit, c->dm_flag.p, sizeof(int), hipMemcpyDeviceToHost, st));
     S.seed_norm = -1.0;
-    S.seed_vertex = k_argmax_mapped(c, c->rns.p, npos, c->pos2node.p, &S.seed_norm);
+    S.seed_vertex = k_argmax_mapped(c, c->rns.p, npos, c->pos2node.p, &S.seed_norm, lowp ? c->dm_flag.p : nullptr, &unfit);
     if (RS && lowp) {
         const double bad = cge_allreduce_scalar_max(c, (unfit & 1) ? 1.0 : 0.0), big = cge_allreduce_scalar_max(c, (unfit & 2) ? 1.0 : 0.0);
         unfit = (bad != 0.0 ? 1 : 0) | (big != 0.0 ? 2 : 0);
@@ -394,19 +401,19 @@
     dm_eval_pairs(c, &far, 1, S.eb);
     const i64 cap = std::min<i64>(S.N * (S.N + 1) / 2, (i64)4 << 20);
     c->bound_list.ensure((size_t)cap);
+    const i64 nhead = std::min(cap, DM_HEAD);
+    S.cand.resize(nhead);
     const i64 cnt = k_bound_select(c, c->Pm.p, c->mp_lref.p, S.N, P.nref, S.L * (1.0 - 1e-9), c->bound_list.p, cap,
-                                   P.by_comm ? c->mp_refoff.p : nullptr, P.by_comm ? c->mp_refmem.p : nullptr);
+                                   P.by_comm ? c->mp_refoff.p : nullptr, P.by_comm ? c->mp_refmem.p : nullptr, S.cand.data(), nhead);
     c->stat_cand_pairs = cnt;
     if (cnt > cap) {
+        S.cand.clear();
         if (S.RS) CGE_THROW(CGE_E_ARG, "diameter (shard_rows): the bounds prune too little (more than %lld candidate landmark pairs) and the brute-force "
                                        "fallback needs every row on one rank", (long long)cap);
         return false;
     }
     S.cand.resize(cnt);
-    if (cnt > 0) {
-        HIP_CHECK(hipMemcpyAsync(S.cand.data(), c->bound_list.p, sizeof(BoundRec) * cnt, hipMemcpyDeviceToHost, c->stream));
-        HIP_CHECK(hipStreamSynchronize(c->stream));
-    }
+    if (cnt > nhead) fetch_words(c, c->bound_list.p, cnt, S.cand.data());
     S.lap("dm_select");
     std::make_heap(S.cand.begin(), S.cand.end(), cand_later);
     S.left = S.cand.size();
diff --git a/cge.jl_amd/csrc/kernels_dist.hip b/cge.jl_amd/csrc/kernels_dist.hip
--- a/cge.jl_amd/csrc/kernels_dist.hip
+++ b/cge.jl_amd/csrc/kernels_dist.hip
@@ -776,10 +776,15 @@
     }
 }
 
-static void best_of_recs(cge_ctx *c, const MaxRec *d_recs, int nwg, double *bv, i64 *bi, i64 *bj, std::vector<double> *wg = nullptr) {
-    std::vector<MaxRec> h(nwg);
-    HIP_CHECK(hipMemcpyAsync(h.data(), d_recs, sizeof(MaxRec) * nwg, hipMemcpyDeviceToHost, c->stream));
-    HIP_CHECK(hipStreamSynchronize(c->stream));
+static void best_of_recs(cge_ctx *c, const MaxRec *d_recs, int nwg, double *bv, i64 *bi, i64 *bj, std::vector<double> *wg = nullptr,
+                         const int *ride_dev = nullptr, int *ride_host = nullptr) {
+    static_assert(sizeof(MaxRec) % 8 == 0, "MaxRec travels as 8-byte items");
+    WordGatherer g(c);
+    const size_t i_recs = g.add(reinterpret_cast<const unsigned long long *>(d_recs), (i64)(sizeof(MaxRec) / 8) * nwg);
+    const size_t i_ride = ride_dev ? g.add(ride_dev, 1) : 0;
+    g.fetch();
+    const MaxRec *h = reinterpret_cast<const MaxRec *>(g.get<unsigned long long>(i_recs));
+    if (ride_dev) *ride_host = *g.get<int>(i_ride);
     *bv = -1.0; *bi = 0; *bj = 0;
     for (int k = 0; k < nwg; k++)
         if (h[k].val > *bv || (h[k].val == *bv && (h[k].i < *bi || (h[k].i == *bi && h[k].j < *bj)))) {
@@ -889,7 +894,7 @@
     }
 }
 i64 k_pair_collect(cge_ctx *c, const double *Xs, const double *rns, i64 ld, i64 nrows, i64 dpad, const int2 *tiles, i64 t0, i64 t1,
-                   int tri, double thr, const i32 *ids, int2 *out, i64 cap) {
+                   int tri, double thr, const i32 *ids, int2 *out, i64 cap, int2 *head, i64 nhead) {
     if (t1 <= t0) return 0;
     c->mp_count.ensure(2);
     unsigned *cnt = reinterpret_cast<unsigned *>(c->mp_count.p);
@@ -899,10 +904,11 @@
         hipLaunchKernelGGL(pair_collect_kernel, dim3((unsigned)std::min<i64>(t1 - t0, MP_NWG)), dim3(256), MP_LDS_BYTES, c->stream, Xs, rns,
                            ld, nrows, dpad, tiles, t0, t1, tri, thr, ids, out, cnt, (unsigned)cap);
     }
-    unsigned h = 0;
-    HIP_CHECK(hipMemcpyAsync(&h, cnt, sizeof(unsigned), hipMemcpyDeviceToHost, c->stream));
-    HIP_CHECK(hipStreamSynchronize(c->stream));
-    return (i64)h;
+    WordGatherer g(c);
+    const size_t i_cnt = g.add(cnt, 1), i_head = g.add(out, head ? nhead : 0);
+    g.fetch();
+    if (head) std::memcpy(head, g.get<int2>(i_head), sizeof(int2) * (size_t)nhead);
+    return (i64)*g.get<unsigned>(i_cnt);
 }
 
 __global__ __launch_bounds__(256) void bound_select_kernel(const double *__restrict__ Q, const i32 *__restrict__ lref,
@@ -991,7 +997,7 @@
     hipLaunchKernelGGL(ref_dist2_fm_kernel, dim3((unsigned)nref), dim3(256), 0, c->stream, Ms_fm, nref, dpad, ldm, c->mp_rd2.p);
 }
 i64 k_bound_select(cge_ctx *c, const double *Q, const i32 *lref, i64 N, i64 nref, double L, BoundRec *list, i64 cap,
-                   const i32 *ref_off, const i32 *ref_mem) {
+                   const i32 *ref_off, const i32 *ref_mem, BoundRec *head, i64 nhead) {
     c->mp_count.ensure(2);
     HIP_CHECK(hipMemsetAsync(c->mp_count.p, 0, 2 * sizeof(i64), c->stream));
     ScopedKernelTimer tm(c, "bound_select");
@@ -1007,10 +1013,11 @@
     } else
         hipLaunchKernelGGL(bound_select_kernel, dim3(grid_for(N * N, 256)), dim3(256), 0, c->stream, Q, lref, c->mp_rd2.p, N,
                            nref, L, list, cap, reinterpret_cast<unsigned long long *>(c->mp_count.p));
-    i64 cnt = 0;
-    HIP_CHECK(hipMemcpyAsync(&cnt, c->mp_count.p, sizeof(i64), hipMemcpyDeviceToHost, c->stream));
-    HIP_CHECK(hipStreamSynchronize(c->stream));
-    return cnt;
+    WordGatherer g(c);
+    const size_t i_cnt = g.add(c->mp_count.p, 1), i_head = g.add(list, head ? nhead : 0);
+    g.fetch();
+    if (head) std::memcpy(head, g.get<BoundRec>(i_head), sizeof(BoundRec) * (size_t)nhead);
+    return *g.get<i64>(i_cnt);
 }
 
 __device__ __forceinline__ double row16_sum(double v) {
@@ -1071,15 +1078,19 @@
         if (v[i] > best) { best = v[i]; bi = i; }
     reduce_best(best, bi, map ? (i64)map[bi] : bi, lds, recs);
 }
-i64 k_argmax_mapped(cge_ctx *c, const double *v, i64 n, const i32 *map, double *val) {
-    if (n <= 0) { if (val) *val = -1.0; return -1; }
+i64 k_argmax_mapped(cge_ctx *c, const double *v, i64 n, const i32 *map, double *val, const int *ride_dev, int *ride_host) {
+    if (n <= 0) {
+        if (val) *val = -1.0;
+        if (ride_dev) fetch_words(c, ride_dev, 1, ride_host);
+        return -1;
+    }
     c->mp_recs.ensure(MP_NWG);
     MaxRec *recs = c->mp_recs.p;
     const int nwg = (int)std::max<i64>(1, std::min<i64>((n + 255) / 256, 256));
     hipLaunchKernelGGL(argmax_kernel, dim3(nwg), dim3(256), 768 * sizeof(double), c->stream, v, n, map, recs);
     double bv;
     i64 bi, bj;
-    best_of_recs(c, recs, nwg, &bv, &bi, &bj);
+    best_of_recs(c, recs, nwg, &bv, &bi, &bj, nullptr, ride_dev, ride_host);
     if (val) *val = bv;
     return bj;
 }
diff --git a/cge.jl_amd/csrc/kernels_lm.hip b/cge.jl_amd/csrc/kernels_lm.hip
--- a/cge.jl_amd/csrc/kernels_lm.hip
+++ b/cge.jl_amd/csrc/kernels_lm.hip
@@ -236,14 +236,16 @@
                         double *rnorm, i64 npos, i64 d, i64 ld, i64 dpad, float *dst32, unsigned short *planes, i64 KP,
                         int *flag) {
     const bool planes_only = planes && !dst && !dst32 && npos > 0;
-    if (dst) HIP_CHECK(hipMemsetAsync(dst, 0, sizeof(double) * (size_t)(ld * dpad), c->stream));
+    WordPacker zr(c);
+    if (dst) zr.zero_bytes(dst, sizeof(double) * (size_t)(ld * dpad));
     if (planes_only) {
         for (int q = 0; q < 2; q++)
-            HIP_CHECK(hipMemsetAsync(planes + (size_t)q * ld * KP + (size_t)npos * KP, 0, sizeof(unsigned short) * (size_t)((ld - npos) * KP), c->stream));
+            zr.zero_bytes(planes + (size_t)q * ld * KP + (size_t)npos * KP, sizeof(unsigned short) * (size_t)((ld - npos) * KP));
     } else if (planes)
-        HIP_CHECK(hipMemsetAsync(planes, 0, sizeof(unsigned short) * (size_t)(2 * ld * KP), c->stream));
-    if (dst32) HIP_CHECK(hipMemsetAsync(dst32, 0, sizeof(float) * (size_t)(ld * dpad), c->stream));
-    HIP_CHECK(hipMemsetAsync(rnorm, 0, sizeof(double) * (size_t)ld, c->stream));
+        zr.zero_bytes(planes, sizeof(unsigned short) * (size_t)(2 * ld * KP));
+    if (dst32) zr.zero_bytes(dst32, sizeof(float) * (size_t)(ld * dpad));
+    zr.zero_bytes(rnorm, sizeof(double) * (size_t)ld);
+    zr.flush();
     if (planes_only) {
         const unsigned nb = (unsigned)std::min<i64>((npos + 15) / 16, 16384);
         hipLaunchKernelGGL(gather_planes_kernel, dim3(nb), dim3(256), 0, c->stream, src_rowmajor, idx, mean, npos, d, ld, planes, KP,
@@ -302,8 +304,7 @@
     hipLaunchKernelGGL(count_distinct_kernel, dim3(grid_for(n, 256, 1024)), dim3(256), 0, c->stream, hash, n, c->uniq_table.p, tsize - 1,
                        c->uniq_table.p + tsize);
     unsigned long long cnt = 0;
-    HIP_CHECK(hipMemcpyAsync(&cnt, c->uniq_table.p + tsize, sizeof(cnt), hipMemcpyDeviceToHost, c->stream));
-    HIP_CHECK(hipStreamSynchronize(c->stream));
+    fetch_words(c, c->uniq_table.p + tsize, 1, &cnt);
     return (i64)cnt;
 }
 
@@ -1715,7 +1716,7 @@
         long long beg = 0;
 #pragma unroll
         for (int q = 0; q < CGE_WORD_SEGS; q++) {
-            if (q < n && i >= beg && i < s.end[q]) s.dst[q][i - beg] = s.src[q][i - beg];
+            if (q < n && i >= beg && i < s.end[q]) s.dst[q][i - beg] = s.src[q] ? s.src[q][i - beg] : 0u;
             if (q < n) beg = s.end[q];
         }
     }
@@ -1734,6 +1735,10 @@
     if (tot == 0) return;
     const unsigned nb = (unsigned)std::min<long long>((tot + 255) / 256, 1024);
     hipLaunchKernelGGL(copy_words_kernel, dim3(nb), dim3(256), 0, c->stream, s, nseg);
+}
+void k_zero_words(cge_ctx *c, int nseg, void *const *dst, const i64 *words) {
+    const void *none[CGE_WORD_SEGS] = {};
+    k_copy_words(c, nseg, dst, none, words);
 }
 
 __device__ __forceinline__ double fast_rcp(double q) {
diff --git a/cge.jl_amd/csrc/kernels_sort.hip b/cge.jl_amd/csrc/kernels_sort.hip
--- a/cge.jl_amd/csrc/kernels_sort.hip
+++ b/cge.jl_amd/csrc/kernels_sort.hip
@@ -404,8 +404,7 @@
     HIP_CHECK(radix_pairs(c->sort_tmp.p, bytes, (const unsigned *)v2l, (unsigned *)c->sort_keys32.p,
                                         c->sort_idx.p, mem, (size_t)n, 0, bits, st));
     i32 bad = 0;
-    HIP_CHECK(hipMemcpyAsync(&bad, c->sort_cnt.p, sizeof(i32), hipMemcpyDeviceToHost, st));
-    HIP_CHECK(hipStreamSynchronize(st));
+    fetch_words(c, c->sort_cnt.p, 1, &bad);
     return bad;
 }
 
diff --git a/cge.jl_amd/csrc/landmarks_host.cpp b/cge.jl_amd/csrc/landmarks_host.cpp
--- a/cge.jl_amd/csrc/landmarks_host.cpp
+++ b/cge.jl_amd/csrc/landmarks_host.cpp
@@ -341,44 +341,6 @@
     B.chunk_order.resize(B.NC);
     for (i64 ch = 0; ch < B.NC; ch++) B.chunk_order[first[bucket(ch)]++] = (i32)ch;
 }
-struct WordGatherer {
-    cge_ctx *c;
-    std::vector<void *> ddst;
-    std::vector<const void *> dsrc;
-    std::vector<i64> words, offs;
-    i64 tot = 0;
-    explicit WordGatherer(cge_ctx *c_) : c(c_) {}
-    template <class T>
-    size_t add(const T *device, i64 count) {
-        static_assert(sizeof(T) % 4 == 0, "4-byte words");
-        dsrc.push_back(device);
-        const i64 w = count * (i64)(sizeof(T) / 4);
-        words.push_back(w);
-        offs.push_back(tot);
-        tot += w + (w & 1);
-        return words.size() - 1;
-    }
-    void fetch() {
-        fetch_async();
-        wait();
-    }
-    void wait() { HIP_CHECK(hipEventSynchronize(c->copy_done)); }
-    void fetch_async() {
-        c->pin_res.ensure((size_t)std::max<i64>(tot, 1));
-        c->dev_res.ensure((size_t)std::max<i64>(tot, 1));
-        ddst.resize(dsrc.size());
-        for (size_t q = 0; q < dsrc.size(); q++) ddst[q] = c->dev_res.p + offs[q];
-        for (size_t q0 = 0; q0 < dsrc.size(); q0 += CGE_WORD_SEGS) {
-            const int n = (int)std::min<size_t>(CGE_WORD_SEGS, dsrc.size() - q0);
-            k_copy_words(c, n, &ddst[q0], &dsrc[q0], &words[q0]);
-        }
-        if (tot > 0)
-            HIP_CHECK(hipMemcpyAsync(c->pin_res.p, c->dev_res.p, sizeof(i32) * (size_t)tot, hipMemcpyDeviceToHost, c->stream));
-        HIP_CHECK(hipEventRecord(c->copy_done, c->stream));
-    }
-    template <class T>
-    const T *get(size_t item) const { return reinterpret_cast<const T *>(c->pin_res.p + offs[item]); }
-};
 void upload_tables(cge_ctx *c, const Batch &B, WordPacker &pk) {
     const i64 d = c->d;
     c->ls_rows.ensure(B.R); c->ls_row_task.ensure(B.R); c->ls_ct.ensure(B.NC); c->ls_cb.ensure(B.NC);
@@ -684,7 +646,6 @@
 void rule_cut_enqueue(cge_ctx *c, SplitBatch &S, bool use_median) {
     const Batch &B = S.B;
     const i64 T = B.T, R = B.R, d = c->d;
-    hipStream_t st = c->stream;
     if (use_median) {
         c->sp_srows.ensure(R); c->sp_zs.ensure(R); c->sp_perm.ensure(R); c->sp_status.ensure(T);
         k_segmented_sort_z(c, c->ls_z.p, c->ls_rows.p, c->ls_row_task.p, c->sp_tro.p, R, T, c->sp_zs.p, c->sp_perm.p,
@@ -693,22 +654,20 @@
     c->ls_nlow.ensure(T);
     k_cut_sides(c, c->ls_z.p, use_median ? c->sp_zs.p : nullptr, c->sp_tro.p, T, use_median ? 1 : 0, c->ls_side.p, c->ls_nlow.p,
                 c->cut_ties.p);
-    c->pin_res.ensure((size_t)T);
-    HIP_CHECK(hipMemcpyAsync(c->pin_res.p, c->ls_nlow.p, sizeof(i32) * T, hipMemcpyDeviceToHost, st));
     k_group_side_sums(c, c->Xr.p, lm_vw(c), c->ls_rows.p, c->ls_side.p, c->ls_cb.p, c->ls_ce.p, B.NC, c->ls_tco.p, B.T, d,
                       c->ls_part.p, c->ls_sums.p);
     c->sp_vals.ensure(2 * T);
     k_side_values_means(c, c->ls_sums.p, T, d, c->sp_vals.p, c->lm_means.p + S.mbase);
-    c->pin_sums.ensure((size_t)2 * T);
-    HIP_CHECK(hipMemcpyAsync(c->pin_sums.p, c->sp_vals.p, sizeof(double) * 2 * T, hipMemcpyDeviceToHost, st));
-    HIP_CHECK(hipEventRecord(c->copy_done, st));
+    S.wg.reset(new WordGatherer(c));
+    S.i_nlow = S.wg->add(c->ls_nlow.p, T); S.i_vals = S.wg->add(c->sp_vals.p, 2 * T);
+    S.wg->fetch_async();
     k_sort_children(c, c->ls_side.p, c->ls_rows.p, c->sp_tro.p, c->ls_cb.p, c->ls_ce.p, c->ls_tco.p, B.NC, R, T, 2, c->lm_arena.p + S.base);
 }
 void rule_cut_collect(cge_ctx *c, SplitBatch &S) {
     const i64 T = S.B.T, d = c->d;
-    HIP_CHECK(hipEventSynchronize(c->copy_done));
-    const double *vals = c->pin_sums.p;
-    std::memcpy(S.nlow.data(), c->pin_res.p, sizeof(i32) * T);
+    S.wg->wait();
+    const double *vals = S.wg->get<double>(S.i_vals);
+    std::memcpy(S.nlow.data(), S.wg->get<i32>(S.i_nlow), sizeof(i32) * T);
     for (i64 t = 0; t < T; t++) {
         Group *g = S.groups[t];
         S.vlow[t] = vals[2 * t];
@@ -1467,9 +1426,13 @@
     }
     DevBuf<i32> &v2l_rows = RS ? c->v2l_loc : c->v2l;
     c->lm_goff.ensure(NG); c->lm_glen.ensure(NG); c->v2l.ensure(n); v2l_rows.ensure(nrows); c->lm_mem.ensure(nrows); c->lm_memoff.ensure(NG + 1);
-    HIP_CHECK(hipMemcpyAsync(c->lm_goff.p, goff, sizeof(i32) * NG, hipMemcpyHostToDevice, st));
-    HIP_CHECK(hipMemcpyAsync(c->lm_glen.p, glen, sizeof(i32) * NG, hipMemcpyHostToDevice, st));
-    HIP_CHECK(hipMemcpyAsync(c->lm_memoff.p, c->h_mem_off.data(), sizeof(i32) * (NG + 1), hipMemcpyHostToDevice, st));
+    {
+        WordPacker pk(c);
+        pk.add(c->lm_goff.p, goff, NG);
+        pk.add(c->lm_glen.p, glen, NG);
+        pk.add(c->lm_memoff.p, c->h_mem_off.data(), NG + 1);
+        pk.flush();
+    }
     const i64 unassigned = k_groups_to_index(c, c->lm_arena.p, c->lm_goff.p, c->lm_glen.p, NG, nrows, v2l_rows.p, c->lm_mem.p);
     bool cover_bad = unassigned != 0 || c->h_mem_off[NG] != nrows || c->h_gl_off[NG] != n;
     if (RS) {
diff --git a/cge.jl_amd/csrc/score_host.cpp b/cge.jl_amd/csrc/score_host.cpp
--- a/cge.jl_amd/csrc/score_host.cpp
+++ b/cge.jl_amd/csrc/score_host.cpp
@@ -131,8 +131,7 @@
         cge_allreduce_dev(c, reinterpret_cast<double *>(cnt.p), 1, 2);
     } else if (!tiled)
         k_compact_count(c, c->wedges.p, N, directed, cnt.p);
-    HIP_CHECK(hipMemcpyAsync(&c->n_ledges, cnt.p, sizeof(i64), hipMemcpyDeviceToHost, st));
-    HIP_CHECK(hipStreamSynchronize(st));
+    fetch_words(c, cnt.p, 1, &c->n_ledges);
     c->wedges_ready = true;
 }
 
@@ -381,8 +380,7 @@
     const i64 N = c->N;
     S.ov = resident_orig_view(c, c->lweight.p);
     S.lcomm_host.resize(N);
-    HIP_CHECK(hipMemcpyAsync(S.lcomm_host.data(), c->lcomm.p, sizeof(i32) * N, hipMemcpyDeviceToHost, c->stream));
-    HIP_CHECK(hipStreamSynchronize(c->stream));
+    fetch_words(c, c->lcomm.p, N, S.lcomm_host.data());
     S.ov.hi = host_diameter_landmarks(c, c->lemb.p, c->lweight.p, S.lcomm_host, c->n_comm_max, N);
     S.ov.h_lcomm = S.lcomm_host.data();
     c->phases.ms["diameter"] = now_ms() - t0;
diff --git a/cge.jl_amd/csrc/wgcl_host.cpp b/cge.jl_amd/csrc/wgcl_host.cpp
--- a/cge.jl_amd/csrc/wgcl_host.cpp
+++ b/cge.jl_amd/csrc/wgcl_host.cpp
@@ -454,9 +454,13 @@
     const double *GD = c->sw_GD.p;
     double *Tin = c->sw_T1.p, *Tout = c->sw_T2.p;
     int *flags = c->sw_flags.p;
-    HIP_CHECK(hipMemsetAsync(flags, 0, sizeof(int) * 4, st));
     const double init[2] = {0.9, 1.0};
-    HIP_CHECK(hipMemcpyAsync(c->sw_fitstate.p, init, sizeof(init), hipMemcpyHostToDevice, st));
+    {
+        WordPacker pk(c);
+        pk.zero(flags, 4);
+        pk.add(c->sw_fitstate.p, init, 2);
+        pk.flush();
+    }
     bool enqueued_only = false;
     if (fit.persistent_dir && k_fit_persistent_dir(c, GD, N, Tin, Tout, G.deg_in, G.deg_out, 0.9, 1.0, AlphaBook::delta,
                                                    &sl.iters, (int *)(c->sw_scal.p + RES_FIT), &enqueued_only)) {
diff --git a/include/cge_hip_testing.h b/include/cge_hip_testing.h
--- a/include/cge_hip_testing.h
+++ b/include/cge_hip_testing.h
@@ -7,6 +7,10 @@
 int cge_host_eig_top(const double *A, int64_t d, double *v);
 int cge_batch_pack_test(const int64_t *N, int64_t K, int cus, int32_t *group_of);
 int cge_host_pos_draw(int64_t seed, int64_t stream_id, int64_t S, int64_t m, int64_t *pos_idx);
+int cge_word_layout_test(const int64_t *words, int64_t n, int64_t *offs, int64_t *total, int64_t *launches);
+int cge_word_exchange_test(void *ctx, int64_t nseg, const int64_t *words, const uint8_t *item8, const uint8_t *copied, int64_t rounds,
+                           const uint32_t *host_in, int64_t nzero, const int64_t *zero_seg, const int64_t *zero_beg,
+                           const int64_t *zero_len, uint32_t *dev_out, uint32_t *gathered);
 int cge_group_eig(void *ctx, const double *A, int64_t T, int64_t d, double *v);
 int cge_group_stats_test(void *ctx, const int32_t *ids, const int32_t *task_row_off, int64_t T, const uint8_t *side, const double *mean_in,
                          double *mean, double *sw, double *cov, double *vec, double *z, double *sums);
diff --git a/profiles/word_exchange_probe.py b/profiles/word_exchange_probe.py
--- /dev/null
+++ b/profiles/word_exchange_probe.py
@@ -0,0 +1,29 @@
+import os
+import sys
+import time
+
+import numpy as np
+
+sys.path.insert(0, os.path.dirname(os.path.dirname(os.path.abspath(__file__))))
+from cge.jl_amd import api
+
+reps = int(sys.argv[1]) if len(sys.argv) > 1 else 5
+ctx = api.Context(0)
+rng = np.random.default_rng(0)
+print(f"{'words':>9s} {'KB':>8s} {'rounds':>6s} {'direct us':>10s} {'copy us':>10s}")
+for W in (64, 1024, 4096, 16384, 65536, 262144, 1048576, 4194304):
+    rounds = 64 if W <= 262144 else 8
+    x = rng.integers(1, 2**32 - 1, size=(rounds, W), dtype=np.uint64).astype(np.uint32)
+    best = {}
+    for mode, limit in (("direct", 1 << 40), ("copy", 0)):
+        ctx.set_option("word_direct_max", limit)
+        ctx.word_exchange_test([W], x)
+        t = []
+        for _ in range(reps):
+            t0 = time.perf_counter()
+            dev, got = ctx.word_exchange_test([W], x)
+            t.append((time.perf_counter() - t0) / rounds * 1e6)
+        assert np.array_equal(got, x)
+        best[mode] = min(t)
+    print(f"{W:9d} {W * 4 / 1024:8.1f} {rounds:6d} {best['direct']:10.1f} {best['copy']:10.1f}", flush=True)
+ctx.close()
```

New measurement: 12.01 billion, median of 6. 1.01x the previous value.
